# NVIDIA/tensorrt-laboratory

Hardware: NVIDIA H100
Metric: ResNet-50 fp16 b=8 inferences/sec (higher is better)
Workload: dtype f16

## Files before the change

### __graft_entry__.py

```python
from __future__ import annotations

import os
import re
import shutil
import subprocess
import sysconfig
import sys

ROOT = os.path.dirname(os.path.abspath(__file__))
PKG = os.path.join(ROOT, "tensorrt_laboratory_b200")
CSRC = os.path.join(PKG, "csrc")
LIB = os.path.join(PKG, "libb200infer.so")

NVCC_FLAGS = [
    "-gencode", "arch=compute_90a,code=sm_90a", "-lineinfo", "-O3", "-std=c++17",
    "-Xcompiler", "-fPIC,-Wall,-Wno-unused-function", "-cudart", "static",
]


def _nvcc() -> str:
    for cand in (os.environ.get("NVCC"), shutil.which("nvcc"), "/usr/local/cuda/bin/nvcc"):
        if cand and os.path.exists(cand):
            return cand
    raise RuntimeError("nvcc not found")


def _sources():
    srcs = []
    for root, _, files in os.walk(CSRC):
        for f in sorted(files):
            if f.endswith((".cu", ".cc")) and not f.endswith(("_main.cc", "_module.cc")):
                srcs.append(os.path.join(root, f))
    return srcs


def _stale(target: str, deps) -> bool:
    if not os.path.exists(target):
        return True
    t = os.path.getmtime(target)
    for d in deps:
        if os.path.getmtime(d) > t:
            return True
    return False


def _all_deps():
    deps = []
    for root, _, files in os.walk(CSRC):
        deps += [os.path.join(root, f) for f in files if f.endswith((".cu", ".cc", ".h", ".cuh", ".hpp"))]
    deps.append(os.path.join(ROOT, "include", "b200infer.h"))
    inc = os.path.join(ROOT, "include")
    for root, _, files in os.walk(inc):
        deps += [os.path.join(root, f) for f in files]
    return deps


_CONV_KERNEL = re.compile(r"conv|net_f16_tcgen05|attention_f16_wgmma|embed_ln|layernorm_h8|pooler")


_SHARED_SM_KERNEL = re.compile(r"_ZN3b2k(?:16conv_f16_tcgen05|20conv3x3_halo_tcgen05|24conv3x3_halo_1x1_tcgen05)ILi(\d+)E")
_SHARED_SM_THREADS = 320


def _shared_sm_register_budget(bn: int):
    ctas = 3 if bn <= 64 else 2 if bn <= 128 else 1
    return None if ctas == 1 else 65536 // (_SHARED_SM_THREADS * ctas) // 8 * 8


def _ptxas_violations(log: str):
    bad = [line.strip() for line in log.splitlines() if "(C7520)" in line or "(C7518)" in line]
    func = None
    for line in log.splitlines():
        m = re.search(r"Function properties for (\S+)", line)
        if m:
            func = m.group(1)
            continue
        m = re.search(r"(\d+) bytes spill stores, (\d+) bytes spill loads", line)
        if m and func and _CONV_KERNEL.search(func) and (int(m.group(1)) or int(m.group(2))):
            bad.append(f"{func}: {line.strip()}")
        m = re.search(r"Used (\d+) registers", line)
        k = _SHARED_SM_KERNEL.match(func) if (m and func) else None
        if k:
            budget = _shared_sm_register_budget(int(k.group(1)))
            if budget is not None and int(m.group(1)) > budget:
                bad.append(f"{func}: {m.group(1)} registers, more than the {budget} at which its CTAs share an SM")
    return bad


def _compile_object(cmd, obj: str, verbose: bool) -> None:
    r = subprocess.run(cmd + ["-Xptxas", "-v"], capture_output=True, text=True)
    log = r.stdout + r.stderr
    shown = [line for line in log.splitlines() if verbose or not (line.startswith("ptxas info") or "bytes stack frame" in line)]
    if shown:
        sys.stderr.write("\n".join(shown) + "\n")
    if r.returncode:
        raise subprocess.CalledProcessError(r.returncode, cmd)
    bad = _ptxas_violations(log)
    if bad:
        os.remove(obj)
        raise RuntimeError(f"{os.path.basename(obj)}: ptxas reports serialised wgmma, spilling convolution / transformer "
                           "kernels or tile kernels over their register budget:\n  " +
                           "\n  ".join(bad))


def build(force: bool = False, verbose: bool = False) -> None:
    nvcc = _nvcc()
    objdir = os.path.join(ROOT, "build", "obj")
    os.makedirs(objdir, exist_ok=True)
    deps = _all_deps()
    objs = []
    for src in _sources():
        obj = os.path.join(objdir, os.path.relpath(src, CSRC).replace(os.sep, "_") + ".o")
        objs.append(obj)
        if force or _stale(obj, deps):
            cmd = [nvcc] + NVCC_FLAGS + ["-I", os.path.join(ROOT, "include"), "-I", CSRC]
            if src.endswith(".cc"):
                cmd += ["-x", "cu"]
            cmd += ["-c", src, "-o", obj]
            if verbose:
                print(" ".join(cmd))
            _compile_object(cmd, obj, verbose)
    if force or _stale(LIB, objs):
        cmd = [nvcc, "-shared", "-cudart", "static", "-o", LIB] + objs + ["-lpthread", "-ldl", "-lrt"]
        if verbose:
            print(" ".join(cmd))
        subprocess.run(cmd, check=True)
    main_src = os.path.join(CSRC, "trtlab", "infer_main.cc")
    exe = os.path.join(ROOT, "examples", "infer.x")
    os.makedirs(os.path.dirname(exe), exist_ok=True)
    if os.path.exists(main_src) and (force or _stale(exe, deps + [LIB])):
        cmd = [nvcc] + NVCC_FLAGS + ["-I", os.path.join(ROOT, "include"), "-I", CSRC, "-x", "cu", main_src,
                                     "-o", exe, "-L", PKG, "-lb200infer", "-Xlinker", "-rpath,$ORIGIN/../tensorrt_laboratory_b200",
                                     "-lpthread", "-ldl"]
        if verbose:
            print(" ".join(cmd))
        subprocess.run(cmd, check=True)
    py_src = os.path.join(CSRC, "pybind", "trtlab_module.cc")
    py_mod = os.path.join(PKG, "trtlab" + sysconfig.get_config_var("EXT_SUFFIX"))
    if os.path.exists(py_src) and (force or _stale(py_mod, deps + [LIB, py_src])):
        import pybind11
        cmd = [nvcc] + NVCC_FLAGS + ["-I", os.path.join(ROOT, "include"), "-I", CSRC, "-I", pybind11.get_include(),
                                     "-I", sysconfig.get_paths()["include"], "-Xcompiler", "-fvisibility=hidden", "-x", "cu", "-shared", py_src,
                                     "-o", py_mod,
                                     "-L", PKG, "-lb200infer", "-Xlinker", "-rpath,$ORIGIN", "-lpthread", "-ldl"]
        if verbose:
            print(" ".join(cmd))
        subprocess.run(cmd, check=True)
    if ROOT not in sys.path:
        sys.path.insert(0, ROOT)
    import tensorrt_laboratory_b200
    from tensorrt_laboratory_b200 import capi
    capi.load()


def smoke() -> None:
    if ROOT not in sys.path:
        sys.path.insert(0, ROOT)
    if not os.path.exists(LIB):
        build()
    from tests import smoke_impl
    smoke_impl.run()


if __name__ == "__main__":
    build(force="--force" in sys.argv, verbose=True)
    if "--smoke" in sys.argv:
# ... 2 lines not shown
```

### tensorrt_laboratory_b200/csrc/engine.cu

```cuda
#include <cuda.h>
#include <cuda_runtime.h>
#include <stdarg.h>
#include <stdio.h>
#include <stdlib.h>
#include <string.h>

#include <algorithm>
#include <map>
#include <memory>
#include <mutex>
#include <string>
#include <vector>

#include "../../include/b200infer.h"
#include "kernels.h"
#include "plan_format.h"

#include "b2_internal.h"

namespace b2i {
thread_local std::string g_err;
int fail(int code, const char* fmt, ...) {
    char buf[1024];
    va_list ap;
// ... 106 lines not shown
             L_OUTPUT_CAST_F8 };

struct NetRun {
    b2k::NetArgs args{};
    int ctas = 0;
    int first_op = 0, last_op = 0;
    void* d_blob = nullptr;
    ~NetRun() {
        if (d_blob) cudaFree(d_blob);
    }
};

struct Launch {
    LKind kind;
    std::string name;
    double flops = 0, bytes = 0;
    b2k::ConvLaunch conv;
    b2k::SimtConvArgs simt;
    const void* in = nullptr;
    void* out = nullptr;
    const void* w = nullptr;
    const float* bias = nullptr;
    int in_binding = -1, out_binding = -1;
    bool src_half = false;
    int max_blocks = 0;
    int side_join = -1;
    std::shared_ptr<NetRun> net;
    b2k::TailArgs tail{};
    b2k::I8ConvLaunch i8{};
    float qscale = 0.f;
    int C_in_phys = 0;
    bool net_member = false;
    b2k::EmbedArgs embed{};
    int in_binding2 = -1, in_binding3 = -1;
    b2k::AttnLaunch attn{};
    float eps = 0.f;
    const int* live = nullptr;
    const int* pos_map = nullptr;
    int N = 0, C = 0, H = 0, W = 0, C_phys = 0, Ho = 0, Wo = 0, k = 0, stride = 0, pad = 0, K = 0, Cout = 0;
};

struct Segment {
    int begin = 0, end = 0;
    bool graphable = false;
    cudaGraphExec_t exec = nullptr;
};
struct BindPatch {
    int launch = -1;
    cudaGraphNode_t node = nullptr;
    cudaKernelNodeParams np{};
    std::vector<void*> params;
    int n_params = 0;
    std::vector<std::pair<int, int>> slots;
    std::vector<void*> values;
    b2k::TailArgs tail{};
    bool is_tail = false;
};
struct Plan {
    int batch = 0;
    bool has_net = false;
    std::vector<Launch> launches;
    std::vector<Segment> segments;
    bool graph_failed = false;
    cudaGraph_t graph = nullptr;
    cudaGraphExec_t exec = nullptr;
    std::vector<BindPatch> patches;
    ~Plan() {
        for (Segment& sg : segments)
            if (sg.exec) cudaGraphExecDestroy(sg.exec);
        if (exec) cudaGraphExecDestroy(exec);
        if (graph) cudaGraphDestroy(graph);
    }
};

}

struct ConvConfig {
    int bn, stages, splits;
    double est_us;
    int sps = 1;
    int ws = 0;
    int cn = 1;
    int halo = 0;
};
static bool stage_depth_useful(int bn, int kb, int st, int kpc) {
    const int stgs[4] = {1, 2, 4, 8};
    int cover = 0, deepest = 0;
    for (int s2 : stgs) {
        if (!b2k::conv_config_exists(bn, kb, s2)) continue;
        deepest = s2;
        if (!cover && s2 >= kpc) cover = s2;
    }
    return st <= (cover ? cover : deepest);
}


constexpr int kHaloStagesTag = 2;

struct b2_runtime {
    b2_alloc_fn alloc = nullptr;
    b2_free_fn free_ = nullptr;
    void* user = nullptr;
};

struct b2_engine {
    b2_runtime* rt = nullptr;
    b2_alloc_fn alloc = nullptr;
    b2_free_fn free_ = nullptr;
    void* alloc_user = nullptr;
    std::string name;
    int precision = 0, max_batch = 0;
    std::vector<Tensor> tensors;
    std::vector<Op> ops;
    std::vector<Binding> bindings;
    uint8_t* d_payload = nullptr;
    size_t payload_bytes = 0;
    size_t arena_bytes = 0;
    size_t act_bytes = 0;
    int device = -1;
    bool inspect_only = false;
    double flops_per_item = 0;
    std::mutex tune_mutex;
    std::mutex tune_run_mutex;
    std::map<std::pair<int, int>, ConvConfig> tuned;
    bool tune_cache_loaded = false;
    std::map<int, float> requant_r;
    bool tactics_from_plan = false;
    bool tuned_at_load = false;
    int pack_tensor = -1;
    bool half() const { return precision != B2_PREC_FP32; }
    bool one_byte() const { return precision == B2_PREC_INT8 || precision == B2_PREC_FP8; }
    bool fp8() const { return precision == B2_PREC_FP8; }
};

struct b2_context {
    b2_engine* e = nullptr;
    uint8_t* scratch = nullptr;
    struct ScratchState {
        std::map<int, std::unique_ptr<Plan>> plans;
    };
    std::map<uint8_t*, ScratchState> states;
    ScratchState* cur = nullptr;
    int* d_counters = nullptr;
    int use_graph = 1;
    int force_simt = 0;
    int force_im2col = 0;
    int force_bn = 0;
    int force_stages = 0;
    int force_splits = 0;
    int force_sps = 0;
    int force_halo = 0;
    int force_fuse = 0;
    int force_cn = 0;
    int force_ws = 0;
    int pdl_trigger = 1;
    int no_fold = 0;
    int autotune = 4;
    int fork = 0;
    int net = 0;
    int net_ctas = 0;
    int net_bn = 0;
    int net_stages = 0;
    int i8_bn = 0;
    int i8_stages = 0;
    int fuse_tail = 1;
    int input_ctas = 0;
    int* d_tail_ctrl = nullptr;
    cudaStream_t side = nullptr;
    cudaEvent_t fork_ev = nullptr, join_ev = nullptr;
};

namespace {

std::string fixed_str(const char* p, size_t n) {
    size_t len = 0;
    while (len < n && p[len]) ++len;
    return std::string(p, len);
}

int validate_transformer_op(b2_engine* e, const Op& op) {
    using namespace b2plan;
    const OpRec& r = op.r;
    const char* nm = op.name.c_str();
    auto act_ok = [&](const Tensor& t) { return t.kind == T_ACT && t.scale == 0.f && t.c % 8 == 0 && t.c <= 1024; };
    switch (r.type) {
        case OP_EMBED_LN: {
            const Tensor& to = e->tensors[r.out];
            const Tensor& tm = e->tensors[op.out2];
            const uint32_t want_c = (op.flags & kOpPacked) ? to.w + 2 : to.w;
            if (!act_ok(to) || to.h != 1 || tm.kind != T_VEC || tm.c != want_c || tm.binding >= 0)
                return fail(B2_EINVAL, "plan: embedding %s: needs an fp16 [1, S, C <= 1024, C %% 8 == 0] output and an fp32 [S] mask tensor "
                            "([S + 2] packing index when packed)", nm);
            if ((op.flags & kOpPacked) && to.w % 32)
                return fail(B2_EINVAL, "plan: packed embedding %s: S = %u is not a multiple of 32", nm, to.w);
            if (op.vocab < 1 || op.types < 1 || op.positions < int(to.w))
                return fail(B2_EINVAL, "plan: embedding %s: vocab %d / positions %d / types %d do not cover S = %u", nm, op.vocab, op.positions,
                            op.types, to.w);
            if (r.w_bytes != uint64_t(op.vocab + op.positions + op.types) * to.c * 2 || r.b_bytes != uint64_t(to.c) * 8)
                return fail(B2_EINVAL, "plan: embedding %s: table / gamma / beta sizes do not match hidden size %u", nm, to.c);
            if (!(op.eps >= 0.f && op.eps < 1.f)) return fail(B2_EINVAL, "plan: embedding %s: bad eps", nm);
            break;
        }
        case OP_LAYERNORM: {
            const Tensor& ti = e->tensors[r.in];
            const Tensor& to = e->tensors[r.out];
            if (!act_ok(ti) || !act_ok(to) || ti.h != to.h || ti.w != to.w || ti.c != to.c || ti.c_phys != to.c_phys)
                return fail(B2_EINVAL, "plan: layernorm %s: needs fp16 input and output of one shape, C %% 8 == 0, C <= 1024", nm);
            if (r.w_bytes != 0 || r.b_bytes != uint64_t(ti.c) * 8) return fail(B2_EINVAL, "plan: layernorm %s: gamma / beta size mismatch", nm);
            if (!(op.eps >= 0.f && op.eps < 1.f)) return fail(B2_EINVAL, "plan: layernorm %s: bad eps", nm);
            break;
        }
        case OP_ATTENTION: {
            const Tensor& ti = e->tensors[r.in];
            const Tensor& to = e->tensors[r.out];
            if (r.res < 0) return fail(B2_EINVAL, "plan: attention %s: no mask tensor", nm);
            const Tensor& tm = e->tensors[r.res];
            if (op.heads < 1 || uint32_t(op.heads) * 64 != to.c)
                return fail(B2_EINVAL, "plan: attention %s: heads * 64 (%d * 64) != hidden size %u", nm, op.heads, to.c);
            if (!act_ok(to) || ti.kind != T_ACT || ti.scale != 0.f || ti.c != 3 * to.c || ti.c_phys != ti.c)
                return fail(B2_EINVAL, "plan: attention %s: needs a fused fp16 QKV input of 3 x %u channels", nm, to.c);
            if (ti.h != 1 || to.h != 1 || ti.w != to.w || tm.kind != T_VEC || tm.c != ((op.flags & kOpPacked) ? ti.w + 2 : ti.w))
                return fail(B2_EINVAL, "plan: attention %s: S does not match between QKV, output and mask", nm);
            if (ti.w != 64 && (ti.w == 0 || ti.w % 128 || ti.w > 512))
                return fail(B2_EINVAL, "plan: attention %s: S = %u (64, or a multiple of 128 up to 512)", nm, ti.w);
            if (r.w_bytes || r.b_bytes) return fail(B2_EINVAL, "plan: attention %s carries no weights", nm);
            e->flops_per_item += 4.0 * double(ti.w) * ti.w * to.c;
            break;
        }
        case OP_POOLER: {
            const Tensor& ti = e->tensors[r.in];
            const Tensor& to = e->tensors[r.out];
            if (!act_ok(ti) || ti.h != 1 || to.kind != T_VEC || to.c != ti.c)
                return fail(B2_EINVAL, "plan: pooler %s: needs an fp16 [1, S, C] input and an fp32 [C] output", nm);
            if (r.w_bytes != uint64_t(ti.c) * ti.c * 2 || r.b_bytes != uint64_t(ti.c) * 4)
                return fail(B2_EINVAL, "plan: pooler %s: weight / bias size mismatch", nm);
            e->flops_per_item += 2.0 * ti.c * ti.c;
            break;
// ... 207 lines not shown
            if (to.h != ho || to.w != wo) return fail(B2_EINVAL, "plan: conv %s output dims mismatch", op.name.c_str());
            e->flops_per_item += 2.0 * ho * wo * r.cout * op.algo_k();
        } else if (r.type == OP_FC) {
            const Tensor& ti = e->tensors[r.in];
            const size_t K = size_t(ti.h) * ti.w * ti.c_phys;
            if (r.w_bytes != size_t(r.cout) * K * elt || r.b_bytes != size_t(r.cout) * 4)
                return fail(B2_EINVAL, "plan: fc %s weight size mismatch", op.name.c_str());
            e->flops_per_item += 2.0 * ti.h * ti.w * ti.c * r.cout;
        } else if (transformer_op) {
            int rc = validate_transformer_op(e, op);
            if (rc) return rc;
        }
        e->ops.push_back(op);
    }
    if (int rc = validate_packed_ops(e)) return rc;
    for (uint32_t i = 0; i < h.n_bindings; ++i, p += sizeof(BindingRec)) {
        BindingRec r;
        memcpy(&r, p, sizeof r);
        Binding b;
        b.name = fixed_str(r.name, 64);
        b.is_input = r.is_input != 0;
        b.dtype = r.dtype;
        b.tensor = r.tensor;
        b.nd = r.nd;
        if (r.nd == 0 || r.nd > 8) return fail(B2_EINVAL, "plan: binding %s has bad rank", b.name.c_str());
        if (r.dtype != B2_DT_FLOAT && !(r.dtype == B2_DT_HALF && b.is_input && h.precision == B2_PREC_FP16) &&
            !(r.dtype == B2_DT_INT32 && b.is_input && v3))
            return fail(B2_EINVAL, "plan: binding %s: bindings are fp32 (inputs of fp16 engines may be fp16)", b.name.c_str());
        size_t n = 1;
        for (uint32_t d = 0; d < 8; ++d) {
            b.dims[d] = d < r.nd ? r.dims[d] : 0;
            if (d < r.nd) n *= size_t(r.dims[d]);
        }
        b.item_bytes = n * (r.dtype == B2_DT_HALF ? 2 : 4);
        e->bindings.push_back(b);
    }
    for (const Op& op : e->ops) {
        const OpRec& r = op.r;
        if (r.type != OP_INPUT_CAST && r.type != OP_OUTPUT_CAST) continue;
        const Binding& b = e->bindings[size_t(r.binding)];
        const Tensor& t = e->tensors[size_t(r.type == OP_INPUT_CAST ? r.out : r.in)];
        size_t n = 1;
        for (int d = 0; d < b.nd; ++d) n *= size_t(b.dims[d] > 0 ? b.dims[d] : 0);
        const bool s2d = r.type == OP_INPUT_CAST && r.k == 2;
        if (b.is_input != (r.type == OP_INPUT_CAST) || (!s2d && n != size_t(t.c) * t.h * t.w))
            return fail(B2_EINVAL, "plan: cast op %s: binding %s and tensor %s disagree", op.name.c_str(), b.name.c_str(), t.name.c_str());
        if (b.dtype == B2_DT_INT32)
            return fail(B2_EINVAL, "plan: cast op %s reads int32 binding %s (int32 bindings feed the embedding op only)", op.name.c_str(),
                        b.name.c_str());
    }
    std::vector<int> int32_readers(e->bindings.size(), 0);
    for (const Op& op : e->ops) {
        const OpRec& r = op.r;
        if (r.type == OP_POOLER && e->tensors[r.out].binding >= 0 && e->bindings[size_t(e->tensors[r.out].binding)].is_input)
            return fail(B2_EINVAL, "plan: pooler %s writes an input binding", op.name.c_str());
        if (r.type != OP_EMBED_LN) continue;
        const uint32_t S = e->tensors[r.out].w;
        for (int bi : {r.binding, op.binding2, op.binding3}) {
            if (bi < 0 || bi >= int(h.n_bindings)) return fail(B2_EINVAL, "plan: embedding %s has a bad binding", op.name.c_str());
            const Binding& b = e->bindings[size_t(bi)];
            if (b.dtype != B2_DT_INT32 || !b.is_input || b.nd != 1 || b.dims[0] != int32_t(S))
                return fail(B2_EINVAL, "plan: embedding %s: binding %s must be an int32 input of shape [S = %u]", op.name.c_str(), b.name.c_str(), S);
            ++int32_readers[size_t(bi)];
        }
    }
    for (size_t i = 0; i < e->bindings.size(); ++i) {
        if (e->bindings[i].dtype != B2_DT_INT32) continue;
        if (int32_readers[i] != 1)
            return fail(B2_EINVAL, "plan: int32 binding %s must feed exactly one embedding op slot", e->bindings[i].name.c_str());
        for (const Tensor& t : e->tensors)
            if (t.binding == int(i))
                return fail(B2_EINVAL, "plan: int32 binding %s is the storage of tensor %s (int32 bindings feed the embedding op only)",
                            e->bindings[i].name.c_str(), t.name.c_str());
    }
    if (h.n_tactics) {
        if (h.tactics_offset > nbytes || size_t(h.n_tactics) > (nbytes - h.tactics_offset) / sizeof(TacticRec))
            return fail(B2_EINVAL, "plan: tactic table outside the blob");
        for (uint32_t i = 0; i < h.n_tactics; ++i) {
            TacticRec t;
            memcpy(&t, base + h.tactics_offset + size_t(i) * sizeof(TacticRec), sizeof t);
            if (t.op >= h.n_ops || t.batch == 0 || t.batch > h.max_batch) return fail(B2_EINVAL, "plan: tactic %u out of range", i);
            ConvConfig cfg{int(t.bn), int(t.stages), int(t.splits), 0.0, int(t.sps), int(t.ws), int(t.cn)};
            cfg.halo = int(t.halo);
            e->tuned[{int(t.op), int(t.batch)}] = cfg;
        }
        e->tactics_from_plan = true;
    }
    *payload = base + h.payload_offset;
    return B2_OK;
}

int fuse_partner(const b2_engine* e, int i);

void plan_arena(b2_engine* e) {
    int busy_until = -1;
    for (size_t i = 0; i < e->ops.size(); ++i) {
        Op& op = e->ops[i];
        op.side_join = -1;
        if (int(i) <= busy_until || op.r.type != b2plan::OP_CONV || op.r.out < 0 || e->tensors[op.r.out].binding >= 0) continue;
        int consumers = 0, join = -1;
        bool as_residual_only = true;
        for (size_t k = i + 1; k < e->ops.size(); ++k) {
            const auto& rk = e->ops[k].r;
            if (rk.in == op.r.out) ++consumers, as_residual_only = false;
            if (rk.res == op.r.out) ++consumers, join = int(k);
        }
        if (consumers == 1 && as_residual_only && join > int(i) + 1) {
            op.side_join = join;
            busy_until = join;
        }
    }
    for (size_t i = 0; i < e->ops.size(); ++i) {
        const auto& r = e->ops[i].r;
        for (int t : {r.out, e->ops[i].out2})
            if (t >= 0 && e->tensors[t].def < 0) e->tensors[t].def = int(i);
        for (int t : {r.in, r.res})
            if (t >= 0) e->tensors[t].last_use = std::max(e->tensors[t].last_use, int(i));
        if (e->ops[i].side_join >= 0 && r.in >= 0) e->tensors[r.in].last_use = std::max(e->tensors[r.in].last_use, e->ops[i].side_join);
        const int j = fuse_partner(e, int(i));
        if (j >= 0) e->tensors[r.in].last_use = std::max(e->tensors[r.in].last_use, j);
    }
    if (e->pack_tensor >= 0) e->tensors[size_t(e->pack_tensor)].last_use = int(e->ops.size()) - 1;
    struct Live {
        size_t off, size;
        int last;
    };
    std::vector<Live> live;
    size_t top = 0;
    std::vector<int> order;
    for (size_t i = 0; i < e->tensors.size(); ++i)
        if (e->tensors[i].binding < 0 && e->tensors[i].def >= 0) order.push_back(int(i));
    std::stable_sort(order.begin(), order.end(), [&](int a, int b) { return e->tensors[a].def < e->tensors[b].def; });
    for (int ti : order) {
        Tensor& t = e->tensors[ti];
        if (t.last_use < t.def) t.last_use = t.def;
        const size_t size = align_up(t.item_bytes * e->max_batch, 1024);
        const int slack = e->half() ? env_int("B2_ARENA_SLACK", env_int("B2_NET", 0) ? 2 : 0) : 0;
        live.erase(std::remove_if(live.begin(), live.end(), [&](const Live& l) { return l.last + slack < t.def; }), live.end());
        std::sort(live.begin(), live.end(), [](const Live& a, const Live& b) { return a.off < b.off; });
        size_t off = 0;
        for (const Live& l : live) {
            if (off + size <= l.off) break;
            off = std::max(off, l.off + l.size);
        }
        t.offset = off;
        live.push_back({off, size, t.last_use});
        top = std::max(top, off + size);
    }
    e->act_bytes = align_up(std::max<size_t>(top, 1024), 1024);
    e->arena_bytes = e->act_bytes + (e->half() ? kSplitWorkspaceBytes : 0);
}

int make_map_2d(CUtensorMap* map, const void* base, uint64_t inner, uint64_t outer, uint32_t box_inner,
                uint32_t box_outer, CUtensorMapSwizzle swz, bool int8 = false) {
    cuuint64_t dims[2] = {inner, outer};
    cuuint64_t strides[1] = {inner * (int8 ? 1u : 2u)};
    cuuint32_t box[2] = {box_inner, box_outer};
    cuuint32_t estr[2] = {1, 1};
    CUresult r = g_encode_tiled(map, int8 ? CU_TENSOR_MAP_DATA_TYPE_UINT8 : CU_TENSOR_MAP_DATA_TYPE_FLOAT16, 2, const_cast<void*>(base), dims, strides, box,
                                estr, CU_TENSOR_MAP_INTERLEAVE_NONE, swz, CU_TENSOR_MAP_L2_PROMOTION_L2_256B,
                                CU_TENSOR_MAP_FLOAT_OOB_FILL_NONE);
    if (r != CUDA_SUCCESS)
        return fail(B2_ECUDA, "cuTensorMapEncodeTiled failed (%d) dims=%llu,%llu box=%u,%u", int(r),
                    (unsigned long long)inner, (unsigned long long)outer, box_inner, box_outer);
    return B2_OK;
}
// ... 63 lines not shown
                const double t_kb = std::max(stage_bytes / (70000.0 / sharing), 1.0 / st);
                double t_epi = 0.6 + bn / 64.0 * 0.4 + (residual ? 0.4 : 0.0);
                if (splits > 1) t_epi += 1.0 + 0.3 * splits;
                const double t_cta = 2.0 + kpc * t_kb + t_epi;
                double total = waves * t_cta;
                const double traffic = double(ctas) * kpc * stage_bytes;
                total = std::max(total, traffic / 5.0e6 + 2.0);
                if (total < best.est_us) best = ConvConfig{bn, st, splits, total};
            }
        }
    }
    return best;
}

bool conv_is_row_folded(const b2_context* c, const Op& op) {
    const b2plan::OpRec& r = op.r;
    return !c->no_fold && r.cin_phys == 8 && op.kw() * 8 * 2 == 64 && op.sw() == 1 && op.pw_lo() == 0 && op.pw_hi() == 0;
}
int conv_kb(const b2_context* c, const Op& op) {
    if (op.r.cin_phys % 64 == 0) return 64;
    return conv_is_row_folded(c, op) ? 32 : 8;
}
int conv_num_kblocks(const b2_context* c, const Op& op) {
    const b2plan::OpRec& r = op.r;
    if (op.group_span()) return int(r.taps) * (op.group_span() / 64);
    if (r.cin_phys % 64 == 0) return int(r.taps) * (int(r.cin_phys) / 64);
    if (conv_is_row_folded(c, op)) return (op.kh() + 1) / 2;
    return (int(r.taps_phys) + 7) / 8;
}

int conv_halo_rows(const b2_engine* e, const Op& op) {
    const b2plan::OpRec& r = op.r;
    const Tensor& ti = e->tensors[r.in];
    const Tensor& to = e->tensors[r.out];
    if (op.groups > 1 || r.cin_phys % 64 || r.cout_phys % 64 || op.kh() != 3 || op.kw() != 3 || op.sh() != 1 || op.sw() != 1 || op.ph() != 1 ||
        op.pw_lo() != 1 || op.pw_hi() != 1 || r.res >= 0 || !(r.relu & 2) || ti.h != to.h || ti.w != to.w)
        return 0;
    const int wp = int(to.w) + 2;
    if (wp > 128) return 0;
    return std::min(128 / wp, int(to.h));
}
int conv_halo_rows(const b2_context* c, const Op& op) { return conv_halo_rows(c->e, op); }
bool conv_on_tensor_cores(const b2_engine* e, const Op& op);

int fuse_partner(const b2_engine* e, int i) {
    if (!e->half() || e->one_byte() || i < 0 || size_t(i) + 1 >= e->ops.size()) return -1;
    const Op &oi = e->ops[size_t(i)], &oj = e->ops[size_t(i) + 1];
    const b2plan::OpRec &ri = oi.r, &rj = oj.r;
    if (ri.type != b2plan::OP_CONV || rj.type != b2plan::OP_CONV || (ri.relu & (4 | b2plan::kConvGelu)) || conv_halo_rows(e, oi) == 0 ||
        !b2k::conv_halo_config_exists(int(ri.cout_phys)) || ri.cin_phys / 64 > 8)
        return -1;
    if (rj.in != ri.out || rj.res < 0 || rj.res == ri.out || oj.kh() != 1 || oj.kw() != 1 || oj.sh() != 1 || oj.sw() != 1 || oj.ph() != 0 ||
        oj.pw_lo() != 0 || oj.pw_hi() != 0 || oj.groups != 1 || !(rj.relu & 2) || (rj.relu & (4 | b2plan::kConvGelu)) ||
        rj.cin_phys != ri.cout_phys || rj.cout_phys % 64 || !conv_on_tensor_cores(e, oj) || e->tensors[ri.out].binding >= 0)
        return -1;
    for (size_t k = 0; k < e->ops.size(); ++k) {
        const b2plan::OpRec& rk = e->ops[k].r;
        if (k != size_t(i) + 1 && (rk.in == ri.out || rk.res == ri.out || e->ops[k].out2 == ri.out)) return -1;
        if (k == size_t(i) + 1 && rk.res == ri.out) return -1;
    }
    return i + 1;
}

bool conv_on_tensor_cores(const b2_engine* e, const Op& op) {
    const b2plan::OpRec& r = op.r;
    const bool kb64 = r.cin_phys % 64 == 0, kb8 = r.cin_phys == 8;
    return e->half() && (kb64 || kb8) && r.cout_phys % 32 == 0 && (kb64 || r.taps_phys % 2 == 0) && (op.groups == 1 || op.group_span() > 0);
}

bool conv_takes_stem_ws(const b2_context* c, const Op& op) {
    const b2plan::OpRec& r = op.r;
    return conv_is_row_folded(c, op) && op.kh() == 7 && op.sh() == 2 && r.cout_phys == 64 && c->e->tensors[r.out].w <= 128 &&
           (r.relu & b2plan::kConvRelu) && !(r.relu & 2) && !(r.relu & b2plan::kConvGelu) && r.res < 0 && op.groups == 1;
}

bool conv_takes_ws(const b2_context* c, const Op& op) {
    return conv_takes_stem_ws(c, op) || (conv_kb(c, op) == 64 && (op.r.relu & 2) && op.groups == 1 && !(op.r.relu & b2plan::kConvGelu));
}

bool tactic_applies(const b2_context* c, const Op& op, int batch, const ConvConfig& cfg) {
    const b2plan::OpRec& r = op.r;
    const Tensor& to = c->e->tensors[r.out];
    const int span = op.group_span(), kb = conv_kb(c, op);
    if (cfg.bn <= 0 || int(r.cout_phys) % cfg.bn || cfg.splits < 1 || cfg.sps < 1 || cfg.ws < 0) return false;
    if (op.groups > 1 && (!span || span % cfg.bn || cfg.splits > 1)) return false;
    if ((op.groups > 1 || (r.relu & b2plan::kConvGelu)) && (cfg.ws || cfg.cn > 1 || cfg.halo)) return false;
    if ((op.flags & b2plan::kOpPacked) && (cfg.ws || cfg.cn > 1 || cfg.halo || cfg.splits > 1)) return false;
    if (cfg.halo == 2) {
        const int j = fuse_partner(c->e, int(&op - &c->e->ops[0]));
        const int R = conv_halo_rows(c, op), cblocks = int(r.cin_phys) / 64;
        return j >= 0 && c->force_fuse >= 0 && cfg.bn == int(r.cout_phys) && cfg.splits == 1 && !cfg.ws && cfg.cn <= 1 &&
               b2k::conv_halo_fused_smem(cfg.bn, int(to.w), R, cblocks, int(c->e->ops[size_t(j)].r.cout_phys)) <= kSmemLimit;
    }
    if (cfg.halo) {
        const int R = conv_halo_rows(c, op), cblocks = int(r.cin_phys) / 64;
        return cfg.halo == 1 && R && cfg.splits == 1 && !cfg.ws && cfg.cn <= 1 && b2k::conv_halo_config_exists(cfg.bn) && cblocks <= 8 &&
               b2k::conv_halo_smem(cfg.bn, int(to.w), R, cblocks) <= kSmemLimit;
    }
    if (cfg.ws && conv_is_row_folded(c, op))
        return conv_takes_stem_ws(c, op) && cfg.bn == 64 && cfg.stages == b2k::kStemWsRing && cfg.sps == 1 && cfg.splits == 1 &&
               cfg.cn <= 1 && b2k::conv_stem_ws_smem() <= kSmemLimit;
    if (cfg.ws)
        return conv_takes_ws(c, op) && cfg.splits == 1 && cfg.cn <= 1 && b2k::conv_ws_config_exists(cfg.bn, cfg.stages, cfg.sps) &&
               b2k::conv_ws_smem(cfg.bn, cfg.stages, cfg.sps, r.res >= 0) <= kSmemLimit;
    if (!b2k::conv_config_exists(cfg.bn, kb, cfg.stages, cfg.sps) || b2k::conv_smem_bytes(cfg.bn, cfg.stages, r.res >= 0, cfg.sps) > kSmemLimit)
        return false;
    const int grid_n = int(r.cout_phys) / cfg.bn;
    if (cfg.cn > 1 && (kb != 64 || grid_n % cfg.cn || !b2k::conv_cluster_config_exists(cfg.bn, cfg.stages, cfg.sps, cfg.cn))) return false;
    if (cfg.splits > 1) {
        const int nkb = conv_num_kblocks(c, op), kpc = (nkb + cfg.splits - 1) / cfg.splits;
        const int tiles = (batch * int(to.h * to.w) + 127) / 128 * grid_n;
        if (kb != 64 || kpc < 4 || (cfg.splits - 1) * kpc >= nkb || tiles > kMaxSplitTiles ||
            size_t(tiles) * cfg.splits * 128 * cfg.bn * 4 > kSplitWorkspaceBytes)
            return false;
    }
    return true;
}

constexpr int kFuseMinStreams = 4;

ConvConfig fused_conv_config(const Op& op) {
    ConvConfig f{int(op.r.cout_phys), kHaloStagesTag, 1, 0.0, 1, 0, 1};
    f.halo = 2;
    return f;
}

std::vector<ConvConfig> conv_candidates(const b2_context* c, const Op& op, int batch, int fixed_splits) {
    const b2plan::OpRec& r = op.r;
    const int kbsz = conv_kb(c, op), nkb = conv_num_kblocks(c, op);
    const int m_tiles = (batch * int(c->e->tensors[r.out].h * c->e->tensors[r.out].w) + 127) / 128;
    const bool ws_only = c->force_ws > 0 && conv_takes_ws(c, op);
    auto ok = [&](const ConvConfig& t) { return tactic_applies(c, op, batch, t); };
    std::vector<ConvConfig> out;
    for (int bn : {256, 128, 64, 32}) {
        if (int(r.cout_phys) % bn) continue;
        const int tiles = m_tiles * (int(r.cout_phys) / bn);
        for (int ws = 0; ws <= 1; ++ws)
        for (int sp : {1, 2, 4, 8})
        for (int sps = 1; sps <= 2; ++sps)
        for (int st : {1, 2, 4, 8}) {
            if ((fixed_splits > 0 && sp != fixed_splits) || (ws ? c->force_ws < 0 : ws_only)) continue;
            ConvConfig t{bn, st, sp, 0.0, sps, ws ? std::min(tiles, g_sms) : 0, 1};
            if (!ok(t)) continue;
            if (ws) {
                if (sps == 2 && nkb < 4) continue;
                out.push_back(t);
                if (tiles > g_sms / 2) t.ws = g_sms / 2, out.push_back(t);
                continue;
            }
            const int kpc = (nkb + sp - 1) / sp;
            if (sps == 2 ? (kpc < 4 || st * 2 > kpc + 2) : !stage_depth_useful(bn, kbsz, st, kpc)) continue;
            if (sp > 1 && (tiles >= 100 || tiles > kMaxSplitTiles / 8 || tiles * sp > 160)) continue;
            ConvConfig cl = t;
            cl.cn = c->force_cn;
            out.push_back(c->force_cn > 1 && ok(cl) ? cl : t);
        }
    }
    if (conv_takes_stem_ws(c, op) && c->force_ws >= 0 && fixed_splits <= 1) {
        const int rows = batch * int(c->e->tensors[r.out].h);
        ConvConfig t{64, b2k::kStemWsRing, 1, 0.0, 1, std::min(rows, g_sms), 1};
        if (ok(t)) {
            out.push_back(t);
            if (rows > g_sms / 2) t.ws = g_sms / 2, out.push_back(t);
        }
    }
    if (c->force_halo >= 0 && fixed_splits <= 1) {
        std::vector<ConvConfig> halo;
        for (int bn : {256, 128, 64, 32}) {
            const ConvConfig h{bn, kHaloStagesTag, 1, 0.0, 1, 0, 1, 1};
            if (ok(h)) halo.push_back(h);
        }
        if (!halo.empty() && c->force_halo > 0) out.clear();
        out.insert(out.end(), halo.begin(), halo.end());
    }
    return out;
}

ConvConfig forced_conv_config(const b2_context* c, const Op& op, int batch) {
    const b2plan::OpRec& r = op.r;
    const int M = batch * int(c->e->tensors[r.out].h * c->e->tensors[r.out].w);
    const int kbsz = conv_kb(c, op), nkb = conv_num_kblocks(c, op);
    ConvConfig cfg = pick_conv_config(M, int(r.cout_phys), nkb, kbsz, r.res >= 0, c, true, op.group_span());
    if (cfg.bn == 0 || ((op.flags & b2plan::kOpPacked) && cfg.splits > 1))
        cfg = pick_conv_config(M, int(r.cout_phys), nkb, kbsz, r.res >= 0, c, false, op.group_span());
    if (cfg.bn == 0) return cfg;
    auto force = [&](auto set) {
        ConvConfig t = cfg;
        set(t);
        if (tactic_applies(c, op, batch, t)) cfg = t;
    };
    if (c->force_sps == 2) force([](ConvConfig& t) { t.sps = 2; });
    if (c->force_ws > 0)
        force([&](ConvConfig& t) {
            if (conv_takes_stem_ws(c, op)) {
                t = ConvConfig{64, b2k::kStemWsRing, 1, t.est_us, 1, 0, 1};
                t.ws = std::min(batch * int(c->e->tensors[r.out].h), c->force_ws > 1 ? c->force_ws : g_sms);
                return;
            }
            t.ws = std::min((M + 127) / 128 * (int(r.cout_phys) / t.bn), c->force_ws > 1 ? c->force_ws : g_sms);
        });
    if (c->force_halo > 0) force([](ConvConfig& t) { t.halo = 1, t.ws = 0, t.cn = 1; });
    if (c->force_cn > 1) force([&](ConvConfig& t) { t.cn = c->force_cn; });
    return cfg;
}

int make_conv_launch(b2_context* c, const Op& op, int batch, const ConvConfig& cfg, b2k::ConvLaunch* out) {
    b2_engine* e = c->e;
    const b2plan::OpRec& r = op.r;
    const Tensor& ti = e->tensors[r.in];
    const Tensor& to = e->tensors[r.out];
    auto tptr = [&](int idx) -> uint8_t* { return c->scratch + e->tensors[idx].offset; };
    const uint8_t* w = e->d_payload + r.w_off;
    const int M = batch * int(to.h) * int(to.w);
    const bool kb64 = r.cin_phys % 64 == 0;
    const bool fold = conv_is_row_folded(c, op);
    const int span = op.group_span();
    if (!tactic_applies(c, op, batch, cfg))
        return fail(B2_EINVAL, "conv %s: tactic bn=%d st=%d sps=%d splits=%d ws=%d cn=%d halo=%d does not apply", op.name.c_str(), cfg.bn,
                    cfg.stages, cfg.sps, cfg.splits, cfg.ws, cfg.cn, cfg.halo);
    const bool gelu = (r.relu & b2plan::kConvGelu) != 0;
    b2k::ConvLaunch& cl = *out;
    memset(&cl, 0, sizeof cl);
    cl.kb = conv_kb(c, op);
    cl.grid_m = (M + 127) / 128;
    const int nkb = conv_num_kblocks(c, op);
    cl.bn = cfg.bn;
    cl.stages = cfg.stages;
    cl.sps = cfg.sps;
    cl.grid_n = int(r.cout_phys) / cl.bn;
    cl.ws_ctas = cfg.ws;
    cl.cn = std::max(cfg.cn, 1);
    cl.args.cn = cl.cn;
    cl.args.tiles_m = cl.grid_m;
    cl.args.tiles_n = cl.grid_n;
    b2k::ConvArgs& a = cl.args;
    a.splits = cfg.splits;
    a.kb_per_split = (nkb + cfg.splits - 1) / cfg.splits;
    a.workspace = reinterpret_cast<float*>(c->scratch + e->act_bytes);
    a.tile_counters = c->d_counters;
    a.pdl_trigger = c->pdl_trigger;
    a.bias = reinterpret_cast<const float*>(e->d_payload + r.b_off);
    a.residual = r.res >= 0 ? reinterpret_cast<const __half*>(tptr(r.res)) : nullptr;
    a.out = reinterpret_cast<__half*>(tptr(r.out));
    a.M = M;
    a.Cout = int(r.cout_phys);
    a.taps = fold ? op.kh() : int(r.taps);
    a.taps_phys = fold ? op.kh() : int(r.taps_phys);
    a.kw = fold ? 1 : op.kw();
    a.cblocks = span ? span / 64 : kb64 ? int(r.cin_phys) / 64 : 1;
    a.group_span = span;
    a.num_kblocks = nkb;
    a.HoWo = int(to.h * to.w);
    a.Wo = int(to.w);
    a.stride_h = op.sh();
    a.stride_w = op.sw();
    a.pad_h = op.ph();
    a.pad_w = op.pw_lo();
    a.relu = int(r.relu & (b2plan::kConvRelu | b2plan::kConvGelu));
    a.wpacked = (r.relu & 2) ? w : nullptr;
    const bool tiled = r.k == 1 && op.kw() == 1 && r.stride == 1 && op.sw() == 1 && r.pad_ == 0 && op.pw_lo() == 0 &&
                       op.pw_hi() == 0 && kb64 && (!c->force_im2col || gelu || (op.flags & b2plan::kOpPacked));
    a.a_mode = tiled ? b2k::A_TILED : b2k::A_IM2COL;
    if (cfg.halo) {
        const int R = conv_halo_rows(c, op);
        cl.halo = 1;
        cl.ws_ctas = 0, cl.cn = 1, a.cn = 1, a.splits = 1, cl.stages = kHaloStagesTag, cl.sps = 1;
        a.halo_rows = R;
        cl.grid_m = batch * ((int(to.h) + R - 1) / R);
        int rc = make_map_nhwc(&cl.mapA, tptr(r.in), int(r.cin_phys), int(ti.w), int(ti.h), batch, uint32_t(ti.w) + 2, uint32_t(R) + 2);
        if (rc) return rc;
        cl.mapB = cl.mapA;
        if (cfg.halo == 2) {
            const Op& oj = e->ops[size_t(fuse_partner(e, int(&op - &e->ops[0])))];
            const b2plan::OpRec& rj = oj.r;
            cl.halo = 2;
            cl.c2.wpacked = e->d_payload + rj.w_off;
            cl.c2.bias = reinterpret_cast<const float*>(e->d_payload + rj.b_off);
            cl.c2.Cout = int(rj.cout_phys);
            cl.c2.relu = int(rj.relu & b2plan::kConvRelu);
            rc = make_map_nhwc(&cl.mapOut, tptr(rj.out), int(rj.cout_phys), int(to.w), int(to.h), batch, uint32_t(to.w) + 2, uint32_t(R));
            if (!rc) rc = make_map_nhwc(&cl.mapRes, tptr(rj.res), int(rj.cout_phys), int(to.w), int(to.h), batch, uint32_t(to.w) + 2, uint32_t(R));
            return rc;
        }
        rc = make_map_nhwc(&cl.mapOut, tptr(r.out), int(r.cout_phys), int(to.w), int(to.h), batch, uint32_t(to.w) + 2, uint32_t(R));
        cl.mapRes = cl.mapOut;
        return rc;
    }
    const CUtensorMapSwizzle swz = kb64 ? CU_TENSOR_MAP_SWIZZLE_128B : (fold ? CU_TENSOR_MAP_SWIZZLE_64B : CU_TENSOR_MAP_SWIZZLE_NONE);
    const uint64_t pix = uint64_t(r.cin_phys) * 2, rowb = uint64_t(ti.w) * pix, imgb = uint64_t(ti.h) * rowb;
    int rc;
    if (tiled)
        rc = make_map_2d(&cl.mapA, tptr(r.in), r.cin_phys, uint64_t(M), 64, uint32_t(128 / cl.cn), swz);
    else if (fold)
        rc = make_map_im2col(&cl.mapA, tptr(r.in), int(r.cin_phys) * op.kw(), int(ti.w) - op.kw() + 1, int(ti.h), batch, pix,
                             rowb, imgb, op.kh(), 1, op.sh(), 1, op.ph(), 0, 0, 32, 128, swz);
    else
        rc = make_map_im2col(&cl.mapA, tptr(r.in), int(r.cin_phys), int(ti.w), int(ti.h), batch, pix, rowb, imgb, op.kh(),
                             op.kw(), op.sh(), op.sw(), op.ph(), op.pw_lo(), op.pw_hi(), uint32_t(cl.kb), uint32_t(128 / cl.cn), swz);
    if (rc) return rc;
    if (r.relu & 2)
        cl.mapB = cl.mapA;
    else
        rc = make_map_2d(&cl.mapB, w, uint64_t(r.taps_phys) * r.cin_phys, r.cout_phys, uint32_t(cl.kb), uint32_t(cl.bn), swz);
    if (rc) return rc;
    if (cfg.ws && fold) {
        rc = make_map_nhwc(&cl.mapOut, tptr(r.out), int(r.cout_phys), int(to.w), int(to.h), batch, 128, 1);
        cl.mapRes = cl.mapOut;
        return rc;
    }
    const uint32_t ow = cl.bn >= 64 ? 64 : 32;
    const CUtensorMapSwizzle oswz = cl.bn >= 64 ? CU_TENSOR_MAP_SWIZZLE_128B : CU_TENSOR_MAP_SWIZZLE_64B;
    rc = make_map_2d(&cl.mapOut, tptr(r.out), r.cout_phys, uint64_t(M), ow, 128, oswz);
    if (rc) return rc;
    if (r.res >= 0) rc = make_map_2d(&cl.mapRes, tptr(r.res), r.cout_phys, uint64_t(M), ow, 128, oswz);
    else cl.mapRes = cl.mapOut;
    return rc;
}

int make_i8_conv_launch(b2_context* c, const Op& op, int batch, int bn, int stages, b2k::I8ConvLaunch* out) {
    b2_engine* e = c->e;
    const b2plan::OpRec& r = op.r;
    const Tensor& ti = e->tensors[r.in];
    const Tensor& to = e->tensors[r.out];
    auto tptr = [&](int idx) -> uint8_t* { return c->scratch + e->tensors[idx].offset; };
    b2k::I8ConvLaunch& cl = *out;
    memset(&cl, 0, sizeof cl);
    const int M = batch * int(to.h) * int(to.w);
    cl.bn = bn, cl.stages = stages;
    cl.grid_m = (M + 127) / 128;
    cl.grid_n = int(r.cout_phys) / bn;
    b2k::I8ConvArgs& a = cl.args;
    a.wpacked = e->d_payload + r.w_off;
    const float* rq = reinterpret_cast<const float*>(e->d_payload + r.b_off);
    a.m = rq;
    a.b = rq + r.cout_phys;
    a.r = e->requant_r.at(int(&op - &e->ops[0]));
    a.has_res = r.res >= 0 ? 1 : 0;
    a.relu = int(r.relu & 1);
    a.M = M, a.Cout = int(r.cout_phys);
    a.cblocks = int(r.cin_phys) / 128;
    a.last_cb_mmas = (int(r.cin) % 128) ? (int(r.cin) % 128 + 31) / 32 : 4;
    a.cout_real = int(r.cout);
    a.num_kblocks = int(r.taps) * a.cblocks;
    a.kw = op.kw(), a.HoWo = int(to.h * to.w), a.Wo = int(to.w);
    a.stride_h = op.sh(), a.stride_w = op.sw(), a.pad_h = op.ph(), a.pad_w = op.pw_lo();
    const bool tiled = r.k == 1 && r.stride == 1 && r.pad_ == 0;
    a.a_mode = tiled ? b2k::A_TILED : b2k::A_IM2COL;
    int rc;
    if (tiled)
        rc = make_map_2d(&cl.mapA, tptr(r.in), r.cin_phys, uint64_t(M), 128, 128, CU_TENSOR_MAP_SWIZZLE_128B, true);
    else {
        const uint64_t pix = uint64_t(r.cin_phys), rowb = uint64_t(ti.w) * pix, imgb = uint64_t(ti.h) * rowb;
        rc = make_map_im2col(&cl.mapA, tptr(r.in), int(r.cin_phys), int(ti.w), int(ti.h), batch, pix, rowb, imgb, op.kh(), op.kw(), op.sh(),
                             op.sw(), op.ph(), op.pw_lo(), op.pw_hi(), 128, 128, CU_TENSOR_MAP_SWIZZLE_128B, true);
    }
    if (rc) return rc;
    rc = make_map_2d(&cl.mapOut, tptr(r.out), r.cout_phys, uint64_t(M), 128, 128, CU_TENSOR_MAP_SWIZZLE_128B, true);
    if (rc) return rc;
    if (r.res >= 0) rc = make_map_2d(&cl.mapRes, tptr(r.res), r.cout_phys, uint64_t(M), 128, 128, CU_TENSOR_MAP_SWIZZLE_128B, true);
    else cl.mapRes = cl.mapOut;
    return rc;
}

struct TuneTimer {
    const int ns;
    const int iters = std::max(4, env_int("B2_TUNE_ITERS", 12));
    const int reps = std::max(1, env_int("B2_TUNE_REPS", 3));
    std::vector<cudaStream_t> ss;
    std::vector<cudaEvent_t> done;
    cudaEvent_t e0 = nullptr, e1 = nullptr;

    explicit TuneTimer(const b2_context* c) : ns(std::max(1, std::min(c->autotune, 8))), ss(size_t(ns), nullptr), done(size_t(ns), nullptr) {}
    ~TuneTimer() {
// ... 5 lines not shown
        if (e1) cudaEventDestroy(e1);
    }
    int init() {
        bool ok = cudaEventCreate(&e0) == cudaSuccess && cudaEventCreate(&e1) == cudaSuccess;
        for (int i = 0; i < ns && ok; ++i)
            ok = cudaStreamCreateWithFlags(&ss[size_t(i)], cudaStreamNonBlocking) == cudaSuccess &&
                 cudaEventCreateWithFlags(&done[size_t(i)], cudaEventDisableTiming) == cudaSuccess;
        if (ok) return B2_OK;
        cudaGetLastError();
        return fail(B2_ECUDA, "autotune: cannot create streams/events");
    }
    template <class F>
    cudaError_t time(F launch, float* ms) {
        int rc = 0;
        for (int i = 0; i < 2 && !rc; ++i)
            for (int k = 0; k < ns && !rc; ++k) rc = launch(k, ss[size_t(k)]);
        for (auto s : ss) cudaStreamSynchronize(s);
        *ms = 1e30f;
        if (rc) return cudaError_t(rc);
        cudaGraph_t g = nullptr;
        cudaGraphExec_t ge = nullptr;
        cudaError_t se = cudaStreamBeginCapture(ss[0], cudaStreamCaptureModeThreadLocal);
        if (se != cudaSuccess) return se;
        cudaEventRecord(done[0], ss[0]);
        for (int k = 1; k < ns; ++k) cudaStreamWaitEvent(ss[size_t(k)], done[0], 0);
        for (int i = 0; i < iters && !rc; ++i)
            for (int k = 0; k < ns && !rc; ++k) rc = launch(k, ss[size_t(k)]);
        for (int k = 1; k < ns; ++k) {
            cudaEventRecord(done[size_t(k)], ss[size_t(k)]);
            cudaStreamWaitEvent(ss[0], done[size_t(k)], 0);
        }
        se = cudaStreamEndCapture(ss[0], &g);
        if (!rc && se == cudaSuccess) se = cudaGraphInstantiate(&ge, g, 0);
        if (!rc && se == cudaSuccess) se = cudaGraphLaunch(ge, ss[0]);
        if (!rc && se == cudaSuccess) se = cudaStreamSynchronize(ss[0]);
        for (int rep = 0; rep < reps && !rc && se == cudaSuccess; ++rep) {
            cudaEventRecord(e0, ss[0]);
            se = cudaGraphLaunch(ge, ss[0]);
            cudaEventRecord(e1, ss[0]);
            if (se == cudaSuccess) se = cudaStreamSynchronize(ss[0]);
            float t = 0.f;
            if (se == cudaSuccess && cudaEventElapsedTime(&t, e0, e1) == cudaSuccess) *ms = std::min(*ms, t);
        }
        if (ge) cudaGraphExecDestroy(ge);
        if (g) cudaGraphDestroy(g);
        if (rc || se != cudaSuccess) cudaGetLastError();
        return rc ? cudaError_t(rc) : se;
    }
    double us_per_launch(double ms) const { return ms * 1e3 / (iters * ns); }
};

int autotune_conv(b2_context* c, const Op& op, int batch, int fixed_splits, ConvConfig* best_out) {
    const b2plan::OpRec& r = op.r;
    const Tensor& to = c->e->tensors[r.out];
    const int M = batch * int(to.h) * int(to.w);
    TuneTimer tt(c);
    int status = tt.init();
    if (status) return status;
    const int verbose = env_int("B2_TUNE_VERBOSE", 0);
    ConvConfig best = *best_out;
    double best_ms = 1e30;
    for (const ConvConfig& cand : conv_candidates(c, op, batch, fixed_splits)) {
        b2k::ConvLaunch cl0;
        if ((status = make_conv_launch(c, op, batch, cand, &cl0))) return status;
        std::vector<b2k::ConvLaunch> cls(size_t(tt.ns), cl0);
        void* tmp_ws = nullptr;
        if (cand.splits > 1) {
            const size_t ws_bytes = size_t(cl0.grid_m) * cl0.grid_n * cand.splits * 128 * cand.bn * 4;
            if (cudaMalloc(&tmp_ws, ws_bytes * tt.ns) != cudaSuccess) {
                cudaGetLastError();
                continue;
            }
            for (int k = 0; k < tt.ns; ++k) {
                cls[size_t(k)].args.workspace = reinterpret_cast<float*>(static_cast<uint8_t*>(tmp_ws) + ws_bytes * k);
                cls[size_t(k)].args.tile_counters = c->d_counters + k * (kMaxSplitTiles / 8);
            }
        }
        float ms = 0.f;
        const cudaError_t err = tt.time([&](int k, cudaStream_t s) { return b2k::launch_conv_f16_tcgen05(cls[size_t(k)], s); }, &ms);
        if (tmp_ws) cudaFree(tmp_ws);
        if (err != cudaSuccess)
            return fail(B2_ECUDA, "autotune of %s (bn=%d st=%d) failed: %s", op.name.c_str(), cand.bn, cand.stages, cudaGetErrorString(err));
        if (verbose > 1)
            fprintf(stderr, "[b2 tune]   %s b=%d cand bn=%d st=%d sp=%d sps=%d ws=%d cn=%d halo=%d : %.3f us/launch\n", op.name.c_str(),
                    batch, cand.bn, cand.stages, cand.splits, cand.sps, cand.ws, cand.cn, cand.halo, tt.us_per_launch(ms));
        if (ms < best_ms) best_ms = ms, best = cand;
    }
    best.est_us = tt.us_per_launch(best_ms);
    if (verbose)
        fprintf(stderr, "[b2 tune] %s b=%d M=%d N=%d K=%d best bn=%d st=%d sp=%d sps=%d ws=%d cn=%d halo=%d : %.3f us/launch (%d streams)\n",
                op.name.c_str(), batch, M, int(r.cout_phys), conv_num_kblocks(c, op) * conv_kb(c, op), best.bn, best.stages, best.splits,
                best.sps, best.ws, best.cn, best.halo, best.est_us, tt.ns);
    *best_out = best;
    return B2_OK;
}

void tune_cache_load(b2_engine* e) {
    if (e->tune_cache_loaded) return;
    e->tune_cache_loaded = true;
    const char* path = getenv("B2_TUNE_CACHE");
    if (!path) return;
    FILE* f = fopen(path, "r");
    if (!f) return;
    char name[128];
    int op, batch, bn, st, sp, sps, ws, cn, halo;
    while (fscanf(f, "%127s %d %d %d %d %d %d %d %d %d", name, &op, &batch, &bn, &st, &sp, &sps, &ws, &cn, &halo) == 10)
        if (e->name == name && op >= 0 && op < int(e->ops.size())) {
            ConvConfig cfg{bn, st, sp, 0.0, sps, ws, cn};
            cfg.halo = halo;
            e->tuned[{op, batch}] = cfg;
        }
    fclose(f);
}
void tune_cache_append(const b2_engine* e, int op, int batch, const ConvConfig& cfg) {
    const char* path = getenv("B2_TUNE_CACHE");
    if (!path) return;
    FILE* f = fopen(path, "a");
    if (!f) return;
    fprintf(f, "%s %d %d %d %d %d %d %d %d %d\n", e->name.c_str(), op, batch, cfg.bn, cfg.stages, cfg.splits, cfg.sps, cfg.ws, cfg.cn,
            cfg.halo);
    fclose(f);
}

int autotune_i8_conv(b2_context* c, const Op& op, int batch, ConvConfig* best_out) {
    const b2plan::OpRec& r = op.r;
    TuneTimer tt(c);
    int status = tt.init();
    if (status) return status;
    const int verbose = env_int("B2_TUNE_VERBOSE", 0);
    const bool fp8 = c->e->fp8();
    const char* fmt = fp8 ? "fp8" : "int8";
    double best_ms = 1e30;
    ConvConfig best = *best_out;
    for (int bn : {128, 256}) {
        if (int(r.cout_phys) % bn) continue;
        for (int st = 1; st <= 4; ++st) {
            if (!b2k::conv_i8_config_exists(bn, st)) continue;
            b2k::I8ConvLaunch cl;
            if ((status = make_i8_conv_launch(c, op, batch, bn, st, &cl))) return status;
            float ms = 0.f;
            const cudaError_t err = tt.time(
                [&](int, cudaStream_t s) { return fp8 ? b2k::launch_conv_f8_tcgen05(cl, s) : b2k::launch_conv_i8_tcgen05(cl, s); }, &ms);
            if (err != cudaSuccess)
                return fail(B2_ECUDA, "autotune of %s (%s bn=%d st=%d) failed: %s", op.name.c_str(), fmt, bn, st, cudaGetErrorString(err));
            if (verbose > 1)
                fprintf(stderr, "[b2 tune]   %s b=%d cand %s bn=%d st=%d : %.3f us/launch\n", op.name.c_str(), batch, fmt, bn, st,
                        tt.us_per_launch(ms));
            if (ms < best_ms) best_ms = ms, best = ConvConfig{bn, st, 1, 0.0, 1, 0, 1};
        }
    }
    best.est_us = tt.us_per_launch(best_ms);
    if (verbose) {
        const Tensor& to = c->e->tensors[r.out];
        const long long M = (long long)batch * to.h * to.w, K = (long long)r.k * r.k * r.cin_phys;
        fprintf(stderr, "[b2 tune] %s b=%d M=%lld N=%d K=%lld best %s bn=%d st=%d : %.3f us/launch (%d streams) %.0f TOP/s\n",
                op.name.c_str(), batch, M, int(r.cout_phys), K, fmt, best.bn, best.stages, best.est_us, tt.ns,
                2.0 * M * r.cout_phys * K / best.est_us * 1e-6);
    }
    *best_out = best;
    return B2_OK;
}

int tune_engine_batch(b2_context* c, int batch) {
    b2_engine* e = c->e;
    for (size_t i = 0; i < e->ops.size(); ++i) {
        const Op& op = e->ops[i];
        const b2plan::OpRec& r = op.r;
        if (r.type != b2plan::OP_CONV || !e->half()) continue;
        if (r.relu & 4) {
            {
                std::lock_guard<std::mutex> lock(e->tune_mutex);
                if (e->tuned.count({int(i), batch})) continue;
            }
            ConvConfig cfg{128, 2, 1, 0.0, 1, 0, 1};
            int rc = autotune_i8_conv(c, op, batch, &cfg);
            if (rc) return rc;
            std::lock_guard<std::mutex> lock(e->tune_mutex);
            e->tuned[{int(i), batch}] = cfg;
            tune_cache_append(e, int(i), batch, cfg);
            continue;
        }
        if (!conv_on_tensor_cores(e, op)) continue;
        {
            std::lock_guard<std::mutex> lock(e->tune_mutex);
            if (e->tuned.count({int(i), batch})) continue;
        }
        const Tensor& to = e->tensors[r.out];
        const int kbsz = conv_kb(c, op), nkb = conv_num_kblocks(c, op);
        const bool side = op.side_join >= 0;
        const bool no_split = side || op.groups > 1;
        static const bool tune_splitk = env_int("B2_TUNE_SPLITK", 0) != 0;
        int splits = (no_split || !tune_splitk) ? 1 : 0;
        if (batch != e->max_batch && !no_split && tune_splitk) {
            std::lock_guard<std::mutex> lock(e->tune_mutex);
            auto it = e->tuned.find({int(i), e->max_batch});
            if (it != e->tuned.end()) splits = it->second.splits;
        }
        ConvConfig cfg = pick_conv_config(batch * int(to.h) * int(to.w), int(r.cout_phys), nkb, kbsz, r.res >= 0, c, false,
                                          op.group_span());
        int rc = autotune_conv(c, op, batch, splits, &cfg);
        if (rc) return rc;
        std::lock_guard<std::mutex> lock(e->tune_mutex);
        e->tuned[{int(i), batch}] = cfg;
// ... 246 lines not shown
    if (e->pack_tensor >= 0) {
        pos_map = reinterpret_cast<int*>(tptr(e->pack_tensor));
        seq_off = pos_map + size_t(batch) * (e->tensors[size_t(e->pack_tensor)].c - 2);
    }
    for (const Op& op : e->ops) {
        const b2plan::OpRec& r = op.r;
        Launch L;
        L.name = op.name;
        L.N = batch;
        L.side_join = op.side_join;
        switch (r.type) {
            case b2plan::OP_INPUT_CAST: {
                const Tensor& t = e->tensors[r.out];
                L.kind = L_INPUT_CAST;
                L.in_binding = r.binding;
                L.src_half = e->bindings[r.binding].dtype == B2_DT_HALF;
                L.out = tptr(r.out);
                L.C = t.c, L.H = t.h, L.W = t.w, L.C_phys = t.c_phys;
                L.k = int(r.k);
                L.max_blocks = c->input_ctas;
                if (r.k == 2) {
                    const Binding& b = e->bindings[r.binding];
                    if (!half || b.nd != 3 || b.dims[0] > 4 || t.c_phys != 8 || int(t.h) != b.dims[1] ||
                        int(t.w) != b.dims[2] / 2 + int(r.pad_) + int(r.stride) || b.dims[2] % 2)
                        return fail(B2_EINVAL, "input cast %s: inconsistent space-to-depth geometry", op.name.c_str());
                    L.C = b.dims[0], L.W = b.dims[2];
                    L.pad = int(r.pad_), L.stride = int(r.stride);
                }
                L.bytes = double(batch) * t.h * t.w * (t.c * 4.0 + t.c_phys * elt);
                break;
            }
            case b2plan::OP_QUANTIZE: {
                const Tensor& ti = e->tensors[r.in];
                const Tensor& to = e->tensors[r.out];
                L.kind = e->fp8() ? L_QUANTIZE_F8 : L_QUANTIZE;
                L.in = tptr(r.in), L.out = tptr(r.out);
                L.C = ti.c, L.H = ti.h, L.W = ti.w, L.C_in_phys = ti.c_phys, L.C_phys = to.c_phys;
                L.qscale = float(1.0 / double(to.scale));
                L.bytes = double(batch) * (ti.item_bytes + to.item_bytes);
                break;
            }
            case b2plan::OP_OUTPUT_CAST: {
                const Tensor& t = e->tensors[r.in];
                L.kind = t.scale > 0.f ? (e->fp8() ? L_OUTPUT_CAST_F8 : L_OUTPUT_CAST_I8) : (op.flags & b2plan::kOpPacked) ? L_OUTPUT_UNPACK : (op.flags & 1) ? L_OUTPUT_ROWS : L_OUTPUT_CAST;
                if (L.kind == L_OUTPUT_UNPACK) L.pos_map = pos_map;
                if (L.kind == L_OUTPUT_ROWS && !half) return fail(B2_EINVAL, "output cast %s: channels-last outputs need an fp16 engine", op.name.c_str());
                L.qscale = t.scale;
                L.in = tptr(r.in);
                L.out_binding = r.binding;
                L.C = t.c, L.H = t.h, L.W = t.w, L.C_phys = t.c_phys;
                L.bytes = double(batch) * t.h * t.w * (t.c * 4.0 + t.c_phys * elt);
                break;
            }
            case b2plan::OP_CONV: {
                const Tensor& ti = e->tensors[r.in];
                const Tensor& to = e->tensors[r.out];
                const uint8_t* w = e->d_payload + r.w_off;
                const float* bias = reinterpret_cast<const float*>(e->d_payload + r.b_off);
                const int M = batch * int(to.h) * int(to.w);
                L.flops = 2.0 * M * r.cout * op.algo_k();
                L.bytes = double(batch) * (ti.item_bytes + to.item_bytes * (r.res >= 0 ? 2 : 1)) + double(r.w_bytes);
                if (r.relu & 4) {
                    L.kind = e->fp8() ? L_CONV_F8 : L_CONV_I8;
                    const int m_tiles = (batch * int(e->tensors[r.out].h * e->tensors[r.out].w) + 127) / 128;
                    int bn = 128, st = m_tiles * (int(r.cout_phys) / 128) >= 2 * g_sms ? 1 : 2;
                    if (c->autotune) {
                        std::lock_guard<std::mutex> lock(e->tune_mutex);
                        tune_cache_load(e);
                        const int op_index = int(&op - &e->ops[0]);
                        auto it = e->tuned.find({op_index, batch});
                        if (it == e->tuned.end()) it = e->tuned.find({op_index, e->max_batch});
                        if (it != e->tuned.end()) bn = it->second.bn, st = it->second.stages;
                    }
                    if (c->i8_bn > 0) bn = c->i8_bn;
                    if (c->i8_stages > 0) st = c->i8_stages;
                    if (int(r.cout_phys) % bn) bn = 128;
                    if (!b2k::conv_i8_config_exists(bn, st)) bn = 128, st = 2;
                    int rc = make_i8_conv_launch(c, op, batch, bn, st, &L.i8);
                    if (rc) return rc;
                } else if (!c->force_simt && conv_on_tensor_cores(e, op)) {
                    L.kind = L_CONV_TC;
                    ConvConfig cfg = forced_conv_config(c, op, batch);
                    if (cfg.bn == 0) return fail(B2_EINVAL, "conv %s: no kernel configuration", op.name.c_str());
                    const bool forced = c->force_bn || c->force_stages || c->force_splits || c->force_sps;
                    const int op_index = int(&op - &e->ops[0]);
                    const bool net_ok = c->net && !forced && conv_kb(c, op) == 64 && (r.relu & 2) && r.cout_phys % 64 == 0 &&
                                        c->force_ws <= 0 && c->force_cn <= 0 && c->force_halo <= 0 && !c->force_im2col && op.groups == 1 &&
                                        !(r.relu & b2plan::kConvGelu) &&
                                        !(op.flags & b2plan::kOpPacked);
                    if (net_ok) {
                        int bn = (r.cout_phys % 128 == 0) ? 128 : 64;
                        if (c->net_bn == 64) bn = 64;
                        cfg = ConvConfig{bn, 4, 1, 0.0, 1, 0, 1};
                        cfg.halo = 0;
                        L.net_member = true;
                    } else if (!forced && c->autotune) {
                        std::lock_guard<std::mutex> lock(e->tune_mutex);
                        tune_cache_load(e);
                        auto it = e->tuned.find({op_index, batch});
                        if (it == e->tuned.end()) it = e->tuned.find({op_index, e->max_batch});
                        if (it != e->tuned.end() && tactic_applies(c, op, batch, it->second)) cfg = it->second;
                    }
                    if (!net_ok && c->force_fuse > 0) {
                        const ConvConfig f = fused_conv_config(op);
                        if (tactic_applies(c, op, batch, f)) cfg = f;
                    }
                    if (op.side_join >= 0 && cfg.splits > 1) cfg.splits = 1;
                    int rc = make_conv_launch(c, op, batch, cfg, &L.conv);
                    if (rc) return rc;
                    if (op.flags & b2plan::kOpPacked) L.conv.args.live_rows = seq_off + batch, L.conv.args.live = 1;
                } else {
                    L.kind = L_CONV_SIMT;
                    b2k::SimtConvArgs& a = L.simt;
                    memset(&a, 0, sizeof a);
                    a.in = tptr(r.in), a.w = w, a.bias = bias;
                    a.residual = r.res >= 0 ? tptr(r.res) : nullptr;
                    a.out = tptr(r.out);
                    a.N = batch, a.H = int(ti.h), a.W = int(ti.w), a.Cin = int(r.cin), a.Cin_phys = int(r.cin_phys);
                    a.Ho = int(to.h), a.Wo = int(to.w), a.Cout = int(r.cout), a.Cout_phys = int(r.cout_phys);
                    a.kh = op.kh(), a.kw = op.kw(), a.taps_phys = int(r.taps_phys);
                    a.stride_h = op.sh(), a.stride_w = op.sw(), a.pad_h = op.ph(), a.pad_w = op.pw_lo();
                    a.relu = int(r.relu & (b2plan::kConvRelu | b2plan::kConvGelu));
                    a.w_packed = int((r.relu >> 1) & 1);
                    a.groups = op.groups;
                    a.wk_tap = op.groups == 1 ? int(r.cin_phys) : op.group_span() ? op.group_span() : int(r.cin) / op.groups;
                }
                break;
            }
            case b2plan::OP_MAXPOOL: {
                const Tensor& ti = e->tensors[r.in];
                const Tensor& to = e->tensors[r.out];
                L.kind = L_MAXPOOL;
                L.in = tptr(r.in), L.out = tptr(r.out);
                L.H = ti.h, L.W = ti.w, L.C_phys = ti.c_phys, L.Ho = to.h, L.Wo = to.w;
                L.k = r.k, L.stride = r.stride, L.pad = r.pad_;
                L.bytes = double(batch) * (ti.item_bytes + to.item_bytes);
                break;
            }
            case b2plan::OP_AVGPOOL: {
                const Tensor& ti = e->tensors[r.in];
                L.kind = ti.scale > 0.f ? (e->fp8() ? L_AVGPOOL_F8 : L_AVGPOOL_I8) : L_AVGPOOL;
                L.in = tptr(r.in), L.out = tptr(r.out);
                L.H = ti.h, L.W = ti.w, L.C_phys = ti.c_phys;
                if (ti.scale > 0.f) {
                    L.C = ti.c, L.C_in_phys = ti.c_phys, L.C_phys = e->tensors[r.out].c_phys;
                    L.qscale = float(double(ti.scale) / double(ti.h * ti.w));
                }
                L.bytes = double(batch) * ti.item_bytes;
                break;
            }
            case b2plan::OP_FC: {
                const Tensor& ti = e->tensors[r.in];
                const Tensor& to = e->tensors[r.out];
                L.kind = L_FC;
                L.in = tptr(r.in);
                L.out = tptr(r.out);
                L.out_binding = to.binding;
                L.w = e->d_payload + r.w_off;
                L.bias = reinterpret_cast<const float*>(e->d_payload + r.b_off);
                L.K = int(ti.h * ti.w * ti.c_phys);
                L.Cout = int(r.cout);
                L.flops = 2.0 * batch * ti.h * ti.w * ti.c * r.cout;
                L.bytes = double(r.w_bytes) + double(batch) * (ti.item_bytes + to.item_bytes);
                break;
            }
            case b2plan::OP_SOFTMAX: {
                const Tensor& ti = e->tensors[r.in];
// ... 418 lines not shown
        if (!rc) rc = b2k::init_attention_kernels();
        if (rc) return fail(B2_ECUDA, "kernel attribute setup failed: %s", cudaGetErrorString(cudaError_t(rc)));
        const size_t bytes = std::max<size_t>(e->payload_bytes, 256);
        if (rt && rt->alloc) {
            e->alloc = rt->alloc, e->free_ = rt->free_, e->alloc_user = rt->user;
            e->d_payload = static_cast<uint8_t*>(rt->alloc(rt->user, bytes, 256, 0));
            if (!e->d_payload) return fail(B2_ENOMEM, "user allocator returned null for %zu weight bytes", bytes);
        } else {
            void* p = nullptr;
            if (cudaMalloc(&p, bytes) != cudaSuccess) {
                cudaGetLastError();
                return fail(B2_ENOMEM, "cudaMalloc(%zu) for weights failed", bytes);
            }
            e->d_payload = static_cast<uint8_t*>(p);
        }
        if (e->payload_bytes) B2_CUDA(cudaMemcpy(e->d_payload, payload, e->payload_bytes, cudaMemcpyHostToDevice));
    }
    *out = e.release();
    return B2_OK;
}

int b2_engine_deserialize(b2_runtime* rt, const void* blob, size_t nbytes, b2_engine** out) {
    return deserialize_impl(rt, blob, nbytes, false, out);
}

int b2_engine_inspect(const void* blob, size_t nbytes, b2_engine** out) {
    return deserialize_impl(nullptr, blob, nbytes, true, out);
}

void b2_engine_destroy(b2_engine* e) {
    if (!e) return;
    if (e->d_payload) {
        if (e->free_)
            e->free_(e->alloc_user, e->d_payload);
        else
            cudaFree(e->d_payload);
    }
    delete e;
}

int b2_engine_nb_bindings(const b2_engine* e) { return e ? int(e->bindings.size()) : 0; }
const char* b2_engine_binding_name(const b2_engine* e, int i) {
    return (e && i >= 0 && i < int(e->bindings.size())) ? e->bindings[i].name.c_str() : nullptr;
}
int b2_engine_binding_index(const b2_engine* e, const char* name) {
    if (!e || !name) return -1;
    for (size_t i = 0; i < e->bindings.size(); ++i)
        if (e->bindings[i].name == name) return int(i);
    return -1;
}
int b2_engine_binding_is_input(const b2_engine* e, int i) {
    return (e && i >= 0 && i < int(e->bindings.size())) ? int(e->bindings[i].is_input) : 0;
}
int b2_engine_binding_dtype(const b2_engine* e, int i) {
    return (e && i >= 0 && i < int(e->bindings.size())) ? e->bindings[i].dtype : -1;
}
int b2_engine_binding_dims(const b2_engine* e, int i, int32_t* dims, int* nd) {
    if (!e || i < 0 || i >= int(e->bindings.size()) || !dims || !nd) return fail(B2_EINVAL, "bad binding query");
    *nd = e->bindings[i].nd;
    for (int d = 0; d < 8; ++d) dims[d] = e->bindings[i].dims[d];
    return B2_OK;
}
int b2_engine_max_batch(const b2_engine* e) { return e ? e->max_batch : 0; }
int b2_engine_precision(const b2_engine* e) { return e ? e->precision : -1; }
const char* b2_engine_name(const b2_engine* e) { return e ? e->name.c_str() : nullptr; }
size_t b2_engine_device_memory_size(const b2_engine* e) { return e ? e->arena_bytes : 0; }
size_t b2_engine_weights_size(const b2_engine* e) { return e ? e->payload_bytes : 0; }
double b2_engine_flops(const b2_engine* e, int batch) { return e ? e->flops_per_item * batch : 0.0; }
int b2_engine_nb_layers(const b2_engine* e) { return e ? int(e->ops.size()) : 0; }

int b2_context_create(b2_engine* e, b2_context** out) {
    if (!e || !out) return fail(B2_EINVAL, "null engine or out");
    if (e->inspect_only) return fail(B2_ESTATE, "engine was loaded with b2_engine_inspect (no device resources)");
    b2_context* c = new b2_context();
    c->e = e;
    c->use_graph = env_int("B2_GRAPH", 1);
    c->force_simt = env_int("B2_FORCE_SIMT", 0);
    c->force_im2col = env_int("B2_FORCE_IM2COL", 0);
    c->force_bn = env_int("B2_FORCE_BN", 0);
    c->force_stages = env_int("B2_FORCE_STAGES", 0);
    c->force_splits = env_int("B2_FORCE_SPLITS", 0);
    c->force_sps = env_int("B2_FORCE_SPS", 0);
    c->force_ws = env_int("B2_FORCE_WS", 0);
    c->force_cn = env_int("B2_FORCE_CN", 0);
    c->force_halo = env_int("B2_FORCE_HALO", 0);
    c->force_fuse = env_int("B2_FORCE_FUSE", 0);
    c->pdl_trigger = env_int("B2_PDL_TRIGGER", 1);
    c->autotune = env_int("B2_AUTOTUNE", 4);
    c->fork = env_int("B2_FORK", 0);
    c->net = env_int("B2_NET", 0);
    c->net_ctas = env_int("B2_NET_CTAS", 0);
    c->net_bn = env_int("B2_NET_BN", 0);
    c->net_stages = env_int("B2_NET_STAGES", 0);
    c->fuse_tail = env_int("B2_FUSE_TAIL", 1);
    c->input_ctas = env_int("B2_INPUT_CTAS", 0);
    c->i8_bn = env_int("B2_I8_BN", 0);
    c->i8_stages = env_int("B2_I8_STAGES", 0);
    if (getenv("B2_PDL")) b2k::set_pdl(env_int("B2_PDL", 1) != 0);
    void* p = nullptr;
    if (cudaMalloc(&p, (kMaxSplitTiles + 16) * sizeof(int)) != cudaSuccess || cudaMemset(p, 0, (kMaxSplitTiles + 16) * sizeof(int)) != cudaSuccess) {
        cudaGetLastError();
        delete c;
        return fail(B2_ENOMEM, "cudaMalloc for split-K counters failed");
    }
    c->d_counters = static_cast<int*>(p);
    c->d_tail_ctrl = c->d_counters + kMaxSplitTiles;
    *out = c;
    return B2_OK;
}

static void drop_cached(b2_context* c) {
    c->states.clear();
    c->cur = c->scratch ? &c->states[c->scratch] : nullptr;
}

void b2_context_destroy(b2_context* c) {
    if (!c) return;
    drop_cached(c);
    if (c->d_counters) cudaFree(c->d_counters);
    if (c->side) cudaStreamDestroy(c->side);
    if (c->fork_ev) cudaEventDestroy(c->fork_ev);
    if (c->join_ev) cudaEventDestroy(c->join_ev);
    delete c;
}

int b2_context_set_device_memory(b2_context* c, void* scratch) {
    if (!c || !scratch) return fail(B2_EINVAL, "null context or scratch");
    if (reinterpret_cast<uintptr_t>(scratch) % 256 != 0) return fail(B2_EINVAL, "scratch must be 256-byte aligned (cudaMalloc alignment)");
    if (c->states.size() >= 32 && c->states.find(static_cast<uint8_t*>(scratch)) == c->states.end()) drop_cached(c);
    c->scratch = static_cast<uint8_t*>(scratch);
    c->cur = &c->states[c->scratch];
    return B2_OK;
}

int b2_context_set_option(b2_context* c, const char* key, int value) {
    if (!c || !key) return fail(B2_EINVAL, "null context or key");
    const std::string k(key);
    if (k == "graph") {
        c->use_graph = value;
        return B2_OK;
    }
    if (k == "pdl") {
        b2k::set_pdl(value != 0);
        value = 0;
    } else if (k == "simt") c->force_simt = value;
    else if (k == "im2col") c->force_im2col = value;
    else if (k == "bn") c->force_bn = value;
    else if (k == "stages") c->force_stages = value;
    else if (k == "splits") c->force_splits = value;
    else if (k == "sps") c->force_sps = value;
    else if (k == "ws") c->force_ws = value;
    else if (k == "cn") c->force_cn = value;
    else if (k == "halo") c->force_halo = value;
    else if (k == "fuse") c->force_fuse = value;
    else if (k == "fork") c->fork = value;
    else if (k == "net") c->net = value;
    else if (k == "net_ctas") c->net_ctas = value;
    else if (k == "net_bn") c->net_bn = value;
    else if (k == "net_stages") c->net_stages = value;
    else if (k == "fuse_tail") c->fuse_tail = value;
    else if (k == "i8_bn") c->i8_bn = value;
    else if (k == "i8_stages") c->i8_stages = value;
    else if (k == "input_ctas") c->input_ctas = value;
    else if (k == "pdl_trigger") c->pdl_trigger = value;
    else if (k == "autotune") c->autotune = value;
    else if (k == "no_fold") c->no_fold = value;
    else return fail(B2_EINVAL, "unknown option '%s'", key);
    drop_cached(c);
    return B2_OK;
}

int b2_context_nb_launches(b2_context* c, int batch) {
    if (!c) return -1;
    Plan* plan = nullptr;
    if (build_plan(c, batch, &plan)) return -1;
    return int(plan->launches.size());
}

int b2_engine_tune(b2_engine* e, int streams, int all_batches) {
    if (!e) return fail(B2_EINVAL, "null engine");
    if (e->inspect_only) return fail(B2_ESTATE, "engine was loaded with b2_engine_inspect (no device resources)");
    if (!e->half() || e->tactics_from_plan) return B2_OK;
    std::lock_guard<std::mutex> run_lock(e->tune_run_mutex);
    b2_context* c = nullptr;
    int rc = b2_context_create(e, &c);
    if (rc) return rc;
    c->autotune = streams > 0 ? streams : c->autotune;
    void* scratch = nullptr;
    if (c->autotune <= 0) {
        b2_context_destroy(c);
        return B2_OK;
    }
    if (cudaMalloc(&scratch, std::max<size_t>(e->arena_bytes, 1024)) != cudaSuccess) {
        cudaGetLastError();
        b2_context_destroy(c);
        return fail(B2_ENOMEM, "cudaMalloc(%zu) for the tuning arena failed", e->arena_bytes);
    }
    rc = b2_context_set_device_memory(c, scratch);
    if (!rc && load_driver_entry_points() != 0) rc = fail(B2_ECUDA, "cuTensorMapEncode* driver entry points unavailable");
    {
        std::lock_guard<std::mutex> lock(e->tune_mutex);
        tune_cache_load(e);
    }
    if (!rc) rc = tune_engine_batch(c, e->max_batch);
    for (int b = 1; !rc && all_batches && b < e->max_batch; ++b) rc = tune_engine_batch(c, b);
    cudaDeviceSynchronize();
    b2_context_destroy(c);
    cudaFree(scratch);
    if (!rc) e->tuned_at_load = true;
    return rc;
}

namespace {
struct RefineCtx {
    b2_context* c = nullptr;
    void* scratch = nullptr;
    std::vector<void*> bind;
    cudaStream_t s = nullptr;
};
}

int b2_engine_refine_tactics(b2_engine* e, int streams, int passes, double* gain_out) {
    if (gain_out) *gain_out = 1.0;
    if (!e) return fail(B2_EINVAL, "null engine");
    if (e->inspect_only) return fail(B2_ESTATE, "engine was loaded with b2_engine_inspect (no device resources)");
    if (!e->half() || e->tactics_from_plan) return B2_OK;
    streams = std::max(1, std::min(streams > 0 ? streams : 4, 8));
    int rc = b2_engine_tune(e, streams, 0);
    if (rc) return rc;
    std::lock_guard<std::mutex> run_lock(e->tune_run_mutex);
    const int batch = e->max_batch;
    std::vector<RefineCtx> ctx(static_cast<size_t>(streams));
    cudaEvent_t e0 = nullptr, e1 = nullptr;
    auto cleanup = [&] {
// ... 51 lines not shown
            if (cudaStreamSynchronize(ctx[0].s) != cudaSuccess) {
                status = fail(B2_ECUDA, "refine: forward pass failed: %s", cudaGetErrorString(cudaGetLastError()));
                break;
            }
            float ms = 0.f;
            cudaEventElapsedTime(&ms, e0, e1);
            if (rep > 0) best = std::min(best, double(ms) / (double(n) * double(ctx.size())));
        }
        return best;
    };
    double base = measure();
    const double first = base;
    const double keep = 1.0 - std::max(0.0, double(env_int("B2_REFINE_MIN_GAIN_PERMILLE", 7))) / 1000.0;
    for (int pass = 0; pass < std::max(1, passes) && !status; ++pass) {
        int changed = 0;
        for (size_t i = 0; i < e->ops.size() && !status; ++i) {
            const Op& op = e->ops[i];
            const b2plan::OpRec& r = op.r;
            if (r.type != b2plan::OP_CONV || (r.relu & 4)) continue;
            ConvConfig cur;
            {
                std::lock_guard<std::mutex> lock(e->tune_mutex);
                auto it = e->tuned.find({int(i), batch});
                if (it == e->tuned.end()) continue;
                cur = it->second;
            }
            const int kbsz = conv_kb(ctx[0].c, op);
            if (kbsz != 64 || cur.ws || cur.cn > 1) continue;
            const int nkb = conv_num_kblocks(ctx[0].c, op);
            std::vector<ConvConfig> cands;
            if (env_int("B2_TUNE_SPLITK", 0) != 0 && !(op.side_join >= 0) && op.groups == 1 && cur.splits == 1 && !cur.halo) {
                const int m_tiles = (batch * int(e->tensors[r.out].h * e->tensors[r.out].w) + 127) / 128;
                for (int sp : {2, 4}) {
                    const int tiles = m_tiles * (int(r.cout_phys) / cur.bn);
                    if (nkb < 16 || tiles >= 100 || tiles * sp > 160 || tiles > kMaxSplitTiles / 8) continue;
                    for (int st : {2, 4})
                        if (tactic_applies(ctx[0].c, op, batch, ConvConfig{cur.bn, st, sp, 0.0, 1, 0, 1}))
                            cands.push_back(ConvConfig{cur.bn, st, sp, 0.0, 1, 0, 1});
                }
            }
            if (cur.splits > 1) continue;
            for (const ConvConfig& t : conv_candidates(ctx[0].c, op, batch, 1))
                if (!t.ws && t.cn <= 1 && t.splits == 1 &&
                    !(t.bn == cur.bn && t.stages == cur.stages && t.sps == cur.sps && t.halo == cur.halo))
                    cands.push_back(t);
            if (streams >= kFuseMinStreams && cur.halo != 2 && tactic_applies(ctx[0].c, op, batch, fused_conv_config(op)))
                cands.push_back(fused_conv_config(op));
            ConvConfig best = cur;
            for (const ConvConfig& cand : cands) {
                {
                    std::lock_guard<std::mutex> lock(e->tune_mutex);
                    e->tuned[{int(i), batch}] = cand;
                }
                const double t = measure();
                if (status) break;
                if (t < base * keep) base = t, best = cand, ++changed;
            }
            std::lock_guard<std::mutex> lock(e->tune_mutex);
            e->tuned[{int(i), batch}] = best;
        }
        if (!changed) break;
    }
    if (!status) {
        const double last = measure();
        if (gain_out && last > 0 && last < 1e29) *gain_out = first / last;
    }
    cleanup();
    return status;
}

int b2_engine_nb_tactics(const b2_engine* e) {
    if (!e) return 0;
    std::lock_guard<std::mutex> lock(const_cast<b2_engine*>(e)->tune_mutex);
    return int(e->tuned.size());
}
int b2_engine_get_tactics(const b2_engine* e, uint32_t* out, int cap) {
    if (!e || !out) return 0;
    std::lock_guard<std::mutex> lock(const_cast<b2_engine*>(e)->tune_mutex);
    int n = 0;
    for (const auto& kv : e->tuned) {
        if (n >= cap) break;
        const ConvConfig& g = kv.second;
        const uint32_t rec[10] = {uint32_t(kv.first.first), uint32_t(kv.first.second), uint32_t(g.bn), uint32_t(g.stages), uint32_t(g.splits),
                                  uint32_t(g.sps), uint32_t(g.ws), uint32_t(g.cn), uint32_t(g.halo), 0u};
        memcpy(out + size_t(n) * 10, rec, sizeof rec);
        ++n;
    }
    return n;
}

int b2_context_prepare(b2_context* c, int batch, b2_stream_t stream_) {
    if (!c) return fail(B2_EINVAL, "null context");
    if (batch < 1 || batch > c->e->max_batch) return fail(B2_EINVAL, "batch %d outside [1, %d]", batch, c->e->max_batch);
    Plan* plan = nullptr;
    int rc = build_plan(c, batch, &plan);
    if (rc) return rc;
    if (!c->use_graph || plan->has_net) return B2_OK;
    cudaStream_t stream = static_cast<cudaStream_t>(stream_);
    cudaStream_t own = nullptr;
    if (!stream) {
        B2_CUDA(cudaStreamCreateWithFlags(&own, cudaStreamNonBlocking));
        stream = own;
    }
    std::vector<void*> dummy(c->e->bindings.size(), reinterpret_cast<void*>(uintptr_t(256)));
    if (c->use_graph != 3 && !plan->exec && !plan->graph_failed) {
        rc = instantiate_plan_graph(c, plan, dummy.data(), stream);
        plan->graph_failed = !rc && plan->exec == nullptr;
    }
    if (!rc && !plan->exec)
        for (Segment& sg : plan->segments)
            if (sg.graphable && !sg.exec && (rc = instantiate_segment(c, plan, &sg, dummy.data(), stream))) break;
    if (own) cudaStreamDestroy(own);
    return rc;
}

int b2_context_enqueue(b2_context* c, int batch, void* const* bindings, b2_stream_t stream_, b2_event_t consumed) {
    int rc = check_args(c, batch, bindings);
    if (rc) return rc;
    cudaStream_t stream = static_cast<cudaStream_t>(stream_);
    Plan* plan = nullptr;
    if ((rc = build_plan(c, batch, &plan))) return rc;
    cudaStreamCaptureStatus cap = cudaStreamCaptureStatusNone;
    B2_CUDA(cudaStreamIsCapturing(stream, &cap));
    if (cap != cudaStreamCaptureStatusNone || !c->use_graph || plan->has_net) {
        if ((rc = run_all(c, *plan, bindings, stream))) return rc;
    } else {
        if (c->use_graph != 3 && !plan->exec && !plan->graph_failed) {
            if ((rc = instantiate_plan_graph(c, plan, bindings, stream))) return rc;
            plan->graph_failed = plan->exec == nullptr;
        }
        if (plan->exec) {
            if ((rc = patch_plan_graph(plan, bindings))) return rc;
            B2_CUDA(cudaGraphLaunch(plan->exec, stream));
        } else {
            for (Segment& sg : plan->segments) {
                if (!sg.graphable) {
                    if ((rc = run_range(c, *plan, size_t(sg.begin), size_t(sg.end), bindings, stream))) return rc;
                    continue;
                }
                if (!sg.exec && (rc = instantiate_segment(c, plan, &sg, bindings, stream))) return rc;
                B2_CUDA(cudaGraphLaunch(sg.exec, stream));
            }
        }
    }
    if (consumed) B2_CUDA(cudaEventRecord(static_cast<cudaEvent_t>(consumed), stream));
    return B2_OK;
}

int b2_context_profile(b2_context* c, int batch, void* const* bindings, b2_stream_t stream_, float* ms, int cap) {
    if (check_args(c, batch, bindings)) return -1;
    cudaStream_t stream = static_cast<cudaStream_t>(stream_);
    Plan* plan = nullptr;
    if (build_plan(c, batch, &plan)) return -1;
    const int n = int(plan->launches.size());
    std::vector<cudaEvent_t> ev(n + 1);
    for (auto& e : ev) cudaEventCreate(&e);
    int rc = 0;
    cudaEventRecord(ev[0], stream);
    for (int i = 0; i < n && !rc; ++i) {
        rc = run_launch(c->e, plan->launches[i], bindings, stream);
        cudaEventRecord(ev[i + 1], stream);
    }
    cudaError_t se = cudaStreamSynchronize(stream);
    if (rc || se != cudaSuccess) {
        fail(B2_ECUDA, "profile run failed: %s", cudaGetErrorString(rc ? cudaError_t(rc) : se));
        n > 0 ? (void)0 : (void)0;
    } else {
// ... 8 lines not shown
    Plan* plan = nullptr;
    if (build_plan(c, batch, &plan)) return nullptr;
    if (i < 0 || i >= int(plan->launches.size())) return nullptr;
    return &plan->launches[i];
}
int b2_context_debug_conv_timing(b2_context* c, int batch, int i, int reps, b2_stream_t stream_, long long* stamps,
                                 int cap_ctas, int* n_ctas) {
    const int dbg_mode = env_int("B2_DBG_MODE", 0);
    Plan* plan = nullptr;
    if (!c || build_plan(c, batch, &plan)) return fail(B2_EINVAL, "no plan");
    if (i < 0 || i >= int(plan->launches.size()) || plan->launches[i].kind != L_CONV_TC) return fail(B2_EINVAL, "not a tcgen05 conv launch");
    b2k::ConvLaunch cl = plan->launches[i].conv;
    const int ctas = cl.ws_ctas > 0 ? cl.ws_ctas : cl.grid_m * cl.grid_n * cl.args.splits;
    if (n_ctas) *n_ctas = ctas;
    if (ctas > cap_ctas) return fail(B2_EINVAL, "stamp buffer too small (%d CTAs)", ctas);
    long long* d = nullptr;
    B2_CUDA(cudaMalloc(&d, size_t(ctas) * 16 * sizeof(long long)));
    cudaMemset(d, 0, size_t(ctas) * 16 * sizeof(long long));
    cl.args.dbg = d;
    cl.args.dbg_mode = dbg_mode;
    cudaStream_t s = static_cast<cudaStream_t>(stream_);
    int rc = 0;
    for (int r = 0; r < reps && !rc; ++r) rc = b2k::launch_conv_f16_tcgen05(cl, s);
    cudaError_t se = cudaStreamSynchronize(s);
    if (!rc && se == cudaSuccess) cudaMemcpy(stamps, d, size_t(ctas) * 16 * sizeof(long long), cudaMemcpyDeviceToHost);
    cudaFree(d);
    if (rc || se != cudaSuccess) return fail(B2_ECUDA, "debug launch failed: %s", cudaGetErrorString(rc ? cudaError_t(rc) : se));
    return B2_OK;
}

int b2_context_debug_net_timing(b2_context* c, int batch, void* const* bindings, b2_stream_t stream_, long long* out, int cap_ctas,
                                int* n_ctas) {
    Plan* plan = nullptr;
    if (!c || build_plan(c, batch, &plan)) return fail(B2_EINVAL, "no plan");
    NetRun* run = nullptr;
    for (Launch& L : plan->launches)
        if (L.kind == L_NET) run = L.net.get();
    if (!run) return fail(B2_EINVAL, "the plan has no persistent network kernel");
    if (n_ctas) *n_ctas = run->ctas;
    if (run->ctas > cap_ctas) return fail(B2_EINVAL, "counter buffer too small (%d CTAs)", run->ctas);
    long long* d = nullptr;
    const size_t bytes = size_t(run->ctas) * 64 * sizeof(long long);
    B2_CUDA(cudaMalloc(&d, bytes));
    cudaMemset(d, 0, bytes);
    cudaStream_t s = static_cast<cudaStream_t>(stream_);
    run->args.dbg = d;
    int rc = run_all(c, *plan, bindings, s);
    cudaError_t se = cudaStreamSynchronize(s);
    run->args.dbg = nullptr;
    if (!rc && se == cudaSuccess) cudaMemcpy(out, d, bytes, cudaMemcpyDeviceToHost);
    cudaFree(d);
    if (rc) return rc;
    if (se != cudaSuccess) return fail(B2_ECUDA, "debug launch failed: %s", cudaGetErrorString(se));
    return B2_OK;
}

int b2_debug_conv_residency(int bn, int kb, int stages, int sps, int residual, int halo_w, int halo_rows, int cblocks,
                            int* ctas_per_sm) {
    if (!ctas_per_sm) return fail(B2_EINVAL, "null output");
    const int rc = b2k::init_conv_kernels();
    if (rc) return fail(B2_ECUDA, "kernel attribute setup failed: %s", cudaGetErrorString(cudaError_t(rc)));
    *ctas_per_sm = b2k::conv_residency(bn, kb, stages, sps, residual != 0, halo_w, halo_rows, cblocks);
    if (*ctas_per_sm <= 0)
        return fail(B2_EINVAL, "no residency for bn=%d kb=%d st=%dx%d res=%d halo_w=%d", bn, kb, stages, sps, residual, halo_w);
    return B2_OK;
}

const char* b2_context_launch_name(b2_context* c, int batch, int i) {
    static thread_local std::string s;
    const Launch* L = get_launch(c, batch, i);
    if (!L) return nullptr;
    static const char* kinds[] = {"input_cast", "conv_tcgen05", "conv_simt", "maxpool", "avgpool", "fc", "softmax", "output_cast", "net_tcgen05", "tail_pool_fc_softmax",
                                  "quantize", "conv_i8_tcgen05", "avgpool_i8", "output_cast_i8", "embed_ln", "layernorm", "attention_f16_wgmma",
                                  "pooler", "output_cast_rows", "output_unpack_rows", "quantize_f8", "conv_f8_tcgen05", "avgpool_f8",
                                  "output_cast_f8"};
    s = std::string(kinds[L->kind]) + (L->kind == L_ATTENTION && L->attn.S > 128 ? "_ks" : "") +
        (L->kind == L_ATTENTION && L->attn.seq_off ? "_varlen" : "") + ":" + L->name;
    if (L->kind == L_CONV_TC)
        s += " bn=" + std::to_string(L->conv.bn) + " kb=" + std::to_string(L->conv.kb) +
             " st=" + std::to_string(L->conv.stages) + "x" + std::to_string(L->conv.sps) +
             (L->conv.ws_ctas ? " ws=" + std::to_string(L->conv.ws_ctas) : std::string()) +
             (L->conv.cn > 1 ? " cn=" + std::to_string(L->conv.cn) : std::string()) +
             (L->conv.halo == 2 ? " halo fused" : L->conv.halo ? " halo" : "") +
             (L->conv.args.a_mode == b2k::A_TILED ? " tiled" : " im2col") +
             " grid=" + std::to_string(L->conv.grid_n) + "x" + std::to_string(L->conv.grid_m) + "x" +
             std::to_string(L->conv.args.splits) + " kblk=" + std::to_string(L->conv.args.num_kblocks) +
             (L->conv.args.group_span ? " span=" + std::to_string(L->conv.args.group_span) : std::string()) +
             ((L->conv.args.relu & b2plan::kConvGelu) ? " gelu" : "") + (L->conv.args.live ? " live" : "");
    if (L->kind == L_CONV_I8 || L->kind == L_CONV_F8)
        s += " bn=" + std::to_string(L->i8.bn) + " st=" + std::to_string(L->i8.stages) + (L->i8.args.a_mode == b2k::A_TILED ? " tiled" : " im2col") + " grid=" +
             std::to_string(L->i8.grid_n) + "x" + std::to_string(L->i8.grid_m) + " kblk=" + std::to_string(L->i8.args.num_kblocks);
    if (L->kind == L_NET)
        s += " layers=" + std::to_string(L->net->args.n_layers) + " tiles=" + std::to_string(L->net->args.total_tiles) +
             " ctas=" + std::to_string(L->net->ctas) + " stages=" + std::to_string(L->net->args.stages);
    if (L->side_join >= 0) s += " side";
    return s.c_str();
}
double b2_context_launch_flops(b2_context* c, int batch, int i) {
    const Launch* L = get_launch(c, batch, i);
    return L ? L->flops : 0.0;
}
double b2_context_launch_bytes(b2_context* c, int batch, int i) {
    const Launch* L = get_launch(c, batch, i);
    return L ? L->bytes : 0.0;
}

}
```

### tensorrt_laboratory_b200/csrc/kernels.cu

```cuda
#include "kernels.h"

#include <stdio.h>
#include <stdlib.h>
#include <string.h>

#include <array>
#include <map>
#include <mutex>

#include "ptx_sm90.cuh"
#include "wgmma_sm90.cuh"

namespace b2k {

template <int BN, int STAGES, int SPS = 1>
struct ConvCfg {
    static constexpr int A_SUBBLK = 128 * 64 * 2;
    static constexpr int B_SUBBLK = BN * 64 * 2;
    static constexpr int A_STAGE = SPS * A_SUBBLK;
    static constexpr int B_STAGE = SPS * B_SUBBLK;
    static constexpr int PIPE_BYTES = STAGES * (A_STAGE + B_STAGE);
    static constexpr int TILE_BYTES = 128 * BN * 2;
    static_assert(TILE_BYTES <= PIPE_BYTES, "the output staging tile reuses the pipeline buffers");
};
// ... 364 lines not shown
            v1 = fmaxf(v1, 0.0f);
        }
        *reinterpret_cast<__half2*>(sOut + so) = __floats2half2_rn(v0, v1);
    };

    bool do_store = true;
    if (!split) {
        if (consumer) {
            if (has_res) mbar_wait(res_bar, 0);
#pragma unroll
            for (int j = 0; j < BN / 8; ++j)
#pragma unroll
                for (int h = 0; h < 2; ++h) finish_pair(fp.row0 + 8 * h, 8 * j + fp.col0, acc[4 * j + 2 * h], acc[4 * j + 2 * h + 1]);
        }
    } else {
        const int tile = blockIdx.y * gridDim.x + blockIdx.x;
        float* ws_tile = p.workspace + static_cast<size_t>(tile) * p.splits * (128 * BN);
        if (consumer) {
            float* mine = ws_tile + static_cast<size_t>(blockIdx.z) * (128 * BN);
#pragma unroll
            for (int j = 0; j < BN / 8; ++j)
#pragma unroll
                for (int h = 0; h < 2; ++h)
                    __stcg(reinterpret_cast<float2*>(mine + (fp.row0 + 8 * h) * BN + 8 * j + fp.col0),
                           make_float2(acc[4 * j + 2 * h], acc[4 * j + 2 * h + 1]));
        }
        __syncthreads();
        if (threadIdx.x == kActWarp * 32) {
            __threadfence();
            const int prev = atomicAdd(p.tile_counters + tile, 1);
            const uint32_t last = (prev == p.splits - 1) ? 1u : 0u;
            if (last) {
                p.tile_counters[tile] = 0;
                if (has_res) load_residual();
            }
            *last_flag = last;
        }
        __syncthreads();
        do_store = *last_flag != 0;
        if (do_store && consumer) {
            __threadfence();
            if (has_res) mbar_wait(res_bar, 0);
#pragma unroll 4
            for (int j = 0; j < BN / 8; ++j) {
#pragma unroll
                for (int h = 0; h < 2; ++h) {
                    const int row = fp.row0 + 8 * h, col = 8 * j + fp.col0;
                    float f0 = 0.f, f1 = 0.f;
                    for (int sp = 0; sp < p.splits; ++sp) {
                        const float2 t = __ldcg(reinterpret_cast<const float2*>(ws_tile + static_cast<size_t>(sp) * (128 * BN) + row * BN + col));
                        f0 += t.x;
                        f1 += t.y;
                    }
                    finish_pair(row, col, f0, f1);
                }
            }
        }
    }
    if (dbg && threadIdx.x == 0) dbg[6] = clock64();
    if (p.pdl_trigger == 2) pdl_launch_dependents();
    fence_proxy_async();
    __syncthreads();
    if (threadIdx.x == kActWarp * 32 && do_store) {
#pragma unroll
        for (int b = 0; b < NBOX; ++b) tma_store_2d(&mapOut, sOut + b * (128 * OROWB), n0 + b * OW, m0);
        tma_store_commit_and_wait_read();
    }
    if (cn > 1) {
        if (warp == kWgtWarp) {
            const int first = nk > STAGES ? nk - STAGES : 0;
            for (int i = first; i < nk; ++i) mbar_wait(&empty_bar[i % STAGES], (i / STAGES) & 1);
        }
        __syncthreads();
        cluster_sync_all();
    }
    if (dbg && threadIdx.x == 0) {
        dbg[7] = clock64();
        unsigned long long gt;
        asm volatile("mov.u64 %0, %%globaltimer;" : "=l"(gt));
        dbg[9] = static_cast<long long>(gt);
    }
}

__host__ __device__ constexpr int conv_ws_smem_bytes(int bn, int stages, int sps, bool residual) {
    return stages * sps * (128 * 64 * 2 + bn * 64 * 2) + 2 * 128 * bn * 2 + (residual ? 2 * 128 * bn * 2 : 0) + 256 + 1024;
}

template <int BN, int STAGES, int SPS>
__global__ void __launch_bounds__(kConvWsThreads, 1)
conv_f16_tcgen05_ws(const __grid_constant__ CUtensorMap mapA, const __grid_constant__ CUtensorMap mapOut,
                    const __grid_constant__ CUtensorMap mapRes, const ConvArgs p) {
    constexpr int A_SUBBLK = 128 * 64 * 2;
    constexpr int B_SUBBLK = BN * 64 * 2;
    constexpr int A_STAGE = SPS * A_SUBBLK;
    constexpr int B_STAGE = SPS * B_SUBBLK;
    constexpr int PIPE_BYTES = STAGES * (A_STAGE + B_STAGE);
    constexpr int TILE_BYTES = 128 * BN * 2;
    constexpr int OW = BN >= 64 ? 64 : 32;
    constexpr int OROWB = OW * 2;
    constexpr int NBOX = BN / OW;

    extern __shared__ uint8_t smem_raw[];
    uint8_t* smem = smem_raw + ((1024u - (smem_u32(smem_raw) & 1023u)) & 1023u);
    const bool has_res = p.residual != nullptr;
    uint8_t* sA = smem;
    uint8_t* sB = smem + STAGES * A_STAGE;
    uint8_t* sOut = smem + PIPE_BYTES;
    uint8_t* sRes = sOut + 2 * TILE_BYTES;
    uint8_t* tail = sRes + (has_res ? 2 * TILE_BYTES : 0);
    uint64_t* full_bar = reinterpret_cast<uint64_t*>(tail);
    uint64_t* empty_bar = full_bar + STAGES;
    uint64_t* res_full = empty_bar + STAGES;
    uint64_t* res_empty = res_full + 2;

    const int warp = threadIdx.x >> 5;
    const int lane = threadIdx.x & 31;
    const int num_tiles = p.tiles_m * p.tiles_n;
    const int nsteps = (p.num_kblocks + SPS - 1) / SPS;
    auto subs_in_step = [&](int i) -> int {
        const int rem = p.num_kblocks - i * SPS;
        return rem < SPS ? rem : SPS;
    };

    if (threadIdx.x == 0) {
        if (p.dbg) p.dbg[static_cast<size_t>(blockIdx.x) * 16] = clock64();
        tma_prefetch_desc(&mapA);
        tma_prefetch_desc(&mapOut);
        if (has_res) tma_prefetch_desc(&mapRes);
        for (int s = 0; s < STAGES; ++s) {
            mbar_init(&full_bar[s], 1);
            mbar_init(&empty_bar[s], kConsumerWarps);
        }
        for (int b = 0; b < 2; ++b) {
            mbar_init(&res_full[b], 1);
            mbar_init(&res_empty[b], 1);
        }
        fence_barrier_init();
        fence_proxy_async();
    }
    __syncthreads();
    if (p.pdl_trigger == 0) pdl_launch_dependents();
    long long* const dbg = p.dbg ? p.dbg + static_cast<size_t>(blockIdx.x) * 16 : nullptr;
    if (dbg && threadIdx.x == 0) dbg[1] = clock64();

    if (warp == 0) {
        pdl_wait();
        long long w_stage = 0;
        int g = 0;
        for (int tile = blockIdx.x; tile < num_tiles; tile += gridDim.x) {
            const int mt = tile / p.tiles_n;
            const int m0 = mt * 128;
            int img0 = 0, p0 = 0, q0 = 0;
            if (p.a_mode == A_IM2COL) {
                img0 = m0 / p.HoWo;
                const int rem = m0 - img0 * p.HoWo;
                p0 = rem / p.Wo;
                q0 = rem - p0 * p.Wo;
            }
            const int base_w = q0 * p.stride_w - p.pad_w;
            const int base_h = p0 * p.stride_h - p.pad_h;
            int cur_cb = 0, cur_r = 0, cur_sx = 0;
            for (int i = 0; i < nsteps; ++i, ++g) {
                const int s = g % STAGES;
                const long long t1 = dbg ? clock64() : 0;
                mbar_wait(&empty_bar[s], ((g / STAGES) & 1) ^ 1);
                if (dbg) w_stage += clock64() - t1;
// ... 731 lines not shown
static int init_one() {
    const int want = conv_smem_layout_bytes(BN, STAGES, true, SPS);
    const int bytes = want > 227 * 1024 ? conv_smem_layout_bytes(BN, STAGES, false, SPS) : want;
    if (CN == 1) {
        int e = set_conv_smem(conv_f16_tcgen05<BN, KB, STAGES, SPS, 1, true>, bytes);
        if (e) return e;
        if constexpr (KB == 64) {
            if ((e = set_conv_smem(conv_f16_tcgen05<BN, KB, STAGES, SPS, 1, false, 1>, bytes))) return e;
            if ((e = set_conv_smem(conv_f16_tcgen05<BN, KB, STAGES, SPS, 1, false, 2>, bytes))) return e;
            if ((e = set_conv_smem(conv_f16_tcgen05<BN, KB, STAGES, SPS, 1, false, 2, true>, bytes))) return e;
            if ((e = set_conv_smem(conv_f16_tcgen05<BN, KB, STAGES, SPS, 1, false, 2, false, true>, bytes))) return e;
            if ((e = set_conv_smem(conv_f16_tcgen05<BN, KB, STAGES, SPS, 1, false, 2, true, true>, bytes))) return e;
        }
    }
    return set_conv_smem(conv_f16_tcgen05<BN, KB, STAGES, SPS, CN>, bytes);
}

int conv_smem_bytes(int bn, int stages, bool residual, int sps) { return conv_smem_layout_bytes(bn, stages, residual, sps); }

#define B2_FOR_EACH_CONV(X) \
    X(32, 64, 1, 1) X(32, 64, 2, 1) X(32, 64, 4, 1) X(32, 64, 8, 1) \
    X(64, 64, 1, 1) X(64, 64, 2, 1) X(64, 64, 4, 1) X(64, 64, 8, 1) \
    X(128, 64, 1, 1) X(128, 64, 2, 1) X(128, 64, 4, 1) X(256, 64, 2, 1) X(256, 64, 4, 1) \
    X(32, 64, 2, 2) X(32, 64, 4, 2) X(64, 64, 2, 2) X(64, 64, 4, 2) X(128, 64, 2, 2) X(256, 64, 2, 2) \
    X(32, 8, 2, 1) X(32, 8, 4, 1) X(64, 8, 2, 1) X(64, 8, 4, 1) X(64, 8, 8, 1) X(128, 8, 4, 1) \
    X(32, 32, 2, 1) X(32, 32, 4, 1) X(64, 32, 1, 1) X(64, 32, 2, 1) X(64, 32, 4, 1) X(128, 32, 2, 1) X(128, 32, 4, 1)

int conv_halo_smem(int bn, int w, int r, int cblocks) { return halo_smem_bytes(bn, w, r, cblocks); }
bool conv_halo_config_exists(int bn) { return bn == 64 || bn == 128 || bn == 256; }
static int init_conv_halo_kernels() {
    int e;
    if ((e = set_conv_smem(conv3x3_halo_tcgen05<64>, 227 * 1024))) return e;
    if ((e = set_conv_smem(conv3x3_halo_tcgen05<128>, 227 * 1024))) return e;
    if ((e = set_conv_smem(conv3x3_halo_tcgen05<256>, 227 * 1024))) return e;
    if ((e = set_conv_smem(conv3x3_halo_1x1_tcgen05<64>, 227 * 1024))) return e;
    if ((e = set_conv_smem(conv3x3_halo_1x1_tcgen05<128>, 227 * 1024))) return e;
    return set_conv_smem(conv3x3_halo_1x1_tcgen05<256>, 227 * 1024);
}
int conv_halo_fused_smem(int bn, int w, int r, int cblocks, int cout2) { return halo_fused_smem_bytes(bn, w, r, cblocks, cout2); }
static int launch_conv_halo_fused(const ConvLaunch& L, cudaStream_t stream) {
    const int R = L.args.halo_rows;
    const size_t smem = size_t(halo_fused_smem_bytes(L.bn, L.args.Wo, R, L.args.cblocks, L.c2.Cout));
    if (smem > 227 * 1024 || R < 1 || R * (L.args.Wo + 2) > 128 || L.args.cblocks > kHaloMaxCBlocks || L.grid_n != 1 ||
        L.bn != L.args.Cout || L.c2.Cout < kFuseChunk || L.c2.Cout % kFuseChunk)
        return static_cast<int>(cudaErrorInvalidValue);
    dim3 grid(1, L.grid_m, 1);
    switch (L.bn) {
        case 64: return launch_kernel(conv3x3_halo_1x1_tcgen05<64>, grid, dim3(kConvThreads), smem, stream, true, L.mapA, L.mapRes, L.mapOut, L.args, L.c2);
        case 128: return launch_kernel(conv3x3_halo_1x1_tcgen05<128>, grid, dim3(kConvThreads), smem, stream, true, L.mapA, L.mapRes, L.mapOut, L.args, L.c2);
        case 256: return launch_kernel(conv3x3_halo_1x1_tcgen05<256>, grid, dim3(kConvThreads), smem, stream, true, L.mapA, L.mapRes, L.mapOut, L.args, L.c2);
    }
    return static_cast<int>(cudaErrorInvalidValue);
}
static int launch_conv_halo(const ConvLaunch& L, cudaStream_t stream) {
    if (L.halo == 2) return launch_conv_halo_fused(L, stream);
    const int R = L.args.halo_rows;
    const size_t smem = size_t(halo_smem_bytes(L.bn, L.args.Wo, R, L.args.cblocks));
    if (smem > 227 * 1024 || R < 1 || R * (L.args.Wo + 2) > 128 || L.args.cblocks > kHaloMaxCBlocks) return static_cast<int>(cudaErrorInvalidValue);
    dim3 grid(L.grid_n, L.grid_m, 1);
    switch (L.bn) {
        case 64: return launch_kernel(conv3x3_halo_tcgen05<64>, grid, dim3(kConvThreads), smem, stream, true, L.mapA, L.mapOut, L.args);
        case 128: return launch_kernel(conv3x3_halo_tcgen05<128>, grid, dim3(kConvThreads), smem, stream, true, L.mapA, L.mapOut, L.args);
        case 256: return launch_kernel(conv3x3_halo_tcgen05<256>, grid, dim3(kConvThreads), smem, stream, true, L.mapA, L.mapOut, L.args);
    }
    return static_cast<int>(cudaErrorInvalidValue);
}

#define B2_FOR_EACH_CONV_CLUSTER(X) \
    X(32, 4, 1, 2) X(32, 4, 1, 4) X(64, 1, 1, 2) X(64, 2, 1, 2) X(64, 2, 1, 4) X(64, 2, 2, 2) X(64, 4, 2, 2) X(64, 4, 2, 4) \
    X(128, 2, 1, 2) X(128, 2, 1, 4) X(128, 2, 2, 2)

int init_conv_ws_kernels();
int launch_conv_f16_tcgen05_ws(const ConvLaunch& L, cudaStream_t stream);

int conv_stem_ws_smem() { return conv_stem_ws_smem_bytes(); }
static int launch_conv_stem_ws(const ConvLaunch& L, cudaStream_t stream) {
    const ConvArgs& a = L.args;
    if (L.bn != 64 || a.Cout != 64 || a.Wo > 128 || a.taps != kStemRows || a.stride_h != kStemStride || a.residual != nullptr)
        return static_cast<int>(cudaErrorInvalidValue);
    return launch_kernel(conv_stem_ws_tcgen05, dim3(L.ws_ctas), dim3(kConvWsThreads), size_t(conv_stem_ws_smem_bytes()), stream, true,
                         L.mapA, L.mapB, L.mapOut, L.args);
}

int init_conv_kernels() {
    int e = init_conv_ws_kernels();
    if (e) return e;
    if ((e = static_cast<int>(cudaFuncSetAttribute(conv_stem_ws_tcgen05, cudaFuncAttributeMaxDynamicSharedMemorySize,
                                                   conv_stem_ws_smem_bytes()))))
        return e;
    if ((e = init_conv_halo_kernels())) return e;
#define B2_INIT(BN_, KB_, ST_, SPS_) \
    if ((e = init_one<BN_, KB_, ST_, SPS_>())) return e;
    B2_FOR_EACH_CONV(B2_INIT)
#undef B2_INIT
#define B2_INIT_CL(BN_, ST_, SPS_, CN_) \
    if ((e = init_one<BN_, 64, ST_, SPS_, CN_>())) return e;
    B2_FOR_EACH_CONV_CLUSTER(B2_INIT_CL)
#undef B2_INIT_CL
    return 0;
}

int launch_conv_f16_tcgen05(const ConvLaunch& L, cudaStream_t stream) {
    if (L.halo) return launch_conv_halo(L, stream);
    if (L.ws_ctas > 0) return L.kb == 32 ? launch_conv_stem_ws(L, stream) : launch_conv_f16_tcgen05_ws(L, stream);
    if (L.cn > 1) {
#define B2_CASE_CL(BN_, ST_, SPS_, CN_) \
    if (L.bn == BN_ && L.kb == 64 && L.stages == ST_ && L.sps == SPS_ && L.cn == CN_) return launch_one<BN_, 64, ST_, SPS_, CN_>(L, stream);
        B2_FOR_EACH_CONV_CLUSTER(B2_CASE_CL)
#undef B2_CASE_CL
        return static_cast<int>(cudaErrorInvalidValue);
    }
#define B2_CASE(BN_, KB_, ST_, SPS_) \
    if (L.bn == BN_ && L.kb == KB_ && L.stages == ST_ && L.sps == SPS_) return launch_one<BN_, KB_, ST_, SPS_>(L, stream);
    B2_FOR_EACH_CONV(B2_CASE)
#undef B2_CASE
    return static_cast<int>(cudaErrorInvalidValue);
}

#define B2_FOR_EACH_CONV_WS(X) \
    X(32, 4, 1) X(64, 2, 1) X(64, 4, 1) X(64, 2, 2) X(64, 4, 2) X(128, 2, 1) X(128, 4, 1) X(128, 2, 2)

template <int BN, int STAGES, int SPS>
static int launch_one_ws(const ConvLaunch& L, cudaStream_t stream) {
    const size_t smem = size_t(conv_ws_smem_bytes(BN, STAGES, SPS, L.args.residual != nullptr));
    return launch_kernel(conv_f16_tcgen05_ws<BN, STAGES, SPS>, dim3(L.ws_ctas), dim3(kConvWsThreads), smem, stream, true, L.mapA, L.mapOut,
                         L.mapRes, L.args);
}

int init_conv_ws_kernels() {
    int e = 0;
#define B2_INIT_WS(BN_, ST_, SPS_)                                                                                        \
    {                                                                                                                     \
        const int want = conv_ws_smem_bytes(BN_, ST_, SPS_, true);                                                        \
        e = static_cast<int>(cudaFuncSetAttribute(conv_f16_tcgen05_ws<BN_, ST_, SPS_>,                                    \
                                                  cudaFuncAttributeMaxDynamicSharedMemorySize,                            \
                                                  want > 227 * 1024 ? conv_ws_smem_bytes(BN_, ST_, SPS_, false) : want)); \
        if (e) return e;                                                                                                  \
    }
    B2_FOR_EACH_CONV_WS(B2_INIT_WS)
#undef B2_INIT_WS
    return 0;
}

int launch_conv_f16_tcgen05_ws(const ConvLaunch& L, cudaStream_t stream) {
#define B2_CASE_WS(BN_, ST_, SPS_) \
    if (L.bn == BN_ && L.stages == ST_ && L.sps == SPS_) return launch_one_ws<BN_, ST_, SPS_>(L, stream);
    B2_FOR_EACH_CONV_WS(B2_CASE_WS)
#undef B2_CASE_WS
    return static_cast<int>(cudaErrorInvalidValue);
}

bool conv_ws_config_exists(int bn, int stages, int sps) {
#define B2_HAS_WS(BN_, ST_, SPS_) \
    if (bn == BN_ && stages == ST_ && sps == SPS_) return true;
    B2_FOR_EACH_CONV_WS(B2_HAS_WS)
#undef B2_HAS_WS
    return false;
}

int conv_ws_smem(int bn, int stages, int sps, bool residual) { return conv_ws_smem_bytes(bn, stages, sps, residual); }

bool conv_cluster_config_exists(int bn, int stages, int sps, int cn) {
#define B2_HAS_CL(BN_, ST_, SPS_, CN_) \
    if (bn == BN_ && stages == ST_ && sps == SPS_ && cn == CN_) return true;
    B2_FOR_EACH_CONV_CLUSTER(B2_HAS_CL)
#undef B2_HAS_CL
    return false;
}

bool conv_config_exists(int bn, int kb, int stages, int sps) {
#define B2_HAS(BN_, KB_, ST_, SPS_) \
    if (bn == BN_ && kb == KB_ && stages == ST_ && sps == SPS_) return true;
    B2_FOR_EACH_CONV(B2_HAS)
#undef B2_HAS
    return false;
}

int conv_residency(int bn, int kb, int stages, int sps, bool residual, int halo_w, int halo_rows, int cblocks) {
    static std::mutex mu;
    static std::map<std::array<int, 8>, int> cache;
    const std::array<int, 8> key{bn, kb, stages, sps, residual ? 1 : 0, halo_w, halo_rows, cblocks};
    {
        std::lock_guard<std::mutex> lock(mu);
        const auto it = cache.find(key);
        if (it != cache.end()) return it->second;
    }
    const void* fn = nullptr;
    int smem = 0;
    if (halo_w > 0) {
        smem = halo_smem_bytes(bn, halo_w, halo_rows, cblocks);
        if (bn == 64) fn = reinterpret_cast<const void*>(conv3x3_halo_tcgen05<64>);
        if (bn == 128) fn = reinterpret_cast<const void*>(conv3x3_halo_tcgen05<128>);
        if (bn == 256) fn = reinterpret_cast<const void*>(conv3x3_halo_tcgen05<256>);
    } else {
        smem = conv_smem_layout_bytes(bn, stages, residual, sps);
#define B2_FN(BN_, KB_, ST_, SPS_) \
    if (bn == BN_ && kb == KB_ && stages == ST_ && sps == SPS_) fn = reinterpret_cast<const void*>(conv_f16_tcgen05<BN_, KB_, ST_, SPS_>);
        B2_FOR_EACH_CONV(B2_FN)
#undef B2_FN
    }
    if (!fn || smem > 227 * 1024) return 0;
    int n = 0;
    if (cudaOccupancyMaxActiveBlocksPerMultiprocessor(&n, fn, kConvThreads, static_cast<size_t>(smem)) != cudaSuccess) {
        cudaGetLastError();
        return 0;
    }
    if (n > 0) {
        std::lock_guard<std::mutex> lock(mu);
        cache[key] = n;
    }
    return n;
}

static thread_local int B2_LAUNCH_RC = 0;

template <typename T>
struct Acc;
template <>
struct Acc<float> {
    using type = double;
};
template <>
struct Acc<__half> {
    using type = float;
};
__device__ __forceinline__ float to_f(float v) { return v; }
__device__ __forceinline__ float to_f(__half v) { return __half2float(v); }
template <typename T>
__device__ __forceinline__ T from_f(float v);
template <>
__device__ __forceinline__ float from_f<float>(float v) { return v; }
template <>
__device__ __forceinline__ __half from_f<__half>(float v) { return __float2half_rn(v); }

template <typename T>
__global__ void conv_simt_kernel(SimtConvArgs a) {
    pdl_launch_dependents();
    pdl_wait();
    using acc_t = typename Acc<T>::type;
    const long long total = static_cast<long long>(a.N) * a.Ho * a.Wo * a.Cout_phys;
    const long long idx = blockIdx.x * static_cast<long long>(blockDim.x) + threadIdx.x;
    if (idx >= total) return;
    const int co = static_cast<int>(idx % a.Cout_phys);
    long long pix = idx / a.Cout_phys;
    const int wo = static_cast<int>(pix % a.Wo);
    pix /= a.Wo;
    const int ho = static_cast<int>(pix % a.Ho);
    const int n = static_cast<int>(pix / a.Ho);
    T* out = reinterpret_cast<T*>(a.out);
    if (co >= a.Cout) {
        out[idx] = from_f<T>(0.0f);
        return;
    }
    const int cin_g = a.Cin / a.groups;
    const int ci0 = co / (a.Cout / a.groups) * cin_g;
    const int kofs = (a.groups > 1 && a.w_packed) ? ci0 - co / a.wk_tap * a.wk_tap : 0;
    const T* in = reinterpret_cast<const T*>(a.in) + ci0;
    const T* w = reinterpret_cast<const T*>(a.w) + static_cast<size_t>(co) * a.taps_phys * a.wk_tap;
    acc_t acc = 0;
    for (int r = 0; r < a.kh; ++r) {
        const int hi = ho * a.stride_h - a.pad_h + r;
        if (hi < 0 || hi >= a.H) continue;
        for (int s = 0; s < a.kw; ++s) {
            const int wi = wo * a.stride_w - a.pad_w + s;
            if (wi < 0 || wi >= a.W) continue;
            const T* ip = in + ((static_cast<size_t>(n) * a.H + hi) * a.W + wi) * a.Cin_phys;
            const T* wp = w + static_cast<size_t>(r * a.kw + s) * a.wk_tap;
            if (a.w_packed) {
                const size_t kbase = static_cast<size_t>(r * a.kw + s) * a.wk_tap + kofs;
                for (int c = 0; c < cin_g; ++c) {
                    const size_t k = kbase + c;
                    const size_t kk = k & 63;
// ... 733 lines not shown
```

### tensorrt_laboratory_b200/csrc/kernels.h

```cpp
#pragma once
#include <cuda.h>
#include <cuda_fp16.h>
#include <cuda_runtime.h>
#include <stdint.h>

namespace b2k {

enum { A_TILED = 0, A_IM2COL = 1 };

struct ConvArgs {
    const float* bias;
    const __half* residual;
    __half* out;
    int M;
    int Cout;
    int num_kblocks;
    int cblocks;
    int taps;
    int taps_phys;
    int kw;
    int HoWo, Wo;
    int stride_h, stride_w;
    int pad_h, pad_w;
    int relu;
    int a_mode;
    int splits;
    int kb_per_split;
    float* workspace;
    union {
        int* tile_counters;
        const int* live_rows;
    };
    int pdl_trigger;
    const uint8_t* wpacked;
    int halo_rows;
    int cn;
    int tiles_m, tiles_n;
    int dbg_mode;
    long long* dbg;
    int group_span;
    int live;
};
static_assert(sizeof(ConvArgs) == 168, "ConvArgs layout");

struct Conv1x1Args {
    const uint8_t* wpacked;
    const float* bias;
    int Cout;
    int relu;
};

struct ConvLaunch {
    CUtensorMap mapA;
    CUtensorMap mapB;
    CUtensorMap mapOut;
    CUtensorMap mapRes;
    ConvArgs args;
    int bn;
    int kb;
    int stages;
    int sps;
    int grid_m, grid_n;
    int cn;
    int halo;
    int ws_ctas;
    Conv1x1Args c2;
};

int launch_conv_f16_tcgen05(const ConvLaunch& L, cudaStream_t stream);
int init_conv_kernels();
bool conv_config_exists(int bn, int kb, int stages, int sps = 1);
int conv_smem_bytes(int bn, int stages, bool residual, int sps = 1);
bool conv_cluster_config_exists(int bn, int stages, int sps, int cn);
bool conv_halo_config_exists(int bn);
int conv_halo_smem(int bn, int w, int r, int cblocks);
int conv_halo_fused_smem(int bn, int w, int r, int cblocks, int cout2);
int conv_residency(int bn, int kb, int stages, int sps, bool residual, int halo_w = 0, int halo_rows = 0, int cblocks = 0);
bool conv_ws_config_exists(int bn, int stages, int sps);
int conv_ws_smem(int bn, int stages, int sps, bool residual);
constexpr int kStemWsRing = 16;
int conv_stem_ws_smem();
void set_pdl(bool on);
bool get_pdl();

constexpr int kNetMaxLayers = 160;

struct NetLayerInfo {
    const uint8_t* wpacked;
    const float* bias;
    __half* out;
    const __half* residual;
    int M, Cout, num_kblocks, cblocks;
    int kw, HoWo, Wo, stride_h;
    int stride_w, pad_h, pad_w, relu;
    int a_mode, bn, tiles_m, tiles_n;
    int tile_begin, total_tiles;
    int in_flag_off;
    int in_need;
    int res_flag_off, res_need;
    int out_flag_off;
    int dep_off;
    int war_upto;
    int pad_[3];
};
static_assert(sizeof(NetLayerInfo) % 16 == 0, "NetLayerInfo is copied to shared memory in 16-byte words");
struct alignas(64) NetLayer {
    CUtensorMap mapA;
    NetLayerInfo info;
};
struct NetArgs {
    const NetLayer* layers;
    const short2* deps;
    int* mt_done;
    int* layer_done;
    int* ctrl;
    int n_layers, total_tiles, n_flags;
    int stages;
    long long* dbg;
};
int init_net_kernel();
int net_smem_bytes(int n_layers, int stages);
int launch_net_f16_tcgen05(const NetArgs& a, int ctas, cudaStream_t stream);

struct I8ConvArgs {
    const uint8_t* wpacked;
    const float* m;
    const float* b;
    float r;
    int has_res, relu;
    int M, Cout, num_kblocks, cblocks;
    int kw, HoWo, Wo, stride_h, stride_w, pad_h, pad_w, a_mode;
    int last_cb_mmas, cout_real;
};
struct I8ConvLaunch {
    CUtensorMap mapA;
    CUtensorMap mapOut;
    CUtensorMap mapRes;
    I8ConvArgs args;
    int bn, stages, grid_m, grid_n;
};
int init_conv_i8_kernels();
bool conv_i8_config_exists(int bn, int stages);
int conv_i8_smem_bytes(int bn, int stages, bool residual);
int launch_conv_i8_tcgen05(const I8ConvLaunch& L, cudaStream_t stream);
int launch_conv_f8_tcgen05(const I8ConvLaunch& L, cudaStream_t stream);
int launch_quantize_h_to_f8(const void* src, void* dst, long long pixels, int C, int C_in_phys, int C_out_phys, float inv_s,
                            cudaStream_t stream);
int launch_avgpool_f8(const void* src, void* dst, int N, int HW, int C, int C_in_phys, int C_out_phys, float k, cudaStream_t stream);
int launch_output_cast_f8(const void* src, float* dst, int N, int C, int H, int W, int C_phys, float s, cudaStream_t stream);
int launch_quantize_h_to_i8(const void* src, void* dst, long long pixels, int C, int C_in_phys, int C_out_phys, float inv_s,
                            cudaStream_t stream);
int launch_avgpool_i8(const void* src, void* dst, int N, int HW, int C, int C_in_phys, int C_out_phys, float k, cudaStream_t stream);
int launch_output_cast_i8(const void* src, float* dst, int N, int C, int H, int W, int C_phys, float s, cudaStream_t stream);

struct SimtConvArgs {
    const void* in;
    const void* w;
    const float* bias;
    const void* residual;
    void* out;
// ... 69 lines not shown
```

### tensorrt_laboratory_b200/csrc/plan_format.h

```cpp
#pragma once
#include <stdint.h>

namespace b2plan {

constexpr char kMagic[8] = {'B', '2', 'E', 'N', 'G', 'I', 'N', 'E'};
constexpr uint32_t kVersion = 1;
constexpr uint32_t kVersionGrouped = 2;
constexpr uint32_t kVersionTransformer = 3;

enum OpType : uint32_t {
    OP_INPUT_CAST = 0,
    OP_CONV = 1,
    OP_MAXPOOL = 2,
    OP_AVGPOOL = 3,
    OP_FC = 4,
    OP_SOFTMAX = 5,
    OP_OUTPUT_CAST = 6,
    OP_QUANTIZE = 7,
    OP_EMBED_LN = 8,
    OP_LAYERNORM = 9,
    OP_ATTENTION = 10,
    OP_POOLER = 11,
};

enum TensorKind : uint32_t { T_ACT = 0 , T_VEC = 1  };

#pragma pack(push, 1)
struct Header {
    char magic[8];
    uint32_t version;
    uint32_t precision;
    uint32_t max_batch;
    uint32_t n_tensors;
    uint32_t n_ops;
    uint32_t n_bindings;
    uint64_t payload_offset;
    uint64_t payload_bytes;
    char name[64];
    uint32_t n_tactics;
    uint32_t reserved;
    uint64_t tactics_offset;
};
struct TacticRec {
    uint32_t op, batch, bn, stages, splits, sps, ws, cn, halo, reserved;
};
struct TensorRec {
    char name[64];
    uint32_t kind;
    uint32_t h, w, c, c_phys;
    int32_t binding;
    float scale;
    uint8_t pad[4];
};
struct OpRec {
    char name[64];
    uint32_t type;
    int32_t in, res, out;
    int32_t binding;
    uint32_t k, stride, pad_;
    uint32_t relu;
    uint32_t ceil_mode;
    uint32_t cin, cout, cin_phys, cout_phys, taps, taps_phys;
    uint64_t w_off, w_bytes, b_off, b_bytes;
    uint32_t kw, stride_w, pad_w_lo, pad_w_hi;
};
struct OpRecV2 {
    OpRec v1;
    uint32_t groups;
    uint8_t reserved[12];
};
struct OpRecV3 {
    OpRec v1;
    uint32_t groups;
    uint32_t heads;
    uint32_t vocab, positions, types;
    int32_t binding2, binding3;
    int32_t out2;
    float eps;
    uint32_t flags;
    uint8_t reserved[8];
};
enum : uint32_t { kConvRelu = 1, kConvPacked = 2, kConvInt8 = 4, kConvGelu = 8 };
enum : uint32_t { kOpRowsOut = 1, kOpPacked = 2 };
struct BindingRec {
    char name[64];
    uint32_t is_input;
    uint32_t dtype;
    int32_t tensor;
    uint32_t nd;
    int32_t dims[8];
    uint8_t pad[16];
};
#pragma pack(pop)

static_assert(sizeof(Header) == 128, "Header size");
static_assert(sizeof(TacticRec) == 40, "TacticRec size");
static_assert(sizeof(TensorRec) == 96, "TensorRec size");
static_assert(sizeof(OpRec) == 176, "OpRec size");
static_assert(sizeof(OpRecV2) == 192, "OpRecV2 size");
static_assert(sizeof(OpRecV3) == 224, "OpRecV3 size");
static_assert(sizeof(BindingRec) == 128, "BindingRec size");

}
```

### tensorrt_laboratory_b200/csrc/wgmma_sm90.cuh

```cuda
#pragma once
#include <stdint.h>

namespace b2k {

__device__ __forceinline__ void wgmma_fence() { asm volatile("wgmma.fence.sync.aligned;" ::: "memory"); }
__device__ __forceinline__ void wgmma_commit() { asm volatile("wgmma.commit_group.sync.aligned;" ::: "memory"); }
template <int N>
__device__ __forceinline__ void wgmma_wait() { asm volatile("wgmma.wait_group.sync.aligned %0;" ::"n"(N) : "memory"); }

enum { WG_NOSWZ = 0, WG_SW128 = 1, WG_SW64 = 2 };
__device__ __forceinline__ uint64_t make_wgmma_desc(uint32_t saddr, uint32_t lbo_bytes, uint32_t sbo_bytes, uint32_t layout) {
    uint64_t d = 0;
    d |= static_cast<uint64_t>((saddr >> 4) & 0x3FFF);
    d |= static_cast<uint64_t>((lbo_bytes >> 4) & 0x3FFF) << 16;
    d |= static_cast<uint64_t>((sbo_bytes >> 4) & 0x3FFF) << 32;
    d |= static_cast<uint64_t>(layout & 3) << 62;
    return d;
}

__device__ __forceinline__ void wgmma_f16_n32(float (&d)[16], uint64_t a, uint64_t b, uint32_t accumulate) {
    asm volatile(
        "{\n.reg .pred p;\nsetp.ne.b32 p, %18, 0;\n"
        "wgmma.mma_async.sync.aligned.m64n32k16.f32.f16.f16 {%0, %1, %2, %3, %4, %5, %6, %7, %8, %9, %10, %11, %12, %13, %14, %15}, %16, %17, p, 1, 1, 0, 0;\n}\n"
        : "+f"(d[0]), "+f"(d[1]), "+f"(d[2]), "+f"(d[3]), "+f"(d[4]), "+f"(d[5]), "+f"(d[6]), "+f"(d[7]), "+f"(d[8]), "+f"(d[9]), "+f"(d[10]), "+f"(d[11]), "+f"(d[12]), "+f"(d[13]), "+f"(d[14]), "+f"(d[15])
        : "l"(a), "l"(b), "r"(accumulate));
}
__device__ __forceinline__ void wgmma_f16_n64(float (&d)[32], uint64_t a, uint64_t b, uint32_t accumulate) {
    asm volatile(
        "{\n.reg .pred p;\nsetp.ne.b32 p, %34, 0;\n"
        "wgmma.mma_async.sync.aligned.m64n64k16.f32.f16.f16 {%0, %1, %2, %3, %4, %5, %6, %7, %8, %9, %10, %11, %12, %13, %14, %15, %16, %17, %18, %19, %20, %21, %22, %23, %24, %25, %26, %27, %28, %29, %30, %31}, %32, %33, p, 1, 1, 0, 0;\n}\n"
        : "+f"(d[0]), "+f"(d[1]), "+f"(d[2]), "+f"(d[3]), "+f"(d[4]), "+f"(d[5]), "+f"(d[6]), "+f"(d[7]), "+f"(d[8]), "+f"(d[9]), "+f"(d[10]), "+f"(d[11]), "+f"(d[12]), "+f"(d[13]), "+f"(d[14]), "+f"(d[15]), "+f"(d[16]), "+f"(d[17]), "+f"(d[18]), "+f"(d[19]), "+f"(d[20]), "+f"(d[21]), "+f"(d[22]), "+f"(d[23]), "+f"(d[24]), "+f"(d[25]), "+f"(d[26]), "+f"(d[27]), "+f"(d[28]), "+f"(d[29]), "+f"(d[30]), "+f"(d[31])
        : "l"(a), "l"(b), "r"(accumulate));
}
__device__ __forceinline__ void wgmma_f16_n128(float (&d)[64], uint64_t a, uint64_t b, uint32_t accumulate) {
    asm volatile(
        "{\n.reg .pred p;\nsetp.ne.b32 p, %66, 0;\n"
        "wgmma.mma_async.sync.aligned.m64n128k16.f32.f16.f16 {%0, %1, %2, %3, %4, %5, %6, %7, %8, %9, %10, %11, %12, %13, %14, %15, %16, %17, %18, %19, %20, %21, %22, %23, %24, %25, %26, %27, %28, %29, %30, %31, %32, %33, %34, %35, %36, %37, %38, %39, %40, %41, %42, %43, %44, %45, %46, %47, %48, %49, %50, %51, %52, %53, %54, %55, %56, %57, %58, %59, %60, %61, %62, %63}, %64, %65, p, 1, 1, 0, 0;\n}\n"
        : "+f"(d[0]), "+f"(d[1]), "+f"(d[2]), "+f"(d[3]), "+f"(d[4]), "+f"(d[5]), "+f"(d[6]), "+f"(d[7]), "+f"(d[8]), "+f"(d[9]), "+f"(d[10]), "+f"(d[11]), "+f"(d[12]), "+f"(d[13]), "+f"(d[14]), "+f"(d[15]), "+f"(d[16]), "+f"(d[17]), "+f"(d[18]), "+f"(d[19]), "+f"(d[20]), "+f"(d[21]), "+f"(d[22]), "+f"(d[23]), "+f"(d[24]), "+f"(d[25]), "+f"(d[26]), "+f"(d[27]), "+f"(d[28]), "+f"(d[29]), "+f"(d[30]), "+f"(d[31]), "+f"(d[32]), "+f"(d[33]), "+f"(d[34]), "+f"(d[35]), "+f"(d[36]), "+f"(d[37]), "+f"(d[38]), "+f"(d[39]), "+f"(d[40]), "+f"(d[41]), "+f"(d[42]), "+f"(d[43]), "+f"(d[44]), "+f"(d[45]), "+f"(d[46]), "+f"(d[47]), "+f"(d[48]), "+f"(d[49]), "+f"(d[50]), "+f"(d[51]), "+f"(d[52]), "+f"(d[53]), "+f"(d[54]), "+f"(d[55]), "+f"(d[56]), "+f"(d[57]), "+f"(d[58]), "+f"(d[59]), "+f"(d[60]), "+f"(d[61]), "+f"(d[62]), "+f"(d[63])
        : "l"(a), "l"(b), "r"(accumulate));
}
__device__ __forceinline__ void wgmma_f16_n256(float (&d)[128], uint64_t a, uint64_t b, uint32_t accumulate) {
    asm volatile(
        "{\n.reg .pred p;\nsetp.ne.b32 p, %130, 0;\n"
        "wgmma.mma_async.sync.aligned.m64n256k16.f32.f16.f16 {%0, %1, %2, %3, %4, %5, %6, %7, %8, %9, %10, %11, %12, %13, %14, %15, %16, %17, %18, %19, %20, %21, %22, %23, %24, %25, %26, %27, %28, %29, %30, %31, %32, %33, %34, %35, %36, %37, %38, %39, %40, %41, %42, %43, %44, %45, %46, %47, %48, %49, %50, %51, %52, %53, %54, %55, %56, %57, %58, %59, %60, %61, %62, %63, %64, %65, %66, %67, %68, %69, %70, %71, %72, %73, %74, %75, %76, %77, %78, %79, %80, %81, %82, %83, %84, %85, %86, %87, %88, %89, %90, %91, %92, %93, %94, %95, %96, %97, %98, %99, %100, %101, %102, %103, %104, %105, %106, %107, %108, %109, %110, %111, %112, %113, %114, %115, %116, %117, %118, %119, %120, %121, %122, %123, %124, %125, %126, %127}, %128, %129, p, 1, 1, 0, 0;\n}\n"
        : "+f"(d[0]), "+f"(d[1]), "+f"(d[2]), "+f"(d[3]), "+f"(d[4]), "+f"(d[5]), "+f"(d[6]), "+f"(d[7]), "+f"(d[8]), "+f"(d[9]), "+f"(d[10]), "+f"(d[11]), "+f"(d[12]), "+f"(d[13]), "+f"(d[14]), "+f"(d[15]), "+f"(d[16]), "+f"(d[17]), "+f"(d[18]), "+f"(d[19]), "+f"(d[20]), "+f"(d[21]), "+f"(d[22]), "+f"(d[23]), "+f"(d[24]), "+f"(d[25]), "+f"(d[26]), "+f"(d[27]), "+f"(d[28]), "+f"(d[29]), "+f"(d[30]), "+f"(d[31]), "+f"(d[32]), "+f"(d[33]), "+f"(d[34]), "+f"(d[35]), "+f"(d[36]), "+f"(d[37]), "+f"(d[38]), "+f"(d[39]), "+f"(d[40]), "+f"(d[41]), "+f"(d[42]), "+f"(d[43]), "+f"(d[44]), "+f"(d[45]), "+f"(d[46]), "+f"(d[47]), "+f"(d[48]), "+f"(d[49]), "+f"(d[50]), "+f"(d[51]), "+f"(d[52]), "+f"(d[53]), "+f"(d[54]), "+f"(d[55]), "+f"(d[56]), "+f"(d[57]), "+f"(d[58]), "+f"(d[59]), "+f"(d[60]), "+f"(d[61]), "+f"(d[62]), "+f"(d[63]), "+f"(d[64]), "+f"(d[65]), "+f"(d[66]), "+f"(d[67]), "+f"(d[68]), "+f"(d[69]), "+f"(d[70]), "+f"(d[71]), "+f"(d[72]), "+f"(d[73]), "+f"(d[74]), "+f"(d[75]), "+f"(d[76]), "+f"(d[77]), "+f"(d[78]), "+f"(d[79]), "+f"(d[80]), "+f"(d[81]), "+f"(d[82]), "+f"(d[83]), "+f"(d[84]), "+f"(d[85]), "+f"(d[86]), "+f"(d[87]), "+f"(d[88]), "+f"(d[89]), "+f"(d[90]), "+f"(d[91]), "+f"(d[92]), "+f"(d[93]), "+f"(d[94]), "+f"(d[95]), "+f"(d[96]), "+f"(d[97]), "+f"(d[98]), "+f"(d[99]), "+f"(d[100]), "+f"(d[101]), "+f"(d[102]), "+f"(d[103]), "+f"(d[104]), "+f"(d[105]), "+f"(d[106]), "+f"(d[107]), "+f"(d[108]), "+f"(d[109]), "+f"(d[110]), "+f"(d[111]), "+f"(d[112]), "+f"(d[113]), "+f"(d[114]), "+f"(d[115]), "+f"(d[116]), "+f"(d[117]), "+f"(d[118]), "+f"(d[119]), "+f"(d[120]), "+f"(d[121]), "+f"(d[122]), "+f"(d[123]), "+f"(d[124]), "+f"(d[125]), "+f"(d[126]), "+f"(d[127])
        : "l"(a), "l"(b), "r"(accumulate));
}
__device__ __forceinline__ void wgmma_i8_n32(int32_t (&d)[16], uint64_t a, uint64_t b, uint32_t accumulate) {
    asm volatile(
        "{\n.reg .pred p;\nsetp.ne.b32 p, %18, 0;\n"
        "wgmma.mma_async.sync.aligned.m64n32k32.s32.s8.s8 {%0, %1, %2, %3, %4, %5, %6, %7, %8, %9, %10, %11, %12, %13, %14, %15}, %16, %17, p;\n}\n"
        : "+r"(d[0]), "+r"(d[1]), "+r"(d[2]), "+r"(d[3]), "+r"(d[4]), "+r"(d[5]), "+r"(d[6]), "+r"(d[7]), "+r"(d[8]), "+r"(d[9]), "+r"(d[10]), "+r"(d[11]), "+r"(d[12]), "+r"(d[13]), "+r"(d[14]), "+r"(d[15])
        : "l"(a), "l"(b), "r"(accumulate));
}
__device__ __forceinline__ void wgmma_i8_n64(int32_t (&d)[32], uint64_t a, uint64_t b, uint32_t accumulate) {
    asm volatile(
        "{\n.reg .pred p;\nsetp.ne.b32 p, %34, 0;\n"
        "wgmma.mma_async.sync.aligned.m64n64k32.s32.s8.s8 {%0, %1, %2, %3, %4, %5, %6, %7, %8, %9, %10, %11, %12, %13, %14, %15, %16, %17, %18, %19, %20, %21, %22, %23, %24, %25, %26, %27, %28, %29, %30, %31}, %32, %33, p;\n}\n"
        : "+r"(d[0]), "+r"(d[1]), "+r"(d[2]), "+r"(d[3]), "+r"(d[4]), "+r"(d[5]), "+r"(d[6]), "+r"(d[7]), "+r"(d[8]), "+r"(d[9]), "+r"(d[10]), "+r"(d[11]), "+r"(d[12]), "+r"(d[13]), "+r"(d[14]), "+r"(d[15]), "+r"(d[16]), "+r"(d[17]), "+r"(d[18]), "+r"(d[19]), "+r"(d[20]), "+r"(d[21]), "+r"(d[22]), "+r"(d[23]), "+r"(d[24]), "+r"(d[25]), "+r"(d[26]), "+r"(d[27]), "+r"(d[28]), "+r"(d[29]), "+r"(d[30]), "+r"(d[31])
        : "l"(a), "l"(b), "r"(accumulate));
}
__device__ __forceinline__ void wgmma_i8_n128(int32_t (&d)[64], uint64_t a, uint64_t b, uint32_t accumulate) {
    asm volatile(
        "{\n.reg .pred p;\nsetp.ne.b32 p, %66, 0;\n"
        "wgmma.mma_async.sync.aligned.m64n128k32.s32.s8.s8 {%0, %1, %2, %3, %4, %5, %6, %7, %8, %9, %10, %11, %12, %13, %14, %15, %16, %17, %18, %19, %20, %21, %22, %23, %24, %25, %26, %27, %28, %29, %30, %31, %32, %33, %34, %35, %36, %37, %38, %39, %40, %41, %42, %43, %44, %45, %46, %47, %48, %49, %50, %51, %52, %53, %54, %55, %56, %57, %58, %59, %60, %61, %62, %63}, %64, %65, p;\n}\n"
        : "+r"(d[0]), "+r"(d[1]), "+r"(d[2]), "+r"(d[3]), "+r"(d[4]), "+r"(d[5]), "+r"(d[6]), "+r"(d[7]), "+r"(d[8]), "+r"(d[9]), "+r"(d[10]), "+r"(d[11]), "+r"(d[12]), "+r"(d[13]), "+r"(d[14]), "+r"(d[15]), "+r"(d[16]), "+r"(d[17]), "+r"(d[18]), "+r"(d[19]), "+r"(d[20]), "+r"(d[21]), "+r"(d[22]), "+r"(d[23]), "+r"(d[24]), "+r"(d[25]), "+r"(d[26]), "+r"(d[27]), "+r"(d[28]), "+r"(d[29]), "+r"(d[30]), "+r"(d[31]), "+r"(d[32]), "+r"(d[33]), "+r"(d[34]), "+r"(d[35]), "+r"(d[36]), "+r"(d[37]), "+r"(d[38]), "+r"(d[39]), "+r"(d[40]), "+r"(d[41]), "+r"(d[42]), "+r"(d[43]), "+r"(d[44]), "+r"(d[45]), "+r"(d[46]), "+r"(d[47]), "+r"(d[48]), "+r"(d[49]), "+r"(d[50]), "+r"(d[51]), "+r"(d[52]), "+r"(d[53]), "+r"(d[54]), "+r"(d[55]), "+r"(d[56]), "+r"(d[57]), "+r"(d[58]), "+r"(d[59]), "+r"(d[60]), "+r"(d[61]), "+r"(d[62]), "+r"(d[63])
        : "l"(a), "l"(b), "r"(accumulate));
}
__device__ __forceinline__ void wgmma_i8_n256(int32_t (&d)[128], uint64_t a, uint64_t b, uint32_t accumulate) {
    asm volatile(
        "{\n.reg .pred p;\nsetp.ne.b32 p, %130, 0;\n"
        "wgmma.mma_async.sync.aligned.m64n256k32.s32.s8.s8 {%0, %1, %2, %3, %4, %5, %6, %7, %8, %9, %10, %11, %12, %13, %14, %15, %16, %17, %18, %19, %20, %21, %22, %23, %24, %25, %26, %27, %28, %29, %30, %31, %32, %33, %34, %35, %36, %37, %38, %39, %40, %41, %42, %43, %44, %45, %46, %47, %48, %49, %50, %51, %52, %53, %54, %55, %56, %57, %58, %59, %60, %61, %62, %63, %64, %65, %66, %67, %68, %69, %70, %71, %72, %73, %74, %75, %76, %77, %78, %79, %80, %81, %82, %83, %84, %85, %86, %87, %88, %89, %90, %91, %92, %93, %94, %95, %96, %97, %98, %99, %100, %101, %102, %103, %104, %105, %106, %107, %108, %109, %110, %111, %112, %113, %114, %115, %116, %117, %118, %119, %120, %121, %122, %123, %124, %125, %126, %127}, %128, %129, p;\n}\n"
        : "+r"(d[0]), "+r"(d[1]), "+r"(d[2]), "+r"(d[3]), "+r"(d[4]), "+r"(d[5]), "+r"(d[6]), "+r"(d[7]), "+r"(d[8]), "+r"(d[9]), "+r"(d[10]), "+r"(d[11]), "+r"(d[12]), "+r"(d[13]), "+r"(d[14]), "+r"(d[15]), "+r"(d[16]), "+r"(d[17]), "+r"(d[18]), "+r"(d[19]), "+r"(d[20]), "+r"(d[21]), "+r"(d[22]), "+r"(d[23]), "+r"(d[24]), "+r"(d[25]), "+r"(d[26]), "+r"(d[27]), "+r"(d[28]), "+r"(d[29]), "+r"(d[30]), "+r"(d[31]), "+r"(d[32]), "+r"(d[33]), "+r"(d[34]), "+r"(d[35]), "+r"(d[36]), "+r"(d[37]), "+r"(d[38]), "+r"(d[39]), "+r"(d[40]), "+r"(d[41]), "+r"(d[42]), "+r"(d[43]), "+r"(d[44]), "+r"(d[45]), "+r"(d[46]), "+r"(d[47]), "+r"(d[48]), "+r"(d[49]), "+r"(d[50]), "+r"(d[51]), "+r"(d[52]), "+r"(d[53]), "+r"(d[54]), "+r"(d[55]), "+r"(d[56]), "+r"(d[57]), "+r"(d[58]), "+r"(d[59]), "+r"(d[60]), "+r"(d[61]), "+r"(d[62]), "+r"(d[63]), "+r"(d[64]), "+r"(d[65]), "+r"(d[66]), "+r"(d[67]), "+r"(d[68]), "+r"(d[69]), "+r"(d[70]), "+r"(d[71]), "+r"(d[72]), "+r"(d[73]), "+r"(d[74]), "+r"(d[75]), "+r"(d[76]), "+r"(d[77]), "+r"(d[78]), "+r"(d[79]), "+r"(d[80]), "+r"(d[81]), "+r"(d[82]), "+r"(d[83]), "+r"(d[84]), "+r"(d[85]), "+r"(d[86]), "+r"(d[87]), "+r"(d[88]), "+r"(d[89]), "+r"(d[90]), "+r"(d[91]), "+r"(d[92]), "+r"(d[93]), "+r"(d[94]), "+r"(d[95]), "+r"(d[96]), "+r"(d[97]), "+r"(d[98]), "+r"(d[99]), "+r"(d[100]), "+r"(d[101]), "+r"(d[102]), "+r"(d[103]), "+r"(d[104]), "+r"(d[105]), "+r"(d[106]), "+r"(d[107]), "+r"(d[108]), "+r"(d[109]), "+r"(d[110]), "+r"(d[111]), "+r"(d[112]), "+r"(d[113]), "+r"(d[114]), "+r"(d[115]), "+r"(d[116]), "+r"(d[117]), "+r"(d[118]), "+r"(d[119]), "+r"(d[120]), "+r"(d[121]), "+r"(d[122]), "+r"(d[123]), "+r"(d[124]), "+r"(d[125]), "+r"(d[126]), "+r"(d[127])
        : "l"(a), "l"(b), "r"(accumulate));
}
__device__ __forceinline__ void wgmma_e4m3_n128(float (&d)[64], uint64_t a, uint64_t b, uint32_t accumulate) {
    asm volatile(
        "{\n.reg .pred p;\nsetp.ne.b32 p, %66, 0;\n"
        "wgmma.mma_async.sync.aligned.m64n128k32.f32.e4m3.e4m3 {%0, %1, %2, %3, %4, %5, %6, %7, %8, %9, %10, %11, %12, %13, %14, %15, %16, %17, %18, %19, %20, %21, %22, %23, %24, %25, %26, %27, %28, %29, %30, %31, %32, %33, %34, %35, %36, %37, %38, %39, %40, %41, %42, %43, %44, %45, %46, %47, %48, %49, %50, %51, %52, %53, %54, %55, %56, %57, %58, %59, %60, %61, %62, %63}, %64, %65, p, 1, 1;\n}\n"
        : "+f"(d[0]), "+f"(d[1]), "+f"(d[2]), "+f"(d[3]), "+f"(d[4]), "+f"(d[5]), "+f"(d[6]), "+f"(d[7]), "+f"(d[8]), "+f"(d[9]), "+f"(d[10]), "+f"(d[11]), "+f"(d[12]), "+f"(d[13]), "+f"(d[14]), "+f"(d[15]), "+f"(d[16]), "+f"(d[17]), "+f"(d[18]), "+f"(d[19]), "+f"(d[20]), "+f"(d[21]), "+f"(d[22]), "+f"(d[23]), "+f"(d[24]), "+f"(d[25]), "+f"(d[26]), "+f"(d[27]), "+f"(d[28]), "+f"(d[29]), "+f"(d[30]), "+f"(d[31]), "+f"(d[32]), "+f"(d[33]), "+f"(d[34]), "+f"(d[35]), "+f"(d[36]), "+f"(d[37]), "+f"(d[38]), "+f"(d[39]), "+f"(d[40]), "+f"(d[41]), "+f"(d[42]), "+f"(d[43]), "+f"(d[44]), "+f"(d[45]), "+f"(d[46]), "+f"(d[47]), "+f"(d[48]), "+f"(d[49]), "+f"(d[50]), "+f"(d[51]), "+f"(d[52]), "+f"(d[53]), "+f"(d[54]), "+f"(d[55]), "+f"(d[56]), "+f"(d[57]), "+f"(d[58]), "+f"(d[59]), "+f"(d[60]), "+f"(d[61]), "+f"(d[62]), "+f"(d[63])
        : "l"(a), "l"(b), "r"(accumulate));
}
__device__ __forceinline__ void wgmma_e4m3_n256(float (&d)[128], uint64_t a, uint64_t b, uint32_t accumulate) {
    asm volatile(
        "{\n.reg .pred p;\nsetp.ne.b32 p, %130, 0;\n"
        "wgmma.mma_async.sync.aligned.m64n256k32.f32.e4m3.e4m3 {%0, %1, %2, %3, %4, %5, %6, %7, %8, %9, %10, %11, %12, %13, %14, %15, %16, %17, %18, %19, %20, %21, %22, %23, %24, %25, %26, %27, %28, %29, %30, %31, %32, %33, %34, %35, %36, %37, %38, %39, %40, %41, %42, %43, %44, %45, %46, %47, %48, %49, %50, %51, %52, %53, %54, %55, %56, %57, %58, %59, %60, %61, %62, %63, %64, %65, %66, %67, %68, %69, %70, %71, %72, %73, %74, %75, %76, %77, %78, %79, %80, %81, %82, %83, %84, %85, %86, %87, %88, %89, %90, %91, %92, %93, %94, %95, %96, %97, %98, %99, %100, %101, %102, %103, %104, %105, %106, %107, %108, %109, %110, %111, %112, %113, %114, %115, %116, %117, %118, %119, %120, %121, %122, %123, %124, %125, %126, %127}, %128, %129, p, 1, 1;\n}\n"
        : "+f"(d[0]), "+f"(d[1]), "+f"(d[2]), "+f"(d[3]), "+f"(d[4]), "+f"(d[5]), "+f"(d[6]), "+f"(d[7]), "+f"(d[8]), "+f"(d[9]), "+f"(d[10]), "+f"(d[11]), "+f"(d[12]), "+f"(d[13]), "+f"(d[14]), "+f"(d[15]), "+f"(d[16]), "+f"(d[17]), "+f"(d[18]), "+f"(d[19]), "+f"(d[20]), "+f"(d[21]), "+f"(d[22]), "+f"(d[23]), "+f"(d[24]), "+f"(d[25]), "+f"(d[26]), "+f"(d[27]), "+f"(d[28]), "+f"(d[29]), "+f"(d[30]), "+f"(d[31]), "+f"(d[32]), "+f"(d[33]), "+f"(d[34]), "+f"(d[35]), "+f"(d[36]), "+f"(d[37]), "+f"(d[38]), "+f"(d[39]), "+f"(d[40]), "+f"(d[41]), "+f"(d[42]), "+f"(d[43]), "+f"(d[44]), "+f"(d[45]), "+f"(d[46]), "+f"(d[47]), "+f"(d[48]), "+f"(d[49]), "+f"(d[50]), "+f"(d[51]), "+f"(d[52]), "+f"(d[53]), "+f"(d[54]), "+f"(d[55]), "+f"(d[56]), "+f"(d[57]), "+f"(d[58]), "+f"(d[59]), "+f"(d[60]), "+f"(d[61]), "+f"(d[62]), "+f"(d[63]), "+f"(d[64]), "+f"(d[65]), "+f"(d[66]), "+f"(d[67]), "+f"(d[68]), "+f"(d[69]), "+f"(d[70]), "+f"(d[71]), "+f"(d[72]), "+f"(d[73]), "+f"(d[74]), "+f"(d[75]), "+f"(d[76]), "+f"(d[77]), "+f"(d[78]), "+f"(d[79]), "+f"(d[80]), "+f"(d[81]), "+f"(d[82]), "+f"(d[83]), "+f"(d[84]), "+f"(d[85]), "+f"(d[86]), "+f"(d[87]), "+f"(d[88]), "+f"(d[89]), "+f"(d[90]), "+f"(d[91]), "+f"(d[92]), "+f"(d[93]), "+f"(d[94]), "+f"(d[95]), "+f"(d[96]), "+f"(d[97]), "+f"(d[98]), "+f"(d[99]), "+f"(d[100]), "+f"(d[101]), "+f"(d[102]), "+f"(d[103]), "+f"(d[104]), "+f"(d[105]), "+f"(d[106]), "+f"(d[107]), "+f"(d[108]), "+f"(d[109]), "+f"(d[110]), "+f"(d[111]), "+f"(d[112]), "+f"(d[113]), "+f"(d[114]), "+f"(d[115]), "+f"(d[116]), "+f"(d[117]), "+f"(d[118]), "+f"(d[119]), "+f"(d[120]), "+f"(d[121]), "+f"(d[122]), "+f"(d[123]), "+f"(d[124]), "+f"(d[125]), "+f"(d[126]), "+f"(d[127])
        : "l"(a), "l"(b), "r"(accumulate));
}
template <int N>
__device__ __forceinline__ void wgmma_f16(float (&d)[N / 2], uint64_t a, uint64_t b, uint32_t accumulate) {
    if constexpr (N == 32) wgmma_f16_n32(d, a, b, accumulate);
    else if constexpr (N == 64) wgmma_f16_n64(d, a, b, accumulate);
    else if constexpr (N == 128) wgmma_f16_n128(d, a, b, accumulate);
    else wgmma_f16_n256(d, a, b, accumulate);
}
template <int N>
__device__ __forceinline__ void wgmma_i8(int32_t (&d)[N / 2], uint64_t a, uint64_t b, uint32_t accumulate) {
    if constexpr (N == 32) wgmma_i8_n32(d, a, b, accumulate);
    else if constexpr (N == 64) wgmma_i8_n64(d, a, b, accumulate);
    else if constexpr (N == 128) wgmma_i8_n128(d, a, b, accumulate);
    else wgmma_i8_n256(d, a, b, accumulate);
}
template <int N>
__device__ __forceinline__ void wgmma_e4m3(float (&d)[N / 2], uint64_t a, uint64_t b, uint32_t accumulate) {
    static_assert(N == 128 || N == 256, "wgmma_e4m3: N tile 128 or 256");
    if constexpr (N == 128) wgmma_e4m3_n128(d, a, b, accumulate);
    else wgmma_e4m3_n256(d, a, b, accumulate);
}

template <int N, class F>
__device__ __forceinline__ void wgmma_group(F&& mma) {
    wgmma_fence();
#pragma unroll
    for (int t = 0; t < N; ++t) mma(t);
    wgmma_commit();
}
template <int MAX, class F>
__device__ __forceinline__ void wgmma_group_upto(int n, F&& mma) {
    if constexpr (MAX > 1) {
        if (n < MAX) {
            wgmma_group_upto<MAX - 1>(n, mma);
            return;
        }
    }
    wgmma_group<MAX>(mma);
}

}
```

Baseline: 33310.

## Add swapped-operand conv kernel with narrow pixel tiles for padded small-M convs

Adds a conv kernel that swaps operand roles: weights (128 output channels) fill the wgmma M side and pixels become a narrow N tile (56, 104, 200 or 224). This is meant to cut wasted MMA work on convolutions whose pixel count leaves 128-row M tiles heavily padded, which is common in late ResNet stages at batch 8. The autotuner gains these candidates when padding is at least 10%, and the tactic cache and plan format gain an np field. It adds compile time, more register and shared-memory variants, and more autotune candidates.

```diff
diff --git a/__graft_entry__.py b/__graft_entry__.py
--- a/__graft_entry__.py
+++ b/__graft_entry__.py
@@ -62,8 +62,12 @@
 _SHARED_SM_THREADS = 320
 
 
-def _shared_sm_register_budget(bn: int):
-    ctas = 3 if bn <= 64 else 2 if bn <= 128 else 1
+_SWAP_KERNEL = re.compile(r"_ZN3b2k21conv_f16_swap_tcgen05ILi(\d+)E")
+
+
+def _shared_sm_register_budget(bn: int, ctas=None):
+    if ctas is None:
+        ctas = 3 if bn <= 64 else 2 if bn <= 128 else 1
     return None if ctas == 1 else 65536 // (_SHARED_SM_THREADS * ctas) // 8 * 8
 
 
@@ -80,8 +84,9 @@
             bad.append(f"{func}: {line.strip()}")
         m = re.search(r"Used (\d+) registers", line)
         k = _SHARED_SM_KERNEL.match(func) if (m and func) else None
-        if k:
-            budget = _shared_sm_register_budget(int(k.group(1)))
+        sw = _SWAP_KERNEL.match(func) if (m and func) else None
+        if k or sw:
+            budget = _shared_sm_register_budget(int(k.group(1))) if k else _shared_sm_register_budget(0, 2 if int(sw.group(1)) <= 104 else 1)
             if budget is not None and int(m.group(1)) > budget:
                 bad.append(f"{func}: {m.group(1)} registers, more than the {budget} at which its CTAs share an SM")
     return bad
diff --git a/tensorrt_laboratory_b200/csrc/engine.cu b/tensorrt_laboratory_b200/csrc/engine.cu
--- a/tensorrt_laboratory_b200/csrc/engine.cu
+++ b/tensorrt_laboratory_b200/csrc/engine.cu
@@ -212,6 +212,7 @@
     int ws = 0;
     int cn = 1;
     int halo = 0;
+    int np = 0;
 };
 static bool stage_depth_useful(int bn, int kb, int st, int kpc) {
     const int stgs[4] = {1, 2, 4, 8};
@@ -283,6 +284,7 @@
     int force_fuse = 0;
     int force_cn = 0;
     int force_ws = 0;
+    int force_np = 0;
     int pdl_trigger = 1;
     int no_fold = 0;
     int autotune = 4;
@@ -656,6 +658,7 @@
             if (t.op >= h.n_ops || t.batch == 0 || t.batch > h.max_batch) return fail(B2_EINVAL, "plan: tactic %u out of range", i);
             ConvConfig cfg{int(t.bn), int(t.stages), int(t.splits), 0.0, int(t.sps), int(t.ws), int(t.cn)};
             cfg.halo = int(t.halo);
+            cfg.np = int(t.np);
             e->tuned[{int(t.op), int(t.batch)}] = cfg;
         }
         e->tactics_from_plan = true;
@@ -885,7 +888,13 @@
     const b2plan::OpRec& r = op.r;
     const Tensor& to = c->e->tensors[r.out];
     const int span = op.group_span(), kb = conv_kb(c, op);
-    if (cfg.bn <= 0 || int(r.cout_phys) % cfg.bn || cfg.splits < 1 || cfg.sps < 1 || cfg.ws < 0) return false;
+    if (cfg.bn <= 0 || int(r.cout_phys) % cfg.bn || cfg.splits < 1 || cfg.sps < 1 || cfg.ws < 0 || cfg.np < 0) return false;
+    if (cfg.np && c->force_np < 0) return false;
+    if (cfg.np)
+        return b2k::conv_swap_config_exists(cfg.np, cfg.stages) && cfg.bn == 128 && cfg.sps == 1 &&
+               kb == 64 && (r.relu & 2) && op.groups == 1 && !span && !(r.relu & b2plan::kConvGelu) && !(op.flags & b2plan::kOpPacked) &&
+               cfg.splits == 1 && !cfg.ws && cfg.cn <= 1 && !cfg.halo && int(r.cout_phys) % 128 == 0 &&
+               b2k::conv_swap_smem(cfg.np, cfg.stages, r.res >= 0) <= kSmemLimit;
     if (op.groups > 1 && (!span || span % cfg.bn || cfg.splits > 1)) return false;
     if ((op.groups > 1 || (r.relu & b2plan::kConvGelu)) && (cfg.ws || cfg.cn > 1 || cfg.halo)) return false;
     if ((op.flags & b2plan::kOpPacked) && (cfg.ws || cfg.cn > 1 || cfg.halo || cfg.splits > 1)) return false;
@@ -976,6 +985,18 @@
         if (!halo.empty() && c->force_halo > 0) out.clear();
         out.insert(out.end(), halo.begin(), halo.end());
     }
+    const bool padded = (m_tiles * 128 - batch * int(c->e->tensors[r.out].h * c->e->tensors[r.out].w)) * 10 >= m_tiles * 128;
+    if (c->force_np >= 0 && fixed_splits <= 1 && (padded || c->force_np > 0)) {
+        std::vector<ConvConfig> swap;
+        for (int np : {56, 104, 200, 224})
+            for (int st : {2, 3, 4}) {
+                ConvConfig t{128, st, 1, 0.0, 1, 0, 1};
+                t.np = np;
+                if ((c->force_np == 0 || c->force_np == np) && ok(t)) swap.push_back(t);
+            }
+        if (!swap.empty() && c->force_np > 0) out.clear();
+        out.insert(out.end(), swap.begin(), swap.end());
+    }
     return out;
 }
 
@@ -1004,6 +1025,11 @@
         });
     if (c->force_halo > 0) force([](ConvConfig& t) { t.halo = 1, t.ws = 0, t.cn = 1; });
     if (c->force_cn > 1) force([&](ConvConfig& t) { t.cn = c->force_cn; });
+    if (c->force_np > 0)
+        force([&](ConvConfig& t) {
+            t = ConvConfig{128, b2k::conv_swap_stages(c->force_np), 1, t.est_us, 1, 0, 1};
+            t.np = c->force_np;
+        });
     return cfg;
 }
 
@@ -1019,8 +1045,8 @@
     const bool fold = conv_is_row_folded(c, op);
     const int span = op.group_span();
     if (!tactic_applies(c, op, batch, cfg))
-        return fail(B2_EINVAL, "conv %s: tactic bn=%d st=%d sps=%d splits=%d ws=%d cn=%d halo=%d does not apply", op.name.c_str(), cfg.bn,
-                    cfg.stages, cfg.sps, cfg.splits, cfg.ws, cfg.cn, cfg.halo);
+        return fail(B2_EINVAL, "conv %s: tactic bn=%d st=%d sps=%d splits=%d ws=%d cn=%d halo=%d np=%d does not apply", op.name.c_str(),
+                    cfg.bn, cfg.stages, cfg.sps, cfg.splits, cfg.ws, cfg.cn, cfg.halo, cfg.np);
     const bool gelu = (r.relu & b2plan::kConvGelu) != 0;
     b2k::ConvLaunch& cl = *out;
     memset(&cl, 0, sizeof cl);
@@ -1092,6 +1118,22 @@
     const CUtensorMapSwizzle swz = kb64 ? CU_TENSOR_MAP_SWIZZLE_128B : (fold ? CU_TENSOR_MAP_SWIZZLE_64B : CU_TENSOR_MAP_SWIZZLE_NONE);
     const uint64_t pix = uint64_t(r.cin_phys) * 2, rowb = uint64_t(ti.w) * pix, imgb = uint64_t(ti.h) * rowb;
     int rc;
+    if (cfg.np) {
+        const uint32_t np = uint32_t(cfg.np);
+        cl.np = cfg.np;
+        cl.grid_m = (M + cfg.np - 1) / cfg.np;
+        cl.args.tiles_m = cl.grid_m;
+        if (tiled)
+            rc = make_map_2d(&cl.mapA, tptr(r.in), r.cin_phys, uint64_t(M), 64, np, swz);
+        else
+            rc = make_map_im2col(&cl.mapA, tptr(r.in), int(r.cin_phys), int(ti.w), int(ti.h), batch, pix, rowb, imgb, op.kh(), op.kw(),
+                                 op.sh(), op.sw(), op.ph(), op.pw_lo(), op.pw_hi(), 64, np, swz);
+        cl.mapB = cl.mapA;
+        if (!rc) rc = make_map_2d(&cl.mapOut, tptr(r.out), r.cout_phys, uint64_t(M), 64, np, CU_TENSOR_MAP_SWIZZLE_128B);
+        if (!rc && r.res >= 0) rc = make_map_2d(&cl.mapRes, tptr(r.res), r.cout_phys, uint64_t(M), 64, np, CU_TENSOR_MAP_SWIZZLE_128B);
+        else cl.mapRes = cl.mapOut;
+        return rc;
+    }
     if (tiled)
         rc = make_map_2d(&cl.mapA, tptr(r.in), r.cin_phys, uint64_t(M), 64, uint32_t(128 / cl.cn), swz);
     else if (fold)
@@ -1263,15 +1305,15 @@
         if (err != cudaSuccess)
             return fail(B2_ECUDA, "autotune of %s (bn=%d st=%d) failed: %s", op.name.c_str(), cand.bn, cand.stages, cudaGetErrorString(err));
         if (verbose > 1)
-            fprintf(stderr, "[b2 tune]   %s b=%d cand bn=%d st=%d sp=%d sps=%d ws=%d cn=%d halo=%d : %.3f us/launch\n", op.name.c_str(),
-                    batch, cand.bn, cand.stages, cand.splits, cand.sps, cand.ws, cand.cn, cand.halo, tt.us_per_launch(ms));
+            fprintf(stderr, "[b2 tune]   %s b=%d cand bn=%d st=%d sp=%d sps=%d ws=%d cn=%d halo=%d np=%d : %.3f us/launch\n", op.name.c_str(),
+                    batch, cand.bn, cand.stages, cand.splits, cand.sps, cand.ws, cand.cn, cand.halo, cand.np, tt.us_per_launch(ms));
         if (ms < best_ms) best_ms = ms, best = cand;
     }
     best.est_us = tt.us_per_launch(best_ms);
     if (verbose)
-        fprintf(stderr, "[b2 tune] %s b=%d M=%d N=%d K=%d best bn=%d st=%d sp=%d sps=%d ws=%d cn=%d halo=%d : %.3f us/launch (%d streams)\n",
+        fprintf(stderr, "[b2 tune] %s b=%d M=%d N=%d K=%d best bn=%d st=%d sp=%d sps=%d ws=%d cn=%d halo=%d np=%d : %.3f us/launch (%d streams)\n",
                 op.name.c_str(), batch, M, int(r.cout_phys), conv_num_kblocks(c, op) * conv_kb(c, op), best.bn, best.stages, best.splits,
-                best.sps, best.ws, best.cn, best.halo, best.est_us, tt.ns);
+                best.sps, best.ws, best.cn, best.halo, best.np, best.est_us, tt.ns);
     *best_out = best;
     return B2_OK;
 }
@@ -1283,14 +1325,18 @@
     if (!path) return;
     FILE* f = fopen(path, "r");
     if (!f) return;
-    char name[128];
-    int op, batch, bn, st, sp, sps, ws, cn, halo;
-    while (fscanf(f, "%127s %d %d %d %d %d %d %d %d %d", name, &op, &batch, &bn, &st, &sp, &sps, &ws, &cn, &halo) == 10)
+    char line[512], name[128];
+    int op, batch, bn, st, sp, sps, ws, cn, halo, np;
+    while (fgets(line, sizeof line, f)) {
+        np = 0;
+        if (sscanf(line, "%127s %d %d %d %d %d %d %d %d %d %d", name, &op, &batch, &bn, &st, &sp, &sps, &ws, &cn, &halo, &np) < 10) continue;
         if (e->name == name && op >= 0 && op < int(e->ops.size())) {
             ConvConfig cfg{bn, st, sp, 0.0, sps, ws, cn};
             cfg.halo = halo;
+            cfg.np = np;
             e->tuned[{op, batch}] = cfg;
         }
+    }
     fclose(f);
 }
 void tune_cache_append(const b2_engine* e, int op, int batch, const ConvConfig& cfg) {
@@ -1298,8 +1344,9 @@
     if (!path) return;
     FILE* f = fopen(path, "a");
     if (!f) return;
-    fprintf(f, "%s %d %d %d %d %d %d %d %d %d\n", e->name.c_str(), op, batch, cfg.bn, cfg.stages, cfg.splits, cfg.sps, cfg.ws, cfg.cn,
-            cfg.halo);
+    fprintf(f, "%s %d %d %d %d %d %d %d %d %d", e->name.c_str(), op, batch, cfg.bn, cfg.stages, cfg.splits, cfg.sps, cfg.ws, cfg.cn, cfg.halo);
+    if (cfg.np) fprintf(f, " %d", cfg.np);
+    fputc('\n', f);
     fclose(f);
 }
 
@@ -1712,7 +1759,7 @@
                     L.kind = L_CONV_TC;
                     ConvConfig cfg = forced_conv_config(c, op, batch);
                     if (cfg.bn == 0) return fail(B2_EINVAL, "conv %s: no kernel configuration", op.name.c_str());
-                    const bool forced = c->force_bn || c->force_stages || c->force_splits || c->force_sps;
+                    const bool forced = c->force_bn || c->force_stages || c->force_splits || c->force_sps || c->force_np > 0;
                     const int op_index = int(&op - &e->ops[0]);
                     const bool net_ok = c->net && !forced && conv_kb(c, op) == 64 && (r.relu & 2) && r.cout_phys % 64 == 0 &&
                                         c->force_ws <= 0 && c->force_cn <= 0 && c->force_halo <= 0 && !c->force_im2col && op.groups == 1 &&
@@ -2297,6 +2344,7 @@
     c->force_splits = env_int("B2_FORCE_SPLITS", 0);
     c->force_sps = env_int("B2_FORCE_SPS", 0);
     c->force_ws = env_int("B2_FORCE_WS", 0);
+    c->force_np = env_int("B2_FORCE_NP", 0);
     c->force_cn = env_int("B2_FORCE_CN", 0);
     c->force_halo = env_int("B2_FORCE_HALO", 0);
     c->force_fuse = env_int("B2_FORCE_FUSE", 0);
@@ -2365,6 +2413,7 @@
     else if (k == "splits") c->force_splits = value;
     else if (k == "sps") c->force_sps = value;
     else if (k == "ws") c->force_ws = value;
+    else if (k == "np") c->force_np = value;
     else if (k == "cn") c->force_cn = value;
     else if (k == "halo") c->force_halo = value;
     else if (k == "fuse") c->force_fuse = value;
@@ -2582,7 +2631,7 @@
         if (n >= cap) break;
         const ConvConfig& g = kv.second;
         const uint32_t rec[10] = {uint32_t(kv.first.first), uint32_t(kv.first.second), uint32_t(g.bn), uint32_t(g.stages), uint32_t(g.splits),
-                                  uint32_t(g.sps), uint32_t(g.ws), uint32_t(g.cn), uint32_t(g.halo), 0u};
+                                  uint32_t(g.sps), uint32_t(g.ws), uint32_t(g.cn), uint32_t(g.halo), uint32_t(g.np)};
         memcpy(out + size_t(n) * 10, rec, sizeof rec);
         ++n;
     }
@@ -2757,6 +2806,7 @@
              (L->conv.ws_ctas ? " ws=" + std::to_string(L->conv.ws_ctas) : std::string()) +
              (L->conv.cn > 1 ? " cn=" + std::to_string(L->conv.cn) : std::string()) +
              (L->conv.halo == 2 ? " halo fused" : L->conv.halo ? " halo" : "") +
+             (L->conv.np ? " swap np" + std::to_string(L->conv.np) : std::string()) +
              (L->conv.args.a_mode == b2k::A_TILED ? " tiled" : " im2col") +
              " grid=" + std::to_string(L->conv.grid_n) + "x" + std::to_string(L->conv.grid_m) + "x" +
              std::to_string(L->conv.args.splits) + " kblk=" + std::to_string(L->conv.args.num_kblocks) +
diff --git a/tensorrt_laboratory_b200/csrc/kernels.cu b/tensorrt_laboratory_b200/csrc/kernels.cu
--- a/tensorrt_laboratory_b200/csrc/kernels.cu
+++ b/tensorrt_laboratory_b200/csrc/kernels.cu
@@ -470,6 +470,193 @@
     }
 }
 
+__host__ __device__ constexpr int swap_smem_layout_bytes(int np, int stages, bool residual) {
+    return stages * (128 * 128 + np * 128) + (residual ? np * 256 : 0) + 256 + 128 * 4 + 1024;
+}
+__host__ __device__ constexpr int swap_min_ctas(int np) { return np <= 104 ? 2 : 1; }
+
+template <int NP, int STAGES, int AV>
+__global__ void __launch_bounds__(kConvThreads, swap_min_ctas(NP))
+conv_f16_swap_tcgen05(const __grid_constant__ CUtensorMap mapA, const __grid_constant__ CUtensorMap mapOut,
+                      const __grid_constant__ CUtensorMap mapRes, const ConvArgs p) {
+    static_assert(NP % 8 == 0 && NP <= 256, "wgmma N: a multiple of 8 up to 256");
+    static_assert(AV == 1 || AV == 2, "im2col or tiled activations, packed weights");
+    constexpr int W_STAGE = 128 * 128;
+    constexpr int X_STAGE = NP * 128;
+    constexpr int PIPE_BYTES = STAGES * (W_STAGE + X_STAGE);
+    constexpr int BOX = NP * 128;
+    static_assert(2 * BOX <= PIPE_BYTES, "the output staging tile reuses the pipeline buffers");
+
+    extern __shared__ uint8_t smem_raw[];
+    uint8_t* smem = smem_raw + ((1024u - (smem_u32(smem_raw) & 1023u)) & 1023u);
+    const bool has_res = p.residual != nullptr;
+    uint8_t* sW = smem;
+    uint8_t* sX = smem + STAGES * W_STAGE;
+    uint8_t* sOut = smem;
+    uint8_t* sRes = smem + PIPE_BYTES;
+    uint8_t* tail = sRes + (has_res ? 2 * BOX : 0);
+    uint64_t* full_bar = reinterpret_cast<uint64_t*>(tail);
+    uint64_t* empty_bar = full_bar + STAGES;
+    uint64_t* res_bar = empty_bar + STAGES;
+    float* s_bias = reinterpret_cast<float*>(tail + 256);
+
+    const int warp = threadIdx.x >> 5;
+    const int lane = threadIdx.x & 31;
+    const int c0 = blockIdx.x * 128;
+    const int m0 = blockIdx.y * NP;
+    const int nk = p.num_kblocks;
+    constexpr uint32_t kStageBytes = W_STAGE + X_STAGE;
+
+    if (threadIdx.x == 0) {
+        tma_prefetch_desc(&mapA);
+        tma_prefetch_desc(&mapOut);
+        if (has_res) tma_prefetch_desc(&mapRes);
+        for (int s = 0; s < STAGES; ++s) {
+            mbar_init(&full_bar[s], 1);
+            mbar_init(&empty_bar[s], static_cast<uint32_t>(kConsumerWarps));
+        }
+        mbar_init(res_bar, 1);
+        fence_barrier_init();
+        fence_proxy_async();
+    }
+    __syncthreads();
+    if (warp == kWgtWarp) {
+#pragma unroll
+        for (int i = 0; i < 4; ++i) s_bias[lane + 32 * i] = __ldg(p.bias + c0 + lane + 32 * i);
+    }
+    if (p.pdl_trigger == 0) pdl_launch_dependents();
+
+    const int npre = nk < STAGES ? nk : STAGES;
+    if (warp == kActWarp) {
+        int img0 = 0, p0 = 0, q0 = 0;
+        if (AV == 1) {
+            img0 = m0 / p.HoWo;
+            const int rem = m0 - img0 * p.HoWo;
+            p0 = rem / p.Wo;
+            q0 = rem - p0 * p.Wo;
+        }
+        const int base_w = q0 * p.stride_w - p.pad_w;
+        const int base_h = p0 * p.stride_h - p.pad_h;
+        int cur_cb = 0, cur_r = 0, cur_sx = 0;
+        auto load_x = [&](int s) {
+            uint8_t* dst = sX + s * X_STAGE;
+            if (AV == 2) {
+                tma_load_2d(&mapA, &full_bar[s], dst, cur_cb * 64, m0);
+            } else {
+                tma_load_im2col_4d(&mapA, &full_bar[s], dst, cur_cb * 64, base_w, base_h, img0, static_cast<uint16_t>(cur_sx),
+                                   static_cast<uint16_t>(cur_r));
+            }
+            if (++cur_cb == p.cblocks) {
+                cur_cb = 0;
+                if (++cur_sx == p.kw) {
+                    cur_sx = 0;
+                    ++cur_r;
+                }
+            }
+        };
+        if (elect_one_sync())
+            for (int i = 0; i < npre; ++i) mbar_expect_tx(&full_bar[i], kStageBytes);
+        __syncwarp();
+        pdl_wait();
+        if (elect_one_sync()) {
+            for (int i = 0; i < npre; ++i) load_x(i);
+            if (has_res) {
+                mbar_expect_tx(res_bar, 2 * BOX);
+                tma_load_2d(&mapRes, res_bar, sRes, c0, m0);
+                tma_load_2d(&mapRes, res_bar, sRes + BOX, c0 + 64, m0);
+            }
+        }
+        __syncwarp();
+        for (int i = npre; i < nk; ++i) {
+            const int s = i % STAGES;
+            mbar_wait(&empty_bar[s], ((i / STAGES) & 1) ^ 1);
+            if (elect_one_sync()) {
+                mbar_expect_tx(&full_bar[s], kStageBytes);
+                load_x(s);
+            }
+            __syncwarp();
+        }
+    }
+
+    const int cw = warp;
+    const bool consumer = warp < kConsumerWarps;
+    float acc[NP / 2];
+    if (consumer) {
+        const uint32_t wg = static_cast<uint32_t>(cw >> 2);
+        auto release_stage = [&](int st) {
+            __syncwarp();
+            if (lane == 0) mbar_arrive(&empty_bar[st]);
+        };
+        for (int i = 0; i < nk; ++i) {
+            const int s = i % STAGES;
+            mbar_wait(&full_bar[s], (i / STAGES) & 1);
+            const uint32_t w_addr = smem_u32(sW + s * W_STAGE);
+            const uint32_t x_addr = smem_u32(sX + s * X_STAGE);
+            wgmma_group<4>([&](int j) {
+                const uint64_t ad = make_wgmma_desc(w_addr + wg * 8192 + j * 32, 16, 1024, WG_SW128);
+                const uint64_t bd = make_wgmma_desc(x_addr + j * 32, 16, 1024, WG_SW128);
+                wgmma_f16<NP>(acc, ad, bd, (i > 0 || j > 0) ? 1u : 0u);
+            });
+            wgmma_wait<1>();
+            if (i > 0) release_stage((i - 1) % STAGES);
+        }
+        wgmma_wait<0>();
+        if (nk > 0) release_stage((nk - 1) % STAGES);
+    }
+
+    if (warp == kWgtWarp) {
+        for (int i = 0; i < nk; ++i) {
+            const int s = i % STAGES;
+            if (i >= STAGES) mbar_wait(&empty_bar[s], ((i / STAGES) & 1) ^ 1);
+            if (elect_one_sync())
+                bulk_load_1d(&full_bar[s], sW + s * W_STAGE, p.wpacked + (static_cast<size_t>(i) * (p.Cout >> 5) + (c0 >> 5)) * 4096, W_STAGE);
+            __syncwarp();
+        }
+    }
+
+    pdl_wait();
+    __syncthreads();
+    if (p.pdl_trigger == 1) pdl_launch_dependents();
+    if (consumer) {
+        const int wg = cw >> 2;
+        const bool odd = (lane >> 2) & 1;
+        const int ch0 = 16 * (cw & 3) + ((lane >> 2) & ~1);
+        const int px0 = 2 * (lane & 3) + (odd ? 1 : 0);
+        uint8_t* box_out = sOut + wg * BOX;
+        const uint8_t* box_res = sRes + wg * BOX;
+        if (has_res) mbar_wait(res_bar, 0);
+#pragma unroll
+        for (int j = 0; j < NP / 8; ++j)
+#pragma unroll
+            for (int h = 0; h < 2; ++h) {
+                const float a0 = acc[4 * j + 2 * h], a1 = acc[4 * j + 2 * h + 1];
+                const float other = __shfl_xor_sync(0xffffffffu, odd ? a0 : a1, 4);
+                const int ch = ch0 + 8 * h, px = 8 * j + px0;
+                const uint32_t so = swz_off<128>(px, ch >> 3) + (ch & 7) * 2;
+                float v0 = (odd ? other : a0) + s_bias[64 * wg + ch];
+                float v1 = (odd ? a1 : other) + s_bias[64 * wg + ch + 1];
+                if (has_res) {
+                    const float2 rf = __half22float2(*reinterpret_cast<const __half2*>(box_res + so));
+                    v0 += rf.x;
+                    v1 += rf.y;
+                }
+                if (p.relu) {
+                    v0 = fmaxf(v0, 0.0f);
+                    v1 = fmaxf(v1, 0.0f);
+                }
+                *reinterpret_cast<__half2*>(box_out + so) = __floats2half2_rn(v0, v1);
+            }
+    }
+    if (p.pdl_trigger == 2) pdl_launch_dependents();
+    fence_proxy_async();
+    __syncthreads();
+    if (threadIdx.x == kActWarp * 32) {
+        tma_store_2d(&mapOut, sOut, c0, m0);
+        tma_store_2d(&mapOut, sOut + BOX, c0 + 64, m0);
+        tma_store_commit_and_wait_read();
+    }
+}
+
 __host__ __device__ constexpr int conv_ws_smem_bytes(int bn, int stages, int sps, bool residual) {
     return stages * sps * (128 * 64 * 2 + bn * 64 * 2) + 2 * 128 * bn * 2 + (residual ? 2 * 128 * bn * 2 : 0) + 256 + 1024;
 }
@@ -1367,6 +1554,7 @@
                          L.mapA, L.mapB, L.mapOut, L.args);
 }
 
+static int init_conv_swap_kernels();
 int init_conv_kernels() {
     int e = init_conv_ws_kernels();
     if (e) return e;
@@ -1374,6 +1562,7 @@
                                                    conv_stem_ws_smem_bytes()))))
         return e;
     if ((e = init_conv_halo_kernels())) return e;
+    if ((e = init_conv_swap_kernels())) return e;
 #define B2_INIT(BN_, KB_, ST_, SPS_) \
     if ((e = init_one<BN_, KB_, ST_, SPS_>())) return e;
     B2_FOR_EACH_CONV(B2_INIT)
@@ -1385,7 +1574,55 @@
     return 0;
 }
 
+#define B2_FOR_EACH_CONV_SWAP(X) X(56, 4) X(104, 4) X(200, 4) X(224, 3)
+
+bool conv_swap_config_exists(int np, int stages) {
+#define B2_HAS_SW(NP_, ST_) \
+    if (np == NP_ && stages == ST_) return true;
+    B2_FOR_EACH_CONV_SWAP(B2_HAS_SW)
+#undef B2_HAS_SW
+    return false;
+}
+int conv_swap_stages(int np) {
+    int st = 0;
+#define B2_ST_SW(NP_, ST_) \
+    if (np == NP_ && ST_ > st) st = ST_;
+    B2_FOR_EACH_CONV_SWAP(B2_ST_SW)
+#undef B2_ST_SW
+    return st;
+}
+int conv_swap_smem(int np, int stages, bool residual) { return swap_smem_layout_bytes(np, stages, residual); }
+
+static int init_conv_swap_kernels() {
+    int e;
+#define B2_INIT_SW(NP_, ST_)                                                                                  \
+    if ((e = set_conv_smem(conv_f16_swap_tcgen05<NP_, ST_, 1>, swap_smem_layout_bytes(NP_, ST_, true)))) return e; \
+    if ((e = set_conv_smem(conv_f16_swap_tcgen05<NP_, ST_, 2>, swap_smem_layout_bytes(NP_, ST_, true)))) return e;
+    B2_FOR_EACH_CONV_SWAP(B2_INIT_SW)
+#undef B2_INIT_SW
+    return 0;
+}
+
+static int launch_conv_swap(const ConvLaunch& L, cudaStream_t stream) {
+    if (L.args.wpacked == nullptr || L.kb != 64 || L.args.splits != 1 || L.args.group_span || (L.args.relu & 8) || L.args.live)
+        return static_cast<int>(cudaErrorInvalidValue);
+    const dim3 grid(L.grid_n, L.grid_m);
+    const size_t smem = size_t(conv_swap_smem(L.np, L.stages, L.args.residual != nullptr));
+#define B2_CASE_SW(NP_, ST_)                                                                                                 \
+    if (L.np == NP_ && L.stages == ST_) {                                                                                    \
+        if (L.args.a_mode == A_TILED)                                                                                        \
+            return launch_kernel(conv_f16_swap_tcgen05<NP_, ST_, 2>, grid, dim3(kConvThreads), smem, stream, true, L.mapA, L.mapOut, \
+                                 L.mapRes, L.args);                                                                          \
+        return launch_kernel(conv_f16_swap_tcgen05<NP_, ST_, 1>, grid, dim3(kConvThreads), smem, stream, true, L.mapA, L.mapOut,     \
+                             L.mapRes, L.args);                                                                              \
+    }
+    B2_FOR_EACH_CONV_SWAP(B2_CASE_SW)
+#undef B2_CASE_SW
+    return static_cast<int>(cudaErrorInvalidValue);
+}
+
 int launch_conv_f16_tcgen05(const ConvLaunch& L, cudaStream_t stream) {
+    if (L.np) return launch_conv_swap(L, stream);
     if (L.halo) return launch_conv_halo(L, stream);
     if (L.ws_ctas > 0) return L.kb == 32 ? launch_conv_stem_ws(L, stream) : launch_conv_f16_tcgen05_ws(L, stream);
     if (L.cn > 1) {
@@ -1461,10 +1698,10 @@
     return false;
 }
 
-int conv_residency(int bn, int kb, int stages, int sps, bool residual, int halo_w, int halo_rows, int cblocks) {
+int conv_residency(int bn, int kb, int stages, int sps, bool residual, int halo_w, int halo_rows, int cblocks, int np) {
     static std::mutex mu;
-    static std::map<std::array<int, 8>, int> cache;
-    const std::array<int, 8> key{bn, kb, stages, sps, residual ? 1 : 0, halo_w, halo_rows, cblocks};
+    static std::map<std::array<int, 9>, int> cache;
+    const std::array<int, 9> key{bn, kb, stages, sps, residual ? 1 : 0, halo_w, halo_rows, cblocks, np};
     {
         std::lock_guard<std::mutex> lock(mu);
         const auto it = cache.find(key);
@@ -1472,7 +1709,13 @@
     }
     const void* fn = nullptr;
     int smem = 0;
-    if (halo_w > 0) {
+    if (np > 0) {
+        smem = conv_swap_smem(np, stages, residual);
+#define B2_FN_SW(NP_, ST_) \
+    if (np == NP_ && stages == ST_) fn = reinterpret_cast<const void*>(conv_f16_swap_tcgen05<NP_, ST_, 1>);
+        B2_FOR_EACH_CONV_SWAP(B2_FN_SW)
+#undef B2_FN_SW
+    } else if (halo_w > 0) {
         smem = halo_smem_bytes(bn, halo_w, halo_rows, cblocks);
         if (bn == 64) fn = reinterpret_cast<const void*>(conv3x3_halo_tcgen05<64>);
         if (bn == 128) fn = reinterpret_cast<const void*>(conv3x3_halo_tcgen05<128>);
diff --git a/tensorrt_laboratory_b200/csrc/kernels.h b/tensorrt_laboratory_b200/csrc/kernels.h
--- a/tensorrt_laboratory_b200/csrc/kernels.h
+++ b/tensorrt_laboratory_b200/csrc/kernels.h
@@ -65,6 +65,7 @@
     int halo;
     int ws_ctas;
     Conv1x1Args c2;
+    int np;
 };
 
 int launch_conv_f16_tcgen05(const ConvLaunch& L, cudaStream_t stream);
@@ -75,7 +76,10 @@
 bool conv_halo_config_exists(int bn);
 int conv_halo_smem(int bn, int w, int r, int cblocks);
 int conv_halo_fused_smem(int bn, int w, int r, int cblocks, int cout2);
-int conv_residency(int bn, int kb, int stages, int sps, bool residual, int halo_w = 0, int halo_rows = 0, int cblocks = 0);
+int conv_residency(int bn, int kb, int stages, int sps, bool residual, int halo_w = 0, int halo_rows = 0, int cblocks = 0, int np = 0);
+bool conv_swap_config_exists(int np, int stages);
+int conv_swap_stages(int np);
+int conv_swap_smem(int np, int stages, bool residual);
 bool conv_ws_config_exists(int bn, int stages, int sps);
 int conv_ws_smem(int bn, int stages, int sps, bool residual);
 constexpr int kStemWsRing = 16;
diff --git a/tensorrt_laboratory_b200/csrc/plan_format.h b/tensorrt_laboratory_b200/csrc/plan_format.h
--- a/tensorrt_laboratory_b200/csrc/plan_format.h
+++ b/tensorrt_laboratory_b200/csrc/plan_format.h
@@ -42,7 +42,8 @@
     uint64_t tactics_offset;
 };
 struct TacticRec {
-    uint32_t op, batch, bn, stages, splits, sps, ws, cn, halo, reserved;
+    uint32_t op, batch, bn, stages, splits, sps, ws, cn, halo;
+    uint32_t np;
 };
 struct TensorRec {
     char name[64];
diff --git a/tensorrt_laboratory_b200/csrc/wgmma_sm90.cuh b/tensorrt_laboratory_b200/csrc/wgmma_sm90.cuh
--- a/tensorrt_laboratory_b200/csrc/wgmma_sm90.cuh
+++ b/tensorrt_laboratory_b200/csrc/wgmma_sm90.cuh
@@ -44,6 +44,34 @@
         "{\n.reg .pred p;\nsetp.ne.b32 p, %130, 0;\n"
         "wgmma.mma_async.sync.aligned.m64n256k16.f32.f16.f16 {%0, %1, %2, %3, %4, %5, %6, %7, %8, %9, %10, %11, %12, %13, %14, %15, %16, %17, %18, %19, %20, %21, %22, %23, %24, %25, %26, %27, %28, %29, %30, %31, %32, %33, %34, %35, %36, %37, %38, %39, %40, %41, %42, %43, %44, %45, %46, %47, %48, %49, %50, %51, %52, %53, %54, %55, %56, %57, %58, %59, %60, %61, %62, %63, %64, %65, %66, %67, %68, %69, %70, %71, %72, %73, %74, %75, %76, %77, %78, %79, %80, %81, %82, %83, %84, %85, %86, %87, %88, %89, %90, %91, %92, %93, %94, %95, %96, %97, %98, %99, %100, %101, %102, %103, %104, %105, %106, %107, %108, %109, %110, %111, %112, %113, %114, %115, %116, %117, %118, %119, %120, %121, %122, %123, %124, %125, %126, %127}, %128, %129, p, 1, 1, 0, 0;\n}\n"
         : "+f"(d[0]), "+f"(d[1]), "+f"(d[2]), "+f"(d[3]), "+f"(d[4]), "+f"(d[5]), "+f"(d[6]), "+f"(d[7]), "+f"(d[8]), "+f"(d[9]), "+f"(d[10]), "+f"(d[11]), "+f"(d[12]), "+f"(d[13]), "+f"(d[14]), "+f"(d[15]), "+f"(d[16]), "+f"(d[17]), "+f"(d[18]), "+f"(d[19]), "+f"(d[20]), "+f"(d[21]), "+f"(d[22]), "+f"(d[23]), "+f"(d[24]), "+f"(d[25]), "+f"(d[26]), "+f"(d[27]), "+f"(d[28]), "+f"(d[29]), "+f"(d[30]), "+f"(d[31]), "+f"(d[32]), "+f"(d[33]), "+f"(d[34]), "+f"(d[35]), "+f"(d[36]), "+f"(d[37]), "+f"(d[38]), "+f"(d[39]), "+f"(d[40]), "+f"(d[41]), "+f"(d[42]), "+f"(d[43]), "+f"(d[44]), "+f"(d[45]), "+f"(d[46]), "+f"(d[47]), "+f"(d[48]), "+f"(d[49]), "+f"(d[50]), "+f"(d[51]), "+f"(d[52]), "+f"(d[53]), "+f"(d[54]), "+f"(d[55]), "+f"(d[56]), "+f"(d[57]), "+f"(d[58]), "+f"(d[59]), "+f"(d[60]), "+f"(d[61]), "+f"(d[62]), "+f"(d[63]), "+f"(d[64]), "+f"(d[65]), "+f"(d[66]), "+f"(d[67]), "+f"(d[68]), "+f"(d[69]), "+f"(d[70]), "+f"(d[71]), "+f"(d[72]), "+f"(d[73]), "+f"(d[74]), "+f"(d[75]), "+f"(d[76]), "+f"(d[77]), "+f"(d[78]), "+f"(d[79]), "+f"(d[80]), "+f"(d[81]), "+f"(d[82]), "+f"(d[83]), "+f"(d[84]), "+f"(d[85]), "+f"(d[86]), "+f"(d[87]), "+f"(d[88]), "+f"(d[89]), "+f"(d[90]), "+f"(d[91]), "+f"(d[92]), "+f"(d[93]), "+f"(d[94]), "+f"(d[95]), "+f"(d[96]), "+f"(d[97]), "+f"(d[98]), "+f"(d[99]), "+f"(d[100]), "+f"(d[101]), "+f"(d[102]), "+f"(d[103]), "+f"(d[104]), "+f"(d[105]), "+f"(d[106]), "+f"(d[107]), "+f"(d[108]), "+f"(d[109]), "+f"(d[110]), "+f"(d[111]), "+f"(d[112]), "+f"(d[113]), "+f"(d[114]), "+f"(d[115]), "+f"(d[116]), "+f"(d[117]), "+f"(d[118]), "+f"(d[119]), "+f"(d[120]), "+f"(d[121]), "+f"(d[122]), "+f"(d[123]), "+f"(d[124]), "+f"(d[125]), "+f"(d[126]), "+f"(d[127])
+        : "l"(a), "l"(b), "r"(accumulate));
+}
+__device__ __forceinline__ void wgmma_f16_n56(float (&d)[28], uint64_t a, uint64_t b, uint32_t accumulate) {
+    asm volatile(
+        "{\n.reg .pred p;\nsetp.ne.b32 p, %30, 0;\n"
+        "wgmma.mma_async.sync.aligned.m64n56k16.f32.f16.f16 {%0, %1, %2, %3, %4, %5, %6, %7, %8, %9, %10, %11, %12, %13, %14, %15, %16, %17, %18, %19, %20, %21, %22, %23, %24, %25, %26, %27}, %28, %29, p, 1, 1, 0, 0;\n}\n"
+        : "+f"(d[0]), "+f"(d[1]), "+f"(d[2]), "+f"(d[3]), "+f"(d[4]), "+f"(d[5]), "+f"(d[6]), "+f"(d[7]), "+f"(d[8]), "+f"(d[9]), "+f"(d[10]), "+f"(d[11]), "+f"(d[12]), "+f"(d[13]), "+f"(d[14]), "+f"(d[15]), "+f"(d[16]), "+f"(d[17]), "+f"(d[18]), "+f"(d[19]), "+f"(d[20]), "+f"(d[21]), "+f"(d[22]), "+f"(d[23]), "+f"(d[24]), "+f"(d[25]), "+f"(d[26]), "+f"(d[27])
+        : "l"(a), "l"(b), "r"(accumulate));
+}
+__device__ __forceinline__ void wgmma_f16_n104(float (&d)[52], uint64_t a, uint64_t b, uint32_t accumulate) {
+    asm volatile(
+        "{\n.reg .pred p;\nsetp.ne.b32 p, %54, 0;\n"
+        "wgmma.mma_async.sync.aligned.m64n104k16.f32.f16.f16 {%0, %1, %2, %3, %4, %5, %6, %7, %8, %9, %10, %11, %12, %13, %14, %15, %16, %17, %18, %19, %20, %21, %22, %23, %24, %25, %26, %27, %28, %29, %30, %31, %32, %33, %34, %35, %36, %37, %38, %39, %40, %41, %42, %43, %44, %45, %46, %47, %48, %49, %50, %51}, %52, %53, p, 1, 1, 0, 0;\n}\n"
+        : "+f"(d[0]), "+f"(d[1]), "+f"(d[2]), "+f"(d[3]), "+f"(d[4]), "+f"(d[5]), "+f"(d[6]), "+f"(d[7]), "+f"(d[8]), "+f"(d[9]), "+f"(d[10]), "+f"(d[11]), "+f"(d[12]), "+f"(d[13]), "+f"(d[14]), "+f"(d[15]), "+f"(d[16]), "+f"(d[17]), "+f"(d[18]), "+f"(d[19]), "+f"(d[20]), "+f"(d[21]), "+f"(d[22]), "+f"(d[23]), "+f"(d[24]), "+f"(d[25]), "+f"(d[26]), "+f"(d[27]), "+f"(d[28]), "+f"(d[29]), "+f"(d[30]), "+f"(d[31]), "+f"(d[32]), "+f"(d[33]), "+f"(d[34]), "+f"(d[35]), "+f"(d[36]), "+f"(d[37]), "+f"(d[38]), "+f"(d[39]), "+f"(d[40]), "+f"(d[41]), "+f"(d[42]), "+f"(d[43]), "+f"(d[44]), "+f"(d[45]), "+f"(d[46]), "+f"(d[47]), "+f"(d[48]), "+f"(d[49]), "+f"(d[50]), "+f"(d[51])
+        : "l"(a), "l"(b), "r"(accumulate));
+}
+__device__ __forceinline__ void wgmma_f16_n200(float (&d)[100], uint64_t a, uint64_t b, uint32_t accumulate) {
+    asm volatile(
+        "{\n.reg .pred p;\nsetp.ne.b32 p, %102, 0;\n"
+        "wgmma.mma_async.sync.aligned.m64n200k16.f32.f16.f16 {%0, %1, %2, %3, %4, %5, %6, %7, %8, %9, %10, %11, %12, %13, %14, %15, %16, %17, %18, %19, %20, %21, %22, %23, %24, %25, %26, %27, %28, %29, %30, %31, %32, %33, %34, %35, %36, %37, %38, %39, %40, %41, %42, %43, %44, %45, %46, %47, %48, %49, %50, %51, %52, %53, %54, %55, %56, %57, %58, %59, %60, %61, %62, %63, %64, %65, %66, %67, %68, %69, %70, %71, %72, %73, %74, %75, %76, %77, %78, %79, %80, %81, %82, %83, %84, %85, %86, %87, %88, %89, %90, %91, %92, %93, %94, %95, %96, %97, %98, %99}, %100, %101, p, 1, 1, 0, 0;\n}\n"
+        : "+f"(d[0]), "+f"(d[1]), "+f"(d[2]), "+f"(d[3]), "+f"(d[4]), "+f"(d[5]), "+f"(d[6]), "+f"(d[7]), "+f"(d[8]), "+f"(d[9]), "+f"(d[10]), "+f"(d[11]), "+f"(d[12]), "+f"(d[13]), "+f"(d[14]), "+f"(d[15]), "+f"(d[16]), "+f"(d[17]), "+f"(d[18]), "+f"(d[19]), "+f"(d[20]), "+f"(d[21]), "+f"(d[22]), "+f"(d[23]), "+f"(d[24]), "+f"(d[25]), "+f"(d[26]), "+f"(d[27]), "+f"(d[28]), "+f"(d[29]), "+f"(d[30]), "+f"(d[31]), "+f"(d[32]), "+f"(d[33]), "+f"(d[34]), "+f"(d[35]), "+f"(d[36]), "+f"(d[37]), "+f"(d[38]), "+f"(d[39]), "+f"(d[40]), "+f"(d[41]), "+f"(d[42]), "+f"(d[43]), "+f"(d[44]), "+f"(d[45]), "+f"(d[46]), "+f"(d[47]), "+f"(d[48]), "+f"(d[49]), "+f"(d[50]), "+f"(d[51]), "+f"(d[52]), "+f"(d[53]), "+f"(d[54]), "+f"(d[55]), "+f"(d[56]), "+f"(d[57]), "+f"(d[58]), "+f"(d[59]), "+f"(d[60]), "+f"(d[61]), "+f"(d[62]), "+f"(d[63]), "+f"(d[64]), "+f"(d[65]), "+f"(d[66]), "+f"(d[67]), "+f"(d[68]), "+f"(d[69]), "+f"(d[70]), "+f"(d[71]), "+f"(d[72]), "+f"(d[73]), "+f"(d[74]), "+f"(d[75]), "+f"(d[76]), "+f"(d[77]), "+f"(d[78]), "+f"(d[79]), "+f"(d[80]), "+f"(d[81]), "+f"(d[82]), "+f"(d[83]), "+f"(d[84]), "+f"(d[85]), "+f"(d[86]), "+f"(d[87]), "+f"(d[88]), "+f"(d[89]), "+f"(d[90]), "+f"(d[91]), "+f"(d[92]), "+f"(d[93]), "+f"(d[94]), "+f"(d[95]), "+f"(d[96]), "+f"(d[97]), "+f"(d[98]), "+f"(d[99])
+        : "l"(a), "l"(b), "r"(accumulate));
+}
+__device__ __forceinline__ void wgmma_f16_n224(float (&d)[112], uint64_t a, uint64_t b, uint32_t accumulate) {
+    asm volatile(
+        "{\n.reg .pred p;\nsetp.ne.b32 p, %114, 0;\n"
+        "wgmma.mma_async.sync.aligned.m64n224k16.f32.f16.f16 {%0, %1, %2, %3, %4, %5, %6, %7, %8, %9, %10, %11, %12, %13, %14, %15, %16, %17, %18, %19, %20, %21, %22, %23, %24, %25, %26, %27, %28, %29, %30, %31, %32, %33, %34, %35, %36, %37, %38, %39, %40, %41, %42, %43, %44, %45, %46, %47, %48, %49, %50, %51, %52, %53, %54, %55, %56, %57, %58, %59, %60, %61, %62, %63, %64, %65, %66, %67, %68, %69, %70, %71, %72, %73, %74, %75, %76, %77, %78, %79, %80, %81, %82, %83, %84, %85, %86, %87, %88, %89, %90, %91, %92, %93, %94, %95, %96, %97, %98, %99, %100, %101, %102, %103, %104, %105, %106, %107, %108, %109, %110, %111}, %112, %113, p, 1, 1, 0, 0;\n}\n"
+        : "+f"(d[0]), "+f"(d[1]), "+f"(d[2]), "+f"(d[3]), "+f"(d[4]), "+f"(d[5]), "+f"(d[6]), "+f"(d[7]), "+f"(d[8]), "+f"(d[9]), "+f"(d[10]), "+f"(d[11]), "+f"(d[12]), "+f"(d[13]), "+f"(d[14]), "+f"(d[15]), "+f"(d[16]), "+f"(d[17]), "+f"(d[18]), "+f"(d[19]), "+f"(d[20]), "+f"(d[21]), "+f"(d[22]), "+f"(d[23]), "+f"(d[24]), "+f"(d[25]), "+f"(d[26]), "+f"(d[27]), "+f"(d[28]), "+f"(d[29]), "+f"(d[30]), "+f"(d[31]), "+f"(d[32]), "+f"(d[33]), "+f"(d[34]), "+f"(d[35]), "+f"(d[36]), "+f"(d[37]), "+f"(d[38]), "+f"(d[39]), "+f"(d[40]), "+f"(d[41]), "+f"(d[42]), "+f"(d[43]), "+f"(d[44]), "+f"(d[45]), "+f"(d[46]), "+f"(d[47]), "+f"(d[48]), "+f"(d[49]), "+f"(d[50]), "+f"(d[51]), "+f"(d[52]), "+f"(d[53]), "+f"(d[54]), "+f"(d[55]), "+f"(d[56]), "+f"(d[57]), "+f"(d[58]), "+f"(d[59]), "+f"(d[60]), "+f"(d[61]), "+f"(d[62]), "+f"(d[63]), "+f"(d[64]), "+f"(d[65]), "+f"(d[66]), "+f"(d[67]), "+f"(d[68]), "+f"(d[69]), "+f"(d[70]), "+f"(d[71]), "+f"(d[72]), "+f"(d[73]), "+f"(d[74]), "+f"(d[75]), "+f"(d[76]), "+f"(d[77]), "+f"(d[78]), "+f"(d[79]), "+f"(d[80]), "+f"(d[81]), "+f"(d[82]), "+f"(d[83]), "+f"(d[84]), "+f"(d[85]), "+f"(d[86]), "+f"(d[87]), "+f"(d[88]), "+f"(d[89]), "+f"(d[90]), "+f"(d[91]), "+f"(d[92]), "+f"(d[93]), "+f"(d[94]), "+f"(d[95]), "+f"(d[96]), "+f"(d[97]), "+f"(d[98]), "+f"(d[99]), "+f"(d[100]), "+f"(d[101]), "+f"(d[102]), "+f"(d[103]), "+f"(d[104]), "+f"(d[105]), "+f"(d[106]), "+f"(d[107]), "+f"(d[108]), "+f"(d[109]), "+f"(d[110]), "+f"(d[111])
         : "l"(a), "l"(b), "r"(accumulate));
 }
 __device__ __forceinline__ void wgmma_i8_n32(int32_t (&d)[16], uint64_t a, uint64_t b, uint32_t accumulate) {
@@ -93,7 +121,11 @@
     if constexpr (N == 32) wgmma_f16_n32(d, a, b, accumulate);
     else if constexpr (N == 64) wgmma_f16_n64(d, a, b, accumulate);
     else if constexpr (N == 128) wgmma_f16_n128(d, a, b, accumulate);
-    else wgmma_f16_n256(d, a, b, accumulate);
+    else if constexpr (N == 256) wgmma_f16_n256(d, a, b, accumulate);
+    else if constexpr (N == 56) wgmma_f16_n56(d, a, b, accumulate);
+    else if constexpr (N == 104) wgmma_f16_n104(d, a, b, accumulate);
+    else if constexpr (N == 200) wgmma_f16_n200(d, a, b, accumulate);
+    else wgmma_f16_n224(d, a, b, accumulate);
 }
 template <int N>
 __device__ __forceinline__ void wgmma_i8(int32_t (&d)[N / 2], uint64_t a, uint64_t b, uint32_t accumulate) {
```

Result: no change. 33620 (median of 6 runs) (+0.9%).
